# swacisko/ALGA

Hardware: AMD Instinct MI355X
Metric: overlap_edges_per_sec (higher is better)
Workload: dtype u32; 1 GPU; cfg4_50M_150bp: 50000000 x 150 bp reads, genome 250000000, seed 11, err 0.00 -> 90621096 nodes (both strands, duplicates removed), min_overlap 82, rsoemo 116; generated on the device (alga_amd.workload.device_build) in 1.0 s; nodes=90621096, edges=92350115

## Files before the change

### alga_amd/csrc/engine.hip

```cpp
#include <hip/hip_runtime.h>

#include <algorithm>
#include <chrono>
#include <cstdio>
#include <cstdlib>
#include <cstring>
#include <new>
#include <string>
#include <thread>
#include <vector>

#include "engine_internal.h"

using namespace alga;

namespace {

using Prepared = AlgaPrepared;

int prepare(alga_engine *e, const alga_nodes *nodes, const alga_prefsuf_params *p, hipStream_t s, Prepared &out) {
    if (!nodes || !p) return alga_fail(e, ALGA_ERR_INVALID_ARGUMENT, "nodes/params must not be NULL");
    if (nodes->n < 0) return alga_fail(e, ALGA_ERR_INVALID_ARGUMENT, "negative node count");
    if (nodes->n > 0 && (!nodes->words || !nodes->len)) return alga_fail(e, ALGA_ERR_INVALID_ARGUMENT, "words/len must not be NULL");
    if (nodes->stride_words <= 0 && nodes->n > 0) return alga_fail(e, ALGA_ERR_INVALID_ARGUMENT, "stride_words must be positive");
    if (p->min_overlap < 1 || p->min_overlap > 501) return alga_fail(e, ALGA_ERR_INVALID_ARGUMENT, "min_overlap must be in [1, 501]");
    if (p->soes != 3) return alga_fail(e, ALGA_ERR_INVALID_ARGUMENT, "soes must be 3 (the reference hard-codes SOES = 3)");
    if (p->max_len_cap < 1 || p->max_len_cap > 500) return alga_fail(e, ALGA_ERR_INVALID_ARGUMENT, "max_len_cap must be in [1, 500]");
    if (p->rsoe_min_overlap < 0) return alga_fail(e, ALGA_ERR_INVALID_ARGUMENT, "rsoe_min_overlap must be >= 0");
    if (p->keys_shared < 0 || p->keys_shared > 2) return alga_fail(e, ALGA_ERR_INVALID_ARGUMENT, "keys_shared must be 0, 1 or 2");
    int rc;
    if ((rc = alga_ensure(e, e->counters, (CNT_TOTAL + 2) * sizeof(unsigned long long)))) return rc;
    HIP_TRY(e, hipMemsetAsync(e->counters.p, 0, (CNT_TOTAL + 2) * sizeof(unsigned long long), s));
    NodesDev nd;
    nd.words = nodes->words; nd.len = nodes->len; nd.from = nodes->align_from; nd.to = nodes->align_to;
    nd.n = nodes->n; nd.stride = nodes->stride_words;
    unsigned long long *cnt = (unsigned long long *) e->counters.p;
    int *d_maxlen = (int *) (cnt + CNT_TOTAL);
    unsigned long long mask_asym = 0;
    int min_len = 0;
    if (p->keys_shared == 2 && e->store_n == nodes->n && e->store_words == (const void *) nodes->words && e->stat_len == (const void *) nodes->len &&
        e->stat_from == (const void *) nodes->align_from && e->stat_to == (const void *) nodes->align_to) {
        out.max_len = e->stat_max_len; out.live = e->stat_live; mask_asym = e->stat_mask_asym; min_len = e->stat_min_len;
    } else {
        launch_node_stats(nd, cnt, d_maxlen, s);
        if ((rc = alga_check_launch(e, "k_node_stats"))) return rc;
        HIP_TRY(e, hipMemcpyAsync(e->h_counters, e->counters.p, (CNT_TOTAL + 2) * sizeof(unsigned long long), hipMemcpyDeviceToHost, s));
        HIP_TRY(e, hipStreamSynchronize(s));
        out.max_len = (int) (e->h_counters[CNT_TOTAL] & 0xFFFFFFFFull);
        min_len = out.max_len > 0 ? 0x7FFFFFFF - (int) (e->h_counters[CNT_TOTAL] >> 32) : 0;
        out.live = e->h_counters[CNT_LIVE_NODES];
        mask_asym = e->h_counters[CNT_MASK_ASYM];
        e->stat_max_len = out.max_len; e->stat_min_len = min_len; e->stat_live = out.live; e->stat_mask_asym = mask_asym;
        e->stat_len = (const void *) nodes->len; e->stat_from = (const void *) nodes->align_from; e->stat_to = (const void *) nodes->align_to;
    }
    out.nd = nd;
    out.uniform_len = (out.max_len > 0 && min_len == out.max_len && !nodes->align_from) ? out.max_len : 0;
    if ((int64_t) blocks_of(out.max_len) > (int64_t) nodes->stride_words)
        return alga_fail(e, ALGA_ERR_INVALID_ARGUMENT, "stride_words is smaller than the longest read needs");
    if (out.max_len > OL_MAX_NODE_LEN) return alga_fail(e, ALGA_ERR_CAPACITY, "a node is longer than 4 194 303 nt (overlap records keep the offset in 22 bits)");
    PrefSufCfg c;
    c.Lmin = p->min_overlap;
    c.rsoemo = p->rsoe_min_overlap;
    c.Lcap = std::min(out.max_len, p->max_len_cap) + 1;
    c.soes = p->soes;
    const int seed_nt = std::min(c.Lmin, SEED_MAX_NT);
    c.seed_words = (2 * seed_nt + 31) >> 5;
    c.seed_last_mask = (2 * seed_nt & 31) ? ((1u << (2 * seed_nt & 31)) - 1u) : 0xFFFFFFFFu;
    c.reversed = (c.rsoemo > c.Lcap) ? 1 : 0;
    c.stats = p->collect_stats ? 1 : 0;
    out.cfg = c;
    if (p->reduction < ALGA_REDUCTION_AUTO || p->reduction > ALGA_REDUCTION_SOURCE_SIDE)
        return alga_fail(e, ALGA_ERR_INVALID_ARGUMENT, "reduction must be an alga_reduction value");
    out.local_ok = out.max_len <= p->max_len_cap && out.max_len - c.Lmin <= LOCAL_MAX_SPAN && c.Lmin <= c.rsoemo && c.rsoemo <= c.Lcap &&
                   mask_asym == 0;
    out.local_sw = out.max_len - c.Lmin <= 63 ? 1 : 2;
    out.cluster_eq = 0;
    const bool wide = out.local_sw == 2 || blocks_of(out.max_len) > 13;
    if (out.local_ok && e->opt_probe != ALGA_PROBE_TABLE && !(wide && e->opt_probe == ALGA_PROBE_AUTO && out.live < (4ull << 20))) {
        int eq = 0;
        if (cluster_plan(c, out.max_len, out.live, e->opt_cluster_bucket_bias, &out.cluster, &eq)) out.cluster_eq = eq;
    }
    out.keys_shared = p->keys_shared;
    out.reduction = p->reduction;
    if (out.reduction == ALGA_REDUCTION_AUTO && e->opt_force_per_target) out.reduction = ALGA_REDUCTION_PER_TARGET;
    return ALGA_OK;
}

int cluster_alloc(alga_engine *e, const Prepared &pp) {
    int rc;
    const uint64_t n = (uint64_t) pp.nd.n;
    for (int k = 0; k < 2; k++) {
        if ((rc = alga_ensure(e, e->cl_keys[k], (n + ALGA_KEY_ARRAY_SLACK + 1) * sizeof(uint32_t)))) return rc;
        if ((rc = alga_ensure(e, e->cl_vals[k], (n + 1) * sizeof(uint32_t)))) return rc;
    }
    if ((rc = alga_ensure(e, e->cl_meta, (n + ALGA_KEY_ARRAY_SLACK + 1) * sizeof(uint32_t)))) return rc;
    if ((rc = alga_ensure(e, e->cl_runs, (n + 1) * CL_RMAX * 8))) return rc;
    if ((rc = alga_ensure(e, e->cl_nruns, n + 16))) return rc;
    if ((rc = alga_ensure(e, e->cl_store, (n + 2) * 16 * (size_t) pp.cluster_eq))) return rc;
    if ((rc = alga_ensure(e, e->cl_dir, ((size_t) pp.cluster.n_buckets + 2) * 16))) return rc;
    return alga_ensure(e, e->sort_temp, cluster_sort_temp_bytes(n));
}

int pile_alloc(alga_engine *e, uint64_t n, uint32_t n_buckets, hipStream_t s) {
    int rc;
    if ((rc = alga_ensure(e, e->cl_pile_rec, pile_record_bytes(n)))) return rc;
    if ((rc = alga_ensure(e, e->cl_pile_rec2, pile_record_bytes(n)))) return rc;
    if ((rc = alga_ensure(e, e->cl_pile_succ, ((size_t) n + 64) * 16))) return rc;
    if ((rc = alga_ensure(e, e->cl_pile_cnt, PILE_CNT_WORDS * sizeof(unsigned long long)))) return rc;
    if ((rc = alga_ensure(e, e->cl_pile_own, pile_own_mask_bytes(n)))) return rc;
    if (e->opt_pile_runs_list && (rc = alga_ensure(e, e->cl_pile_list, pile_list_bytes(n)))) return rc;
    if ((rc = alga_ensure(e, e->cl_defer, (size_t) (n + 64) * sizeof(int32_t)))) return rc;
    const void *before = e->cl_pile_tab.p;
    const size_t cap_before = e->cl_pile_tab.cap;
    if ((rc = alga_ensure(e, e->cl_pile_tab, pile_table_bytes(n_buckets)))) return rc;
    if (e->cl_pile_tab.p != before || e->cl_pile_tab.cap != cap_before) {
        HIP_TRY(e, hipMemsetAsync(e->cl_pile_tab.p, 0, e->cl_pile_tab.cap, s));
        HIP_TRY(e, hipStreamSynchronize(s));
        e->pile_epoch = 0;
    }
    return ALGA_OK;
}

int discover_impl(alga_engine *e, const Prepared &pp, int32_t src_begin, int32_t src_end, hipStream_t s, uint64_t *n_rec, bool local = false,
                  bool *overflow = nullptr) {
    int rc;
    const NodesDev &nd = pp.nd;
    const PrefSufCfg &cfg = pp.cfg;
    unsigned long long *cnt = (unsigned long long *) e->counters.p;
    *n_rec = 0;
    HIP_TRY(e, hipEventRecord(e->ev[EV_START], s));
    if (pp.live >= (1ull << 31)) return alga_fail(e, ALGA_ERR_CAPACITY, "too many nodes for one seed table; shard the input");
    const bool clustered = local && pp.cluster_eq != 0;
    e->pairs_timed = false;
    e->store_timed = false;
    e->pile_timed = false;
    e->pile_deg_pending = false;
    const bool all_sources = src_begin == 0 && src_end == pp.nd.n;
    const bool pile_index_left = e->opt_pile_range != 0 && e->pile_n == pp.nd.n && e->pile_words == (const void *) pp.nd.words;
    bool pile = clustered && e->opt_pile != 0 && e->opt_cluster_pairs != 0 && e->opt_cluster_order != 0 && pp.local_sw == 1 &&
                      (pp.keys_shared == 0 || (pp.keys_shared == 2 && pile_index_left)) &&
                      (all_sources || (e->opt_pile_range != 0 && src_begin >= 0 && src_end <= pp.nd.n && src_begin < src_end)) && pile_plan(cfg, pp.cluster, pp.cluster_eq, pp.uniform_len, pp.nd.from != nullptr || pp.nd.to != nullptr);
    e->loc_second_used = false;
    bool keys_only = false;
    const bool need_vals = !e->opt_own_sort || e->opt_test_unsorted_index;
    uint32_t n_buckets = 0, filter_bits = 0;
    bool have_table = false;
    auto build_table = [&]() -> int {
        n_buckets = seed_buckets_for(pp.live, e->seed_fill_x10);
        const size_t table_bytes = (size_t) n_buckets * SEED_BUCKET * sizeof(unsigned long long);
        int r;
        if ((r = alga_ensure(e, e->table, table_bytes))) return r;
        HIP_TRY(e, hipMemsetAsync(e->table.p, 0xFF, table_bytes, s));
        filter_bits = seed_filter_bits_for(pp.live);
        if (filter_bits) {
            if ((r = alga_ensure(e, e->filter, filter_bits / 8))) return r;
            HIP_TRY(e, hipMemsetAsync(e->filter.p, 0, filter_bits / 8, s));
        }
        launch_seed_build(nd, cfg, (unsigned long long *) e->table.p, n_buckets, (uint32_t *) e->filter.p, filter_bits, s);
        if ((r = alga_check_launch(e, "k_seed_build"))) return r;
        e->stats.table_slots = (uint64_t) n_buckets * SEED_BUCKET;
        have_table = true;
        return ALGA_OK;
    };
    ClusterCfg cc{};
    if (clustered) {
        cc = pp.cluster;
        if ((rc = cluster_alloc(e, pp))) return rc;
        if (pp.keys_shared == 2) {
            const bool store_left = e->store_n == nd.n && e->store_words == (const void *) nd.words && e->store_eq == pp.cluster_eq && e->store_buckets == cc.n_buckets;
            const bool piles_serve = pile && e->pile_kept_pure && e->store_buckets == cc.n_buckets && e->store_eq == pp.cluster_eq;
            if (!(store_left || piles_serve) || src_begin < e->store_run_begin || src_end > e->store_run_end)
                return alga_fail(e, ALGA_ERR_INVALID_ARGUMENT, "keys_shared = 2: no entry array of this node set that covers the sources is left from the previous build");
            keys_only = pile && e->pile_keys_only;
        } else {
            int32_t run_begin = 0, run_end = nd.n;
            if (pp.keys_shared == 1) {
                if (e->keyed_n != nd.n || e->keyed_words != (const void *) nd.words || src_begin < e->keyed_begin || src_end > e->keyed_end)
                    return alga_fail(e, ALGA_ERR_INVALID_ARGUMENT, "keys_shared: alga_prefsuf_keys_device has not been called on this node set for a range that covers the sources");
                run_begin = e->keyed_begin; run_end = e->keyed_end;
            } else {
                keys_only = pile && e->opt_pile_runs != 0 && !e->expect_pairwise && !e->opt_pile_check;
                launch_cluster_keys(nd, cfg, cc, 0, nd.n, (uint32_t *) e->cl_keys[0].p, need_vals ? (uint32_t *) e->cl_vals[0].p : nullptr, (uint32_t *) e->cl_meta.p, e->cl_runs.p,
                                    (uint8_t *) e->cl_nruns.p, s, !keys_only);
                if ((rc = alga_check_launch(e, "k_node_runs"))) return rc;
            }
            HIP_TRY(e, hipEventRecord(e->ev[EV_KEYS], s));
            e->keyed_n = -1;
            e->store_n = -1;
            HIP_TRY(e, launch_cluster_store(nd, cc, (uint32_t *) e->cl_keys[0].p, (uint32_t *) e->cl_vals[0].p, (uint32_t *) e->cl_keys[1].p,
                                            (uint32_t *) e->cl_vals[1].p, e->sort_temp.p, cluster_sort_temp_bytes((uint64_t) nd.n), e->cl_dir.p, pp.keys_shared == 1 || !need_vals,
                                            e->ev[EV_SORT], cnt + CNT_TOTAL + 1, e->opt_test_unsorted_index != 0, s, e->opt_own_sort != 0));
            HIP_TRY(e, hipEventRecord(e->ev[EV_DIR], s));
            e->pile_n = -1;
            if (pile) {
                rc = e->opt_test_pile_oom ? alga_fail(e, ALGA_ERR_OUT_OF_MEMORY, "pile_alloc (option test_pile_oom)") : pile_alloc(e, (uint64_t) nd.n, cc.n_buckets, s);
                if (rc == ALGA_ERR_OUT_OF_MEMORY) {
                    (void) hipGetLastError();
                    alga_release(e->cl_pile_tab); alga_release(e->cl_pile_rec); alga_release(e->cl_pile_rec2); alga_release(e->cl_pile_succ); alga_release(e->cl_pile_own);
                    alga_release(e->cl_pile_list);
                    e->pile_epoch = 0; e->pile_n = -1;
                    e->err.clear();
                    pile = false;
                    rc = ALGA_OK;
                    if (keys_only) {
                        launch_cluster_keys(nd, cfg, cc, 0, nd.n, (uint32_t *) e->cl_keys[0].p, (uint32_t *) e->cl_vals[0].p, (uint32_t *) e->cl_meta.p, e->cl_runs.p,
                                            (uint8_t *) e->cl_nruns.p, s, true);
                        if ((rc = alga_check_launch(e, "k_node_runs"))) return rc;
                        keys_only = false;
                    }
                } else if (rc) return rc;
            }
            if (pile) {
                launch_pile_sample(nd, cc, pp.uniform_len, (const uint32_t *) e->cl_keys[1].p, (const uint32_t *) e->cl_vals[1].p, e->cl_dir.p,
                                   (unsigned long long *) e->cl_pile_cnt.p, e->opt_pile >= 2 ? e->opt_pile - 1 : 0, s);
                if ((rc = alga_check_launch(e, "k_pile_build<sample>"))) return rc;
            }
            HIP_TRY(e, launch_cluster_gather(nd, cc, pp.cluster_eq, (const uint32_t *) e->cl_keys[1].p, (const uint32_t *) e->cl_vals[1].p, (const uint32_t *) e->cl_meta.p,
                                             pp.uniform_len, e->cl_store.p, (pile && e->opt_pile_skip_gather) ? (const unsigned long long *) e->cl_pile_cnt.p : nullptr, s));
            HIP_TRY(e, hipEventRecord(e->ev[EV_GATHER], s));
            if (pile) {
                if (e->pile_epoch >= 511u) {
                    HIP_TRY(e, hipMemsetAsync(e->cl_pile_tab.p, 0, e->cl_pile_tab.cap, s));
                    e->pile_epoch = 0;
                }
                e->pile_epoch++;
                const bool from_consensus = e->opt_pile_runs != 0;
                launch_pile_build(nd, cfg, cc, pp.uniform_len, (const uint32_t *) e->cl_keys[1].p, (const uint32_t *) e->cl_vals[1].p, e->cl_dir.p, e->cl_pile_rec.p, e->cl_pile_rec2.p, e->cl_pile_tab.p,
                                  e->pile_epoch, e->cl_pile_succ.p, e->cl_runs.p, pp.uniform_len - cfg.Lmin + 1, (const unsigned long long *) e->cl_pile_cnt.p,
                                  from_consensus ? (uint32_t *) e->cl_pile_own.p : nullptr, (from_consensus && e->opt_pile_runs_list) ? e->cl_pile_list.p : nullptr, s);
                if ((rc = alga_check_launch(e, "k_pile_build"))) return rc;
                if (keys_only) {
                    launch_pile_own_ids((const uint32_t *) e->cl_pile_own.p, (const uint32_t *) e->cl_vals[1].p, (uint64_t) nd.n, (int32_t *) e->cl_defer.p, (uint32_t) nd.n,
                                        (unsigned long long *) e->cl_pile_cnt.p, s);
                    launch_cluster_runs_list(nd, cfg, cc, (const int32_t *) e->cl_defer.p, (const unsigned long long *) e->cl_pile_cnt.p + 3, (uint32_t) nd.n, (uint32_t) e->n_cu * 16u,
                                             e->cl_runs.p, (uint8_t *) e->cl_nruns.p, s);
                    launch_cluster_keys(nd, cfg, cc, 0, nd.n, (uint32_t *) e->cl_keys[0].p, (uint32_t *) e->cl_vals[0].p, (uint32_t *) e->cl_meta.p, e->cl_runs.p,
                                        (uint8_t *) e->cl_nruns.p, s, true, (const unsigned long long *) e->cl_pile_cnt.p);
                    if ((rc = alga_check_launch(e, "k_node_runs (own lists)"))) return rc;
                }
                if (e->opt_pile_check && from_consensus)
                    launch_pile_check(e->cl_pile_succ.p, (uint64_t) nd.n, cc.n_buckets, e->cl_pile_tab.p, e->cl_pile_rec2.p, e->pile_epoch, e->cl_runs.p, nd.n, pp.uniform_len - cfg.Lmin + 1,
                                      (unsigned long long *) e->cl_pile_cnt.p, s);
                e->pile_n = nd.n; e->pile_words = (const void *) nd.words;
                e->pile_keys_only = keys_only; e->pile_kept_pure = false;
                e->pile_timed = nd.n > 0;
            }
            e->store_timed = nd.n > 0;
            e->store_n = pile ? -1 : nd.n;
            e->store_words = (const void *) nd.words; e->store_eq = pp.cluster_eq; e->store_buckets = cc.n_buckets;
            e->store_run_begin = run_begin; e->store_run_end = run_end;
        }
        e->stats.table_slots = cc.n_buckets;
    } else if ((rc = build_table())) return rc;
    HIP_TRY(e, hipEventRecord(e->ev[EV_SEED], s));

    const uint64_t n_src = (uint64_t) std::max<int64_t>(0, (int64_t) src_end - src_begin);
    const uint64_t slack = std::max(probe_record_slack(e->n_cu, n_src, local), clustered ? cluster_record_slack(e->n_cu, n_src) : 0);
    uint64_t &hint = local ? e->rec_cap_hint_local : e->rec_cap_hint;
    uint64_t cap = std::max<uint64_t>(hint, (local ? 2 : 16) * n_src + 4096) + slack;
    if (local) {
        if ((rc = alga_ensure(e, e->outdeg, (size_t) (n_src + 1) * sizeof(uint32_t)))) return rc;
        if ((rc = alga_ensure(e, e->loc_first, (size_t) (n_src + 1) * sizeof(unsigned long long)))) return rc;
    }
    const uint32_t big_list_cap = 1u << 20;
    if (local && (rc = alga_ensure(e, e->loc_big_list, big_list_cap * sizeof(int32_t)))) return rc;
    for (int attempt = 0; attempt < 4; attempt++) {
        if (cap >= (1ull << 32) - 16) return alga_fail(e, ALGA_ERR_CAPACITY, "more than 2^32 overlap records; shard the input");
        if (local) HIP_TRY(e, hipMemsetAsync(e->outdeg.p, 0, (size_t) (n_src + 1) * sizeof(uint32_t), s));
        if ((rc = alga_ensure(e, e->rec_dst, cap * sizeof(uint32_t)))) return rc;
        if ((rc = alga_ensure(e, e->rec_val, cap * sizeof(unsigned long long)))) return rc;
        HIP_TRY(e, hipMemsetAsync(cnt, 0, CNT_TOTAL * sizeof(unsigned long long), s));
        ProbeBig big{(int32_t *) e->loc_big_list.p, big_list_cap, 0u, nullptr, 0u};
        e->defer_list_valid = clustered && e->opt_cluster_pairs && pp.local_sw == 1 && pp.cluster_eq <= 4;
        if (clustered) {
            if (e->opt_cluster_pairs && pp.local_sw == 1 && pp.cluster_eq <= 4) {
                if ((rc = alga_ensure(e, e->cl_defer, (size_t) (n_src + 64) * sizeof(int32_t)))) return rc;
                const uint32_t slot_stride = e->opt_stream_slots >= 4 ? (uint32_t) (n_src + 1) : 0u;
                if ((rc = alga_ensure(e, e->loc_second, (size_t) (slot_stride ? LOCAL_SLOTS_MAX - 1 : 1) * (n_src + 1) * sizeof(unsigned long long)))) return rc;
                e->loc_second_used = true;
                e->loc_slot_stride = slot_stride;
                const bool by_key = e->opt_cluster_order != 0 && src_begin == 0 && src_end == nd.n;
                const bool piled = pile && e->pile_n == nd.n && e->pile_words == (const void *) nd.words;
                if (piled) {
                    if (!all_sources) {
                        if ((rc = alga_ensure(e, e->cl_pile_side_r, (size_t) (n_src + 64) * 16))) return rc;
                        if ((rc = alga_ensure(e, e->cl_pile_cursor, 64))) return rc;
                    }
                    launch_pile_probe(nd, cfg, cc, pp.uniform_len, e->cl_pile_tab.p, e->pile_epoch, e->cl_pile_rec.p, e->cl_pile_rec2.p, e->cl_pile_succ.p,
                                      e->cl_runs.p, cnt, (uint32_t *) e->outdeg.p, (unsigned long long *) e->loc_first.p, (unsigned long long *) e->loc_second.p,
                                      (int32_t *) e->cl_defer.p, (uint32_t) n_src, (const unsigned long long *) e->cl_pile_cnt.p, e->n_cu, s, src_begin, src_end,
                                      e->cl_pile_side_r.p, (unsigned long long *) e->cl_pile_cursor.p, e->opt_pile_probe_lean != 0);
                    if ((rc = alga_check_launch(e, "k_pile_probe"))) return rc;
                    if (keys_only)
                        launch_cluster_runs_list(nd, cfg, cc, (const int32_t *) e->cl_defer.p, cnt + CNT_DEFERRED, (uint32_t) std::min<uint64_t>(n_src + 64, 0xFFFFFFFFull),
                                                 (uint32_t) e->n_cu * 16u, e->cl_runs.p, (uint8_t *) e->cl_nruns.p, s);
                }
                launch_probe_stream(nd, cfg, cc, pp.cluster_eq, e->cl_store.p, e->cl_dir.p, e->cl_runs.p, (const uint8_t *) e->cl_nruns.p,
                                    src_begin, src_end, by_key, cnt, e->n_cu, (uint32_t *) e->outdeg.p, (unsigned long long *) e->loc_first.p,
                                    (unsigned long long *) e->loc_second.p, (int32_t *) e->cl_defer.p, (uint32_t) n_src,
                                    piled ? (const unsigned long long *) e->cl_pile_cnt.p : nullptr, s, slot_stride);
                if ((rc = alga_check_launch(e, "k_probe_stream"))) return rc;
                if (piled) {
                    if ((rc = alga_ensure(e, e->cl_defer2, (size_t) (n_src + 64) * sizeof(int32_t)))) return rc;
                    launch_probe_stream_list(nd, cfg, cc, pp.cluster_eq, e->cl_store.p, e->cl_dir.p, e->cl_runs.p, (const uint8_t *) e->cl_nruns.p, (int32_t *) e->cl_defer.p,
                                             (uint32_t) n_src, cnt, e->n_cu, (uint32_t *) e->outdeg.p, (unsigned long long *) e->loc_first.p,
                                             (unsigned long long *) e->loc_second.p, (int32_t *) e->cl_defer2.p, (const unsigned long long *) e->cl_pile_cnt.p, s, slot_stride, src_begin);
                    if ((rc = alga_check_launch(e, "k_probe_stream (list)"))) return rc;
                }
                HIP_TRY(e, hipEventRecord(e->ev[EV_PAIRS], s));
                e->pairs_timed = true;
                launch_probe_clustered(nd, cfg, cc, pp.cluster_eq, e->cl_store.p, e->cl_dir.p, e->cl_runs.p, (const uint8_t *) e->cl_nruns.p, 0,
                                       (int32_t) n_src, (const int32_t *) e->cl_defer.p, src_begin, (uint32_t *) e->rec_dst.p, (unsigned long long *) e->rec_val.p,
                                       cap, cnt, e->n_cu, (uint32_t *) e->outdeg.p, (unsigned long long *) e->loc_first.p, &big, cnt + CNT_DEFERRED, 1, s,
                                       (const uint32_t *) e->cl_keys[1].p, (const uint32_t *) e->cl_vals[1].p, pp.uniform_len,
                                       (piled && e->opt_pile_skip_gather) ? (const unsigned long long *) e->cl_pile_cnt.p : nullptr);
                e->pile_deg_pending = piled && e->opt_pile_deg_fold != 0;
                if (piled && !e->pile_deg_pending) launch_pile_deg((int32_t) n_src, (unsigned long long *) e->loc_first.p, (uint32_t *) e->outdeg.p, (const unsigned long long *) e->cl_pile_cnt.p, s);
            } else {
                launch_probe_clustered(nd, cfg, cc, pp.cluster_eq, e->cl_store.p, e->cl_dir.p, e->cl_runs.p, (const uint8_t *) e->cl_nruns.p, src_begin,
                                       src_end, nullptr, src_begin, (uint32_t *) e->rec_dst.p, (unsigned long long *) e->rec_val.p, cap, cnt, e->n_cu,
                                       (uint32_t *) e->outdeg.p, (unsigned long long *) e->loc_first.p, &big, nullptr, pp.local_sw, s);
            }
        }
        else
            launch_probe(nd, cfg, (const unsigned long long *) e->table.p, n_buckets, (const uint32_t *) e->filter.p, filter_bits, src_begin, src_end,
                         (uint32_t *) e->rec_dst.p, (unsigned long long *) e->rec_val.p, cap, cnt, e->n_cu, local ? pp.local_sw : 0, (uint32_t *) e->outdeg.p,
                         (unsigned long long *) e->loc_first.p, local ? &big : nullptr, s);
        if ((rc = alga_check_launch(e, "k_probe_sources"))) return rc;
        HIP_TRY(e, hipEventRecord(e->ev[EV_PROBE], s));
        HIP_TRY(e, hipMemcpyAsync(e->h_counters, cnt, (CNT_TOTAL + 2) * sizeof(unsigned long long), hipMemcpyDeviceToHost, s));
        HIP_TRY(e, hipStreamSynchronize(s));
        if (clustered && e->h_counters[CNT_TOTAL + 1] != 0) {
            e->store_n = -1; e->keyed_n = -1;
            return alga_fail(e, ALGA_ERR_HIP, "clustered index: the sorted key array is not in order (entry directory invalid)");
        }
        if (local && e->h_counters[CNT_LOCAL_OVERFLOW] != 0) {
            const uint64_t n_big = e->h_counters[CNT_LOCAL_OVERFLOW], max_items = e->h_counters[CNT_LOCAL_MAXITEMS];
            const uint64_t limit = e->big_limit >= 0 ? (uint64_t) e->big_limit : (uint64_t) local_big_limit();
            if (n_big > big_list_cap || max_items > limit) { if (overflow) *overflow = true; *n_rec = 0; return ALGA_OK; }
            big.count = (uint32_t) n_big;
            big.item_cap = (uint32_t) ((max_items + 63) & ~63ull);
            if ((rc = alga_ensure(e, e->loc_big_items, probe_big_bytes(e->n_cu, big.count, pp.local_sw, big.item_cap)))) return rc;
            big.items = e->loc_big_items.p;
            if (!have_table && (rc = build_table())) return rc;
            if (e->pile_deg_pending) {
                launch_pile_deg((int32_t) n_src, (unsigned long long *) e->loc_first.p, (uint32_t *) e->outdeg.p, (const unsigned long long *) e->cl_pile_cnt.p, s);
                e->pile_deg_pending = false;
            }
            HIP_TRY(e, hipMemsetAsync(cnt + CNT_LOCAL_OVERFLOW, 0, sizeof(unsigned long long), s));
            launch_probe(nd, cfg, (const unsigned long long *) e->table.p, n_buckets, (const uint32_t *) e->filter.p, filter_bits, src_begin, src_end,
                         (uint32_t *) e->rec_dst.p, (unsigned long long *) e->rec_val.p, cap, cnt, e->n_cu, pp.local_sw, (uint32_t *) e->outdeg.p,
                         (unsigned long long *) e->loc_first.p, &big, s);
            if ((rc = alga_check_launch(e, "k_probe_sources (second pass)"))) return rc;
            HIP_TRY(e, hipEventRecord(e->ev[EV_PROBE], s));
            HIP_TRY(e, hipMemcpyAsync(e->h_counters, cnt, CNT_TOTAL * sizeof(unsigned long long), hipMemcpyDeviceToHost, s));
            HIP_TRY(e, hipStreamSynchronize(s));
            if (e->h_counters[CNT_LOCAL_OVERFLOW] != 0) { if (overflow) *overflow = true; *n_rec = 0; return ALGA_OK; }
            e->stats.big_sources = n_big;
        }
        const uint64_t need = e->h_counters[CNT_RECORDS];
        if (need <= cap) {
            *n_rec = need;
            hint = std::max<uint64_t>(hint, need + need / 16 + 4096);
            if (overflow) *overflow = false;
            if (local) { e->stats.transitive_compares = e->h_counters[CNT_TR_COMPARES]; e->stats.generic_sources = e->h_counters[CNT_LOCAL_GENERIC]; }
            e->stats.records = e->h_counters[CNT_VALID_RECORDS];
            e->stats.raw_overlaps = e->h_counters[CNT_RAW];
            e->stats.windows_probed = e->h_counters[CNT_WINDOWS];
            e->stats.slots_scanned = e->h_counters[CNT_SLOTS];
            e->stats.probe_rounds = e->h_counters[CNT_ROUNDS];
            e->stats.pile_buckets = e->h_counters[CNT_PILE_BUCKETS]; e->stats.pile_irregular = e->h_counters[CNT_PILE_IRREGULAR];
            e->stats.pile_own_lists = e->h_counters[CNT_PILE_OWN];
            if (pile && pp.keys_shared != 2 && e->pile_n == nd.n) {
                const bool kept = e->opt_pile == 2 || e->stats.pile_irregular * (uint64_t) ALGA_PILE_DECLINE_ONE_IN <= e->stats.pile_buckets;
                e->stats.pile_mixed = kept && e->stats.pile_irregular * (uint64_t) ALGA_PILE_IRREGULAR_ONE_IN > e->stats.pile_buckets;
                e->stats.pile_deferred = e->stats.pile_mixed ? e->h_counters[CNT_DEFERRED_PILE] : (kept ? e->h_counters[CNT_DEFERRED] : 0);
                if (!kept || e->stats.pile_mixed || !e->opt_pile_skip_gather) e->store_n = nd.n;
                e->expect_pairwise = !kept;
                e->pile_kept_pure = kept && !e->stats.pile_mixed && e->opt_pile_skip_gather != 0;
                e->stats.pile_list_checked = 0; e->stats.pile_list_mismatch = 0;
                if (e->opt_pile_check) {
                    unsigned long long chk[2] = {0ull, 0ull};
                    HIP_TRY(e, hipMemcpyAsync(chk, (const unsigned long long *) e->cl_pile_cnt.p + 4, sizeof(chk), hipMemcpyDeviceToHost, s));
                    HIP_TRY(e, hipStreamSynchronize(s));
                    e->stats.pile_list_checked = chk[0]; e->stats.pile_list_mismatch = chk[1];
                }
            }
            if (!pile) e->expect_pairwise = false;
            e->stats.probe_used = clustered ? ALGA_PROBE_CLUSTER : ALGA_PROBE_TABLE;
            if (clustered) e->stats.deferred_sources = e->defer_list_valid ? e->h_counters[CNT_DEFERRED] : n_src;
            return ALGA_OK;
        }
        cap = need + need / 16 + 4096 + slack;
    }
    return alga_fail(e, ALGA_ERR_HIP, "record buffer kept overflowing");
}

int key_bits_for(int64_t n_owned) {
    int b = 1;
    while (b < 31 && (1ll << b) < n_owned) b++;
    return std::min(32, b + 1);
}

int reduce_impl(alga_engine *e, const Prepared &pp, const uint32_t *rec_dst, const unsigned long long *rec_val, uint64_t n_rec,
                uint64_t n_valid_hint, int32_t dst_begin, int32_t dst_end, hipStream_t s, uint64_t *n_edges) {
    int rc;
    const NodesDev &nd = pp.nd;
    const PrefSufCfg &cfg = pp.cfg;
    unsigned long long *cnt = (unsigned long long *) e->counters.p;
    const int32_t n_owned = dst_end - dst_begin;
    *n_edges = 0;
    if (n_rec >= (1ull << 32) - 16) return alga_fail(e, ALGA_ERR_CAPACITY, "more than 2^32 overlap records; shard the input");
    const int bits = key_bits_for(n_owned);
    const size_t temp_bytes = sort_records_temp_bytes(n_rec, bits);
    if ((rc = alga_ensure(e, e->keys, (size_t) (n_rec + 1) * sizeof(uint32_t)))) return rc;
    if ((rc = alga_ensure(e, e->seg_key, (size_t) (n_rec + 1) * sizeof(uint32_t)))) return rc;
    if ((rc = alga_ensure(e, e->seg_val, (size_t) (n_rec + 1) * sizeof(unsigned long long)))) return rc;
    if ((rc = alga_ensure(e, e->sort_temp, temp_bytes))) return rc;
    if ((rc = alga_ensure(e, e->heads, (size_t) (n_rec + 1) * 16))) return rc;
    if ((rc = alga_ensure(e, e->rowptr, (size_t) (n_owned + 2) * sizeof(uint32_t)))) return rc;
    HIP_TRY(e, hipMemsetAsync(cnt + CNT_SORT_VALID, 0, sizeof(unsigned long long), s));
    launch_make_keys(rec_dst, n_rec, dst_begin, dst_end, (uint32_t *) e->keys.p, cnt + CNT_SORT_VALID, s);
    if ((rc = alga_check_launch(e, "k_make_keys"))) return rc;
    HIP_TRY(e, sort_records(e->sort_temp.p, temp_bytes, (const uint32_t *) e->keys.p, (uint32_t *) e->seg_key.p, rec_val,
                            (unsigned long long *) e->seg_val.p, n_rec, bits, s));
    launch_rowptr_from_sorted((const uint32_t *) e->seg_key.p, cnt + CNT_SORT_VALID, n_rec, n_owned, (uint32_t *) e->rowptr.p, s);
    if ((rc = alga_check_launch(e, "k_rowptr_from_sorted"))) return rc;
    launch_gather_heads(nd, (const unsigned long long *) e->seg_val.p, cnt + CNT_SORT_VALID, n_rec, e->heads.p, s);
    if ((rc = alga_check_launch(e, "k_gather_heads"))) return rc;
    HIP_TRY(e, hipEventRecord(e->ev[EV_GROUP], s));

    if ((rc = alga_ensure(e, e->out_cnt, (size_t) (n_owned + 1) * sizeof(uint32_t)))) return rc;
    if ((rc = alga_ensure(e, e->outdeg, (size_t) (nd.n + 1) * sizeof(uint32_t)))) return rc;
    HIP_TRY(e, hipMemsetAsync(e->outdeg.p, 0, (size_t) (nd.n + 1) * sizeof(uint32_t), s));
    const int tpb = reduce_targets_per_block(n_valid_hint, (uint64_t) std::max(1, n_owned));
    launch_reduce_targets(nd, cfg, dst_begin, n_owned, tpb, (const uint32_t *) e->rowptr.p, (unsigned long long *) e->seg_val.p,
                          e->heads.p, (uint32_t *) e->out_cnt.p, (uint32_t *) e->outdeg.p, cnt, s);
    if ((rc = alga_check_launch(e, "k_reduce_targets"))) return rc;
    HIP_TRY(e, hipEventRecord(e->ev[EV_REDUCE], s));

    if ((rc = alga_ensure(e, e->scan_scratch, scan_scratch_bytes((uint64_t) nd.n)))) return rc;
    if ((rc = alga_ensure(e, e->out_rowptr, (size_t) (nd.n + 1) * sizeof(uint32_t)))) return rc;
    launch_exclusive_scan((const uint32_t *) e->outdeg.p, (uint64_t) nd.n, (uint32_t *) e->out_rowptr.p, (uint64_t *) e->scan_scratch.p, s);
    if ((rc = alga_check_launch(e, "scan(outdeg)"))) return rc;
    uint64_t *d_total = (uint64_t *) e->scan_scratch.p + scan_total_index((uint64_t) nd.n);
    HIP_TRY(e, hipMemcpyAsync(&e->h_counters[CNT_TOTAL], d_total, sizeof(uint64_t), hipMemcpyDeviceToHost, s));
    HIP_TRY(e, hipMemcpyAsync(e->h_counters, cnt, CNT_TOTAL * sizeof(unsigned long long), hipMemcpyDeviceToHost, s));
    HIP_TRY(e, hipStreamSynchronize(s));
    const uint64_t E = e->h_counters[CNT_TOTAL];
    if (E >= (1ull << 32) - 16) return alga_fail(e, ALGA_ERR_CAPACITY, "more than 2^32 edges; shard the input");
    if ((rc = alga_ensure(e, e->edges, (size_t) (E + 1) * sizeof(alga_edge_dev)))) return rc;
    launch_scatter_by_source(cfg, dst_begin, n_owned, (const uint32_t *) e->rowptr.p, (const unsigned long long *) e->seg_val.p,
                             (const uint32_t *) e->out_cnt.p, (const uint32_t *) e->out_rowptr.p, (uint32_t *) e->outdeg.p,
                             (alga_edge_dev *) e->edges.p, s);
    if ((rc = alga_check_launch(e, "k_scatter_by_source"))) return rc;
    launch_sort_rows(nd.n, (const uint32_t *) e->out_rowptr.p, (alga_edge_dev *) e->edges.p, s);
    if ((rc = alga_check_launch(e, "k_sort_rows"))) return rc;
    HIP_TRY(e, hipEventRecord(e->ev[EV_EMIT], s));
    HIP_TRY(e, hipStreamSynchronize(s));
    *n_edges = E;
    e->stats.edges = E;
    e->stats.transitive_listed = e->h_counters[CNT_TR_LISTED];
    e->stats.transitive_compares = e->h_counters[CNT_TR_COMPARES];
    e->stats.transitive_removed = e->h_counters[CNT_TR_REMOVED];
    e->stats.max_in_records = e->h_counters[CNT_MAX_IN];
    return ALGA_OK;
}

int finalize_local(alga_engine *e, const Prepared &pp, int32_t src_begin, int32_t src_end, uint64_t n_rec, hipStream_t s, uint64_t *n_edges) {
    int rc;
    *n_edges = 0;
    const uint64_t n_src = (uint64_t) std::max<int64_t>(0, (int64_t) src_end - src_begin);
    if ((rc = alga_ensure(e, e->scan_scratch, scan_scratch_bytes(n_src)))) return rc;
    if ((rc = alga_ensure(e, e->out_rowptr, (size_t) (n_src + 1) * sizeof(uint32_t)))) return rc;
    if ((rc = alga_ensure(e, e->out_cnt, (size_t) (n_src + 1) * sizeof(uint32_t)))) return rc;
    HIP_TRY(e, hipEventRecord(e->ev[EV_GROUP], s));
    HIP_TRY(e, hipEventRecord(e->ev[EV_REDUCE], s));
    if (e->pile_deg_pending)
        launch_exclusive_scan_pile_deg((uint32_t *) e->outdeg.p, n_src, (uint32_t *) e->out_rowptr.p, (uint64_t *) e->scan_scratch.p, (unsigned long long *) e->loc_first.p,
                                       (const unsigned long long *) e->cl_pile_cnt.p, s);
    else
        launch_exclusive_scan((const uint32_t *) e->outdeg.p, n_src, (uint32_t *) e->out_rowptr.p, (uint64_t *) e->scan_scratch.p, s);
    e->pile_deg_pending = false;
    if ((rc = alga_check_launch(e, "scan(outdeg)"))) return rc;
    const uint64_t E = e->stats.records;
    if (E >= (1ull << 32) - 16) return alga_fail(e, ALGA_ERR_CAPACITY, "more than 2^32 edges; shard the input");
    if ((rc = alga_ensure(e, e->edges, (size_t) (E + 1) * sizeof(alga_edge_dev)))) return rc;
    launch_local_emit(src_begin, (int32_t) n_src, (const uint32_t *) e->outdeg.p, (const unsigned long long *) e->loc_first.p,
                      e->loc_second_used ? (const unsigned long long *) e->loc_second.p : nullptr, (const uint32_t *) e->rec_dst.p, (const unsigned long long *) e->rec_val.p, n_rec, (const uint32_t *) e->out_rowptr.p,
                      (uint32_t *) e->out_cnt.p, (alga_edge_dev *) e->edges.p,
                      e->defer_list_valid ? (const int32_t *) e->cl_defer.p : nullptr, (const unsigned long long *) e->counters.p + CNT_DEFERRED, (uint32_t) n_src, s,
                      e->loc_second_used ? e->loc_slot_stride : 0u);
    if ((rc = alga_check_launch(e, "k_local_emit"))) return rc;
    HIP_TRY(e, hipEventRecord(e->ev[EV_EMIT], s));
    uint64_t *d_total = (uint64_t *) e->scan_scratch.p + scan_total_index(n_src);
    HIP_TRY(e, hipMemcpyAsync(&e->h_counters[CNT_TOTAL], d_total, sizeof(uint64_t), hipMemcpyDeviceToHost, s));
    HIP_TRY(e, hipStreamSynchronize(s));
    if (e->h_counters[CNT_TOTAL] != E) return alga_fail(e, ALGA_ERR_HIP, "source-side emit: out-degrees and edge count disagree");
    *n_edges = E;
    e->stats.edges = E;
    return ALGA_OK;
}

int build_local(alga_engine *e, const Prepared &pp, int32_t src_begin, int32_t src_end, hipStream_t s, uint64_t *n_edges) {
    if (!pp.local_ok) return alga_fail(e, ALGA_ERR_UNSUPPORTED, "source-side reduction is not exact for this input (read lengths / masks / rsoemo)");
    uint64_t n_rec = 0;
    bool overflow = false;
    int rc = discover_impl(e, pp, src_begin, src_end, s, &n_rec, true, &overflow);
    if (rc) return rc;
    if (overflow) return alga_fail(e, ALGA_ERR_UNSUPPORTED, "a source node has more raw overlaps than the source-side reduction holds");
    if ((rc = finalize_local(e, pp, src_begin, src_end, n_rec, s, n_edges))) return rc;
    e->stats.reduction_used = ALGA_REDUCTION_SOURCE_SIDE;
    return ALGA_OK;
}

double now_ms_host() { return std::chrono::duration<double, std::milli>(std::chrono::steady_clock::now().time_since_epoch()).count(); }

float ev_ms(alga_engine *e, int a, int b) {
    float ms = 0.f;
    if (hipEventElapsedTime(&ms, e->ev[a], e->ev[b]) != hipSuccess) return 0.f;
    return ms;
}

void store_phase_stats(alga_engine *e) {
    if (!e->store_timed) return;
    e->stats.ms_keys = ev_ms(e, EV_START, EV_KEYS);
    e->stats.ms_sort = ev_ms(e, EV_KEYS, EV_SORT);
    e->stats.ms_dir = ev_ms(e, EV_SORT, EV_DIR);
    e->stats.ms_gather = ev_ms(e, EV_DIR, EV_GATHER);
    e->stats.ms_pile = e->pile_timed ? ev_ms(e, EV_GATHER, EV_SEED) : 0.0;
}

}

int alga_prepare(alga_engine *e, const alga_nodes *nodes, const alga_prefsuf_params *p, hipStream_t s, AlgaPrepared &out) { return prepare(e, nodes, p, s, out); }
int alga_cluster_alloc(alga_engine *e, const AlgaPrepared &pp) { return cluster_alloc(e, pp); }

extern "C" {

int alga_abi_version(void) { return ALGA_AMD_ABI_VERSION; }

struct DeviceGuard {
    int prev = -1;
    DeviceGuard() { if (hipGetDevice(&prev) != hipSuccess) prev = -1; }
    ~DeviceGuard() { if (prev >= 0) (void) hipSetDevice(prev); }
};

static void engine_free_handles(alga_engine *e) {
    if (e->h_counters) (void) hipHostFree(e->h_counters);
    for (int i = 0; i < EV_COUNT; i++) if (e->ev[i]) (void) hipEventDestroy(e->ev[i]);
    if (e->own_stream) (void) hipStreamDestroy(e->own_stream);
    if (e->side_stream) (void) hipStreamDestroy(e->side_stream);
    if (e->ev_side) (void) hipEventDestroy(e->ev_side);
    e->h_counters = nullptr; e->own_stream = nullptr; e->side_stream = nullptr; e->ev_side = nullptr;
    for (int i = 0; i < EV_COUNT; i++) e->ev[i] = nullptr;
}

int alga_engine_create(int hip_device, alga_engine **out) {
    if (!out) return ALGA_ERR_INVALID_ARGUMENT;
    *out = nullptr;
    int ndev = 0;
    hipError_t err = hipGetDeviceCount(&ndev);
    if (err != hipSuccess || ndev <= 0) return ALGA_ERR_NO_DEVICE;
    if (hip_device < 0 || hip_device >= ndev) return ALGA_ERR_INVALID_ARGUMENT;
    DeviceGuard guard;
    if (hipSetDevice(hip_device) != hipSuccess) return ALGA_ERR_NO_DEVICE;
    alga_engine *e = new (std::nothrow) alga_engine();
    if (!e) return ALGA_ERR_OUT_OF_MEMORY;
    e->device = hip_device;
    memset(&e->stats, 0, sizeof(e->stats));
    hipDeviceProp_t prop;
    if (hipGetDeviceProperties(&prop, hip_device) == hipSuccess) {
        snprintf(e->dev_name, sizeof(e->dev_name), "%s (%s, %d CUs)", prop.name, prop.gcnArchName, prop.multiProcessorCount);
        if (prop.multiProcessorCount > 0) e->n_cu = prop.multiProcessorCount;
    }
    int rc = ALGA_OK;
    if (hipStreamCreateWithFlags(&e->own_stream, hipStreamNonBlocking) != hipSuccess) { e->own_stream = nullptr; rc = ALGA_ERR_HIP; }
    if (rc == ALGA_OK && hipStreamCreateWithFlags(&e->side_stream, hipStreamNonBlocking) != hipSuccess) { e->side_stream = nullptr; rc = ALGA_ERR_HIP; }
    if (rc == ALGA_OK && hipEventCreateWithFlags(&e->ev_side, hipEventDisableTiming) != hipSuccess) { e->ev_side = nullptr; rc = ALGA_ERR_HIP; }
    for (int i = 0; i < EV_COUNT && rc == ALGA_OK; i++)
        if (hipEventCreate(&e->ev[i]) != hipSuccess) { e->ev[i] = nullptr; rc = ALGA_ERR_HIP; }
    if (rc == ALGA_OK && hipHostMalloc((void **) &e->h_counters, (CNT_TOTAL + 2 + alga_engine::H_EXTRA) * sizeof(unsigned long long)) != hipSuccess) { e->h_counters = nullptr; rc = ALGA_ERR_OUT_OF_MEMORY; }
    if (rc == ALGA_OK && hipHostGetDevicePointer((void **) &e->h_counters_dev, e->h_counters, 0) != hipSuccess) rc = ALGA_ERR_HIP;
    if (rc != ALGA_OK) { engine_free_handles(e); delete e; return rc; }
    *out = e;
    return ALGA_OK;
}

void alga_engine_destroy(alga_engine *e) {
    if (!e) return;
    DeviceGuard guard;
    (void) hipSetDevice(e->device);
    if (e->own_stream) (void) hipStreamSynchronize(e->own_stream);
    if (e->side_stream) (void) hipStreamSynchronize(e->side_stream);
    for (DevBuf *b : e->owned) alga_release(*b);
    alga_release(e->up_raw);
    for (DevBuf *b : {&e->in_bytes[0], &e->in_bytes[1], &e->in_nl[0], &e->in_nl[1], &e->in_tiles, &e->in_tile_off}) alga_release(*b);
    for (DevBuf *b : {&e->sp_rowptr, &e->sp_sorted, &e->sp_list, &e->sp_cnt, &e->sp_orow, &e->sp_out, &e->sp_in}) alga_release(*b);
    alga_staging_release(e);
    for (void *&p : e->gfa_pin) { if (p) (void) hipHostFree(p); p = nullptr; }
    for (auto &kv : e->host_lists) free(kv.first);
    e->host_lists.clear();
    engine_free_handles(e);
    delete e;
}

const char *alga_last_error(const alga_engine *e) { return e ? e->err.c_str() : "no engine"; }

int alga_engine_device_name(const alga_engine *e, char *buf, size_t buflen) {
    if (!e || !buf || buflen == 0) return ALGA_ERR_INVALID_ARGUMENT;
    snprintf(buf, buflen, "%s", e->dev_name);
    return ALGA_OK;
}

int alga_engine_set_option(alga_engine *e, const char *name, int64_t value) {
    if (!e || !name) return ALGA_ERR_INVALID_ARGUMENT;
    e->err.clear();
    if (!strcmp(name, "probe")) {
        if (value < ALGA_PROBE_AUTO || value > ALGA_PROBE_CLUSTER) return alga_fail(e, ALGA_ERR_INVALID_ARGUMENT, "option probe: 0 auto, 1 table, 2 cluster");
        e->opt_probe = (int) value;
    } else if (!strcmp(name, "cluster_bucket_bias")) {
        if (value < -8 || value > 8) return alga_fail(e, ALGA_ERR_INVALID_ARGUMENT, "option cluster_bucket_bias: -8 .. 8");
        e->opt_cluster_bucket_bias = (int) value;
    } else if (!strcmp(name, "cluster_pairs")) {
        e->opt_cluster_pairs = value != 0;
    } else if (!strcmp(name, "pile")) {
        e->opt_pile = (value == 2 || value == 3) ? (int) value : (value != 0);
    } else if (!strcmp(name, "pile_runs")) {
        e->opt_pile_runs = value != 0;
    } else if (!strcmp(name, "pile_runs_list")) {
        e->opt_pile_runs_list = value != 0;
    } else if (!strcmp(name, "pile_deg_fold")) {
        e->opt_pile_deg_fold = value != 0;
    } else if (!strcmp(name, "pile_probe_lean")) {
        e->opt_pile_probe_lean = value != 0;
    } else if (!strcmp(name, "pile_check")) {
        e->opt_pile_check = value != 0;
    } else if (!strcmp(name, "pile_skip_gather")) {
        e->opt_pile_skip_gather = value != 0;
    } else if (!strcmp(name, "cluster_order")) {
        e->opt_cluster_order = value != 0;
    } else if (!strcmp(name, "local_big_max")) {
        e->big_limit = value < 0 ? -1 : (int) std::min<int64_t>(value, 1 << 20);
    } else if (!strcmp(name, "shard_bucket_max")) {
        e->opt_shard_dmax = (int) std::max<int64_t>(1, std::min<int64_t>(value, 4096));
    } else if (!strcmp(name, "rsort_variant")) {
        rsort_set_variant((int) value);
    } else if (!strcmp(name, "stream_slots")) {
        e->opt_stream_slots = value >= 4 ? 4 : 2;
    } else if (!strcmp(name, "pile_range")) {
        e->opt_pile_range = value != 0;
    } else if (!strcmp(name, "pkb_legacy")) {
        e->opt_pkb_legacy = (int) value;
    } else if (!strcmp(name, "own_sort")) {
        e->opt_own_sort = value != 0;
    } else if (!strcmp(name, "test_presort_oom")) {
        e->opt_test_presort_oom = value != 0;
    } else if (!strcmp(name, "test_pile_oom")) {
        e->opt_test_pile_oom = value != 0;
    } else if (!strcmp(name, "test_unsorted_index")) {
        e->opt_test_unsorted_index = value != 0;
    } else if (!strcmp(name, "gfa_chunk_mb")) {
        if (value < 1 || value > 4096) return alga_fail(e, ALGA_ERR_INVALID_ARGUMENT, "option gfa_chunk_mb: 1 .. 4096");
        e->opt_gfa_chunk_mb = (int) value;
    } else if (!strcmp(name, "mst_mid_nodes")) {
        if (value < 8 || value > (1 << 20)) return alga_fail(e, ALGA_ERR_INVALID_ARGUMENT, "option mst_mid_nodes: 8 .. 2^20");
        e->opt_mst_mid_nodes = (int) value;
    } else if (!strcmp(name, "consensus_max_blocks")) {
        if (value < 0 || value > (1 << 20)) return alga_fail(e, ALGA_ERR_INVALID_ARGUMENT, "option consensus_max_blocks: 0 .. 2^20");
        e->opt_consensus_max_blocks = (int) value;
    } else if (!strcmp(name, "unitig_ruling")) {
        if (value < -1 || value > 1) return alga_fail(e, ALGA_ERR_INVALID_ARGUMENT, "option unitig_ruling: -1, 0 or 1");
        e->opt_unitig_ruling = (int) value;
    } else if (!strcmp(name, "auto_reduction_per_target")) {
        e->opt_force_per_target = value != 0;
    } else return alga_fail(e, ALGA_ERR_INVALID_ARGUMENT, "unknown option");
    return ALGA_OK;
}

int alga_engine_reserve(alga_engine *e, int32_t n_nodes, int32_t max_len, int32_t min_overlap, uint64_t n_edges_hint) {
    if (!e) return ALGA_ERR_INVALID_ARGUMENT;
    e->err.clear();
    if (n_nodes < 0 || max_len < 1 || min_overlap < 1) return alga_fail(e, ALGA_ERR_INVALID_ARGUMENT, "alga_engine_reserve: n_nodes >= 0, max_len >= 1, min_overlap >= 1");
    DeviceGuard guard;
    HIP_TRY(e, hipSetDevice(e->device));
    int rc;
    const uint64_t n = (uint64_t) n_nodes;
    const uint64_t E = n_edges_hint ? n_edges_hint : n + n / 16 + 4096;
    if ((rc = alga_ensure(e, e->counters, (CNT_TOTAL + 2) * sizeof(unsigned long long)))) return rc;
    Prepared pp;
    pp.nd.n = n_nodes; pp.max_len = max_len; pp.live = n;
    pp.cfg.Lmin = min_overlap; pp.cfg.Lcap = std::min(max_len, 500) + 1; pp.cfg.rsoemo = min_overlap; pp.cfg.soes = 3;
    int eq = 0;
    const bool local = max_len <= 500 && max_len - min_overlap <= LOCAL_MAX_SPAN;
    const bool clustered = local && e->opt_probe != ALGA_PROBE_TABLE &&
                           cluster_plan(pp.cfg, max_len, n, e->opt_cluster_bucket_bias, &pp.cluster, &eq);
    if (clustered) {
        pp.cluster_eq = eq;
        if ((rc = cluster_alloc(e, pp))) return rc;
        if (max_len - min_overlap <= 63 && eq <= 4) {
            if ((rc = alga_ensure(e, e->cl_defer, (size_t) (n + 64) * sizeof(int32_t)))) return rc;
            if ((rc = alga_ensure(e, e->loc_second, (size_t) (e->opt_stream_slots >= 4 ? LOCAL_SLOTS_MAX - 1 : 1) * (n + 1) * sizeof(unsigned long long)))) return rc;
        }
        if (e->opt_pile != 0 && e->opt_cluster_pairs != 0 && e->opt_cluster_order != 0 && max_len - min_overlap <= 63 && pile_plan(pp.cfg, pp.cluster, eq, max_len, false)) {
            if ((rc = pile_alloc(e, n, pp.cluster.n_buckets, e->own_stream))) return rc;
        }
    } else {
        const uint32_t nb = seed_buckets_for(n, e->seed_fill_x10);
        if ((rc = alga_ensure(e, e->table, (size_t) nb * SEED_BUCKET * sizeof(unsigned long long)))) return rc;
        const uint32_t fb = seed_filter_bits_for(n);
        if (fb && (rc = alga_ensure(e, e->filter, fb / 8))) return rc;
    }
    if (local) {
        const uint64_t slack = std::max(probe_record_slack(e->n_cu, n, true), clustered ? cluster_record_slack(e->n_cu, n) : 0);
        const uint64_t cap = std::max<uint64_t>(e->rec_cap_hint_local, 2 * n + 4096) + slack;
        if ((rc = alga_ensure(e, e->outdeg, (size_t) (n + 1) * sizeof(uint32_t)))) return rc;
        if ((rc = alga_ensure(e, e->loc_first, (size_t) (n + 1) * sizeof(unsigned long long)))) return rc;
        if ((rc = alga_ensure(e, e->loc_big_list, (1u << 20) * sizeof(int32_t)))) return rc;
        if ((rc = alga_ensure(e, e->rec_dst, cap * sizeof(uint32_t)))) return rc;
        if ((rc = alga_ensure(e, e->rec_val, cap * sizeof(unsigned long long)))) return rc;
        if ((rc = alga_ensure(e, e->scan_scratch, scan_scratch_bytes(n)))) return rc;
        if ((rc = alga_ensure(e, e->out_rowptr, (size_t) (n + 1) * sizeof(uint32_t)))) return rc;
        if ((rc = alga_ensure(e, e->out_cnt, (size_t) (n + 1) * sizeof(uint32_t)))) return rc;
    }
    if ((rc = alga_ensure(e, e->edges, (size_t) (E + 1) * sizeof(alga_edge_dev)))) return rc;
    if (!e->warmed && n_nodes > 0) {
        const int W = blocks_of(max_len), stride = hbm_row_stride(W), wn = 4096;
        std::vector<uint32_t> rows((size_t) wn * stride, 0u);
        std::vector<int32_t> lens((size_t) wn, max_len);
        uint64_t x = 0x9E3779B97F4A7C15ull;
        for (int i = 0; i < wn; i++)
            for (int k = 0; k < W; k++) {
                x ^= x << 13; x ^= x >> 7; x ^= x << 17;
                uint32_t w = (uint32_t) (x >> 16);
                const int used = 2 * max_len - 32 * k;
                if (used < 32) w &= used <= 0 ? 0u : ((1u << used) - 1u);
                rows[(size_t) i * stride + k] = w;
            }
        void *d_rows = nullptr, *d_len = nullptr;
        if (hipMalloc(&d_rows, rows.size() * 4) == hipSuccess && hipMalloc(&d_len, lens.size() * 4) == hipSuccess &&
            hipMemcpy(d_rows, rows.data(), rows.size() * 4, hipMemcpyHostToDevice) == hipSuccess &&
            hipMemcpy(d_len, lens.data(), lens.size() * 4, hipMemcpyHostToDevice) == hipSuccess) {
            alga_nodes nd{(const uint32_t *) d_rows, stride, (const int32_t *) d_len, wn, nullptr, nullptr};
            alga_prefsuf_params wp;
            alga_prefsuf_default_params(&wp);
            wp.min_overlap = min_overlap; wp.rsoe_min_overlap = std::min(max_len, min_overlap + (max_len - min_overlap) / 2);
            const alga_edge *d = nullptr;
            uint64_t m = 0;
            const int wrc = alga_prefsuf_build_device(e, &nd, &wp, nullptr, &d, &m);
            (void) wrc;
            e->err.clear();
            e->warmed = true;
        }
        if (d_rows) (void) hipFree(d_rows);
        if (d_len) (void) hipFree(d_len);
        (void) hipGetLastError();
        alga_forget_node_set(e);
        memset(&e->stats, 0, sizeof(e->stats));
    }
    return ALGA_OK;
}

void alga_prefsuf_default_params(alga_prefsuf_params *p) {
    if (!p) return;
    memset(p, 0, sizeof(*p));
    p->min_overlap = 0;
    p->rsoe_min_overlap = 0;
    p->soes = 3;
    p->max_len_cap = 500;
    p->collect_stats = 0;
}

int alga_prefsuf_build_device(alga_engine *e, const alga_nodes *nodes, const alga_prefsuf_params *p, void *hip_stream,
                              const alga_edge **d_edges, uint64_t *n_edges) {
    if (!e) return ALGA_ERR_INVALID_ARGUMENT;
    e->err.clear();
    if (!d_edges || !n_edges) return alga_fail(e, ALGA_ERR_INVALID_ARGUMENT, "output pointers must not be NULL");
    *d_edges = nullptr; *n_edges = 0;
    HIP_TRY(e, hipSetDevice(e->device));
    hipStream_t s = hip_stream ? (hipStream_t) hip_stream : e->own_stream;
    memset(&e->stats, 0, sizeof(e->stats));
    Prepared pp;
    int rc = prepare(e, nodes, p, s, pp);
    if (rc) return rc;
    e->stats.nodes_live = pp.live;
    uint64_t n_rec = 0, E = 0;
    bool done = false;
    if (pp.reduction == ALGA_REDUCTION_SOURCE_SIDE || (pp.reduction == ALGA_REDUCTION_AUTO && pp.local_ok)) {
        rc = build_local(e, pp, 0, nodes->n, s, &E);
        if (rc == ALGA_OK) done = true;
        else if (rc != ALGA_ERR_UNSUPPORTED || pp.reduction == ALGA_REDUCTION_SOURCE_SIDE) return rc;
        else { e->err.clear(); memset(&e->stats, 0, sizeof(e->stats)); e->stats.nodes_live = pp.live; }
    }
    if (!done) {
        if ((rc = discover_impl(e, pp, 0, nodes->n, s, &n_rec))) return rc;
        if ((rc = reduce_impl(e, pp, (const uint32_t *) e->rec_dst.p, (const unsigned long long *) e->rec_val.p, n_rec, e->stats.records,
                              0, nodes->n, s, &E))) return rc;
        e->stats.reduction_used = ALGA_REDUCTION_PER_TARGET;
    }
    e->stats.ms_seed = ev_ms(e, EV_START, EV_SEED);
    e->stats.ms_probe = ev_ms(e, EV_SEED, EV_PROBE);
    e->stats.ms_probe_pairs = e->pairs_timed ? ev_ms(e, EV_SEED, EV_PAIRS) : 0.0;
    store_phase_stats(e);
    e->stats.ms_group = ev_ms(e, EV_PROBE, EV_GROUP);
    e->stats.ms_reduce = ev_ms(e, EV_GROUP, EV_REDUCE);
    e->stats.ms_emit = ev_ms(e, EV_REDUCE, EV_EMIT);
    e->stats.ms_total = ev_ms(e, EV_START, EV_EMIT);
    *d_edges = (const alga_edge *) e->edges.p;
    *n_edges = E;
    return ALGA_OK;
}

static int upload_nodes_impl(alga_engine *e, const alga_nodes *nodes, alga_nodes *dev, bool twin_rows, int mode = 0, uint64_t row_begin = 0, uint64_t row_end = 0,
                             uint64_t raw_rows_cap = 0, uint32_t **d_raw = nullptr);

int alga_upload_nodes(alga_engine *e, const alga_nodes *nodes, alga_nodes *dev) { return upload_nodes_impl(e, nodes, dev, false); }
int alga_upload_twin_nodes(alga_engine *e, const alga_nodes *nodes, alga_nodes *dev) { return upload_nodes_impl(e, nodes, dev, true); }
int alga_upload_nodes_phase(alga_engine *e, const alga_nodes *nodes, bool twin_rows, int mode, uint64_t row_begin, uint64_t row_end, uint64_t raw_rows_cap, alga_nodes *dev,
                            uint32_t **d_raw) { return upload_nodes_impl(e, nodes, dev, twin_rows, mode, row_begin, row_end, raw_rows_cap, d_raw); }

static int upload_nodes_impl(alga_engine *e, const alga_nodes *nodes, alga_nodes *dev, bool twin_rows, int mode, uint64_t row_begin, uint64_t row_end, uint64_t raw_rows_cap,
                             uint32_t **d_raw) {
    if (!e) return ALGA_ERR_INVALID_ARGUMENT;
    e->err.clear();
    if (!nodes || !dev) return alga_fail(e, ALGA_ERR_INVALID_ARGUMENT, "nodes / output must not be NULL");
    if (nodes->n < 0 || (nodes->n > 0 && (!nodes->words || !nodes->len || nodes->stride_words <= 0)))
        return alga_fail(e, ALGA_ERR_INVALID_ARGUMENT, "bad node set");
    HIP_TRY(e, hipSetDevice(e->device));
    hipStream_t s = e->own_stream;
    int rc;
    const size_t n = (size_t) nodes->n;
    const double t_check0 = now_ms_host();
    int32_t max_len = 0;
    if (twin_rows && (n & 1)) return alga_fail(e, ALGA_ERR_INVALID_ARGUMENT, "twin_rows: the node count must be even");
    const char *check_msg = nullptr;
    double check_ms = 0.0;
    auto check = [&]() {
        const int T = n >= (1u << 22) ? 8 : 1;
        int32_t part[8] = {0, 0, 0, 0, 0, 0, 0, 0};
        char bad[8] = {0, 0, 0, 0, 0, 0, 0, 0};
        auto job = [&](int t) {
            int32_t m = 0; char b = 0;
            size_t i0 = n * (size_t) t / T, i1 = n * (size_t) (t + 1) / T;
            i0 &= ~(size_t) 1; if (t + 1 < T) i1 &= ~(size_t) 1;
            if (twin_rows) { for (size_t i = i0; i + 1 < i1 + 1 && i + 1 < n; i += 2) { const int32_t a = nodes->len[i], c = nodes->len[i + 1]; m = std::max(m, std::max(a, c)); b |= (a != 0 && a != c); } }
            else for (size_t i = i0; i < i1; i++) m = std::max(m, nodes->len[i]);
            part[t] = m; bad[t] = b;
        };
        std::vector<std::thread> th;
        try { for (int t = 1; t < T; t++) th.emplace_back(job, t); } catch (...) { }
        job(0);
        for (size_t t = th.size() + 1; t < (size_t) T; t++) job((int) t);
        for (std::thread &x : th) x.join();
        bool any_bad = false;
        int32_t mx = 0;
        for (int t = 0; t < T; t++) { mx = std::max(mx, part[t]); any_bad = any_bad || bad[t]; }
        max_len = mx;
        if ((int64_t) blocks_of(mx) > (int64_t) nodes->stride_words) check_msg = "stride_words is smaller than the longest read needs";
        else if (any_bad) check_msg = "twin_rows: node 2k is neither removed nor as long as node 2k + 1";
        check_ms = now_ms_host() - t_check0;
    };
    struct Joiner { std::thread t; ~Joiner() { if (t.joinable()) t.join(); } } chk;
    bool async_check = n >= (1u << 22) && mode != 2;
    if (mode == 2) async_check = false;
    if (async_check) { try { chk.t = std::thread(check); } catch (...) { async_check = false; } }
    if (!async_check && mode != 2) { check(); if (check_msg) return alga_fail(e, ALGA_ERR_INVALID_ARGUMENT, check_msg); }
    const double t_up0 = now_ms_host();
    auto upload_len = [&]() -> int {
        int r;
        const int len_bytes = max_len <= 255 ? 1 : (max_len <= 65535 ? 2 : 4);
        if (len_bytes == 4 || n < (1u << 20)) return alga_staged_h2d(e, e->up_len.p, nodes->len, n * sizeof(int32_t));
        if ((r = alga_ensure(e, e->up_len_narrow, n * (size_t) len_bytes + 16))) return r;
        const int32_t *src = nodes->len;
        const AlgaStageFill fill = [src, len_bytes](void *dst, size_t off, size_t bytes) {
            if (len_bytes == 1) { uint8_t *d = (uint8_t *) dst; const int32_t *p = src + off; for (size_t i = 0; i < bytes; i++) d[i] = (uint8_t) p[i]; }
            else { uint16_t *d = (uint16_t *) dst; const int32_t *p = src + off / 2; for (size_t i = 0; i < bytes / 2; i++) d[i] = (uint16_t) p[i]; }
        };
        if ((r = alga_staged_h2d_fill(e, e->up_len_narrow.p, n * (size_t) len_bytes, fill))) return r;
        launch_widen_len(e->up_len_narrow.p, len_bytes, (int32_t *) e->up_len.p, (uint64_t) n, s);
        return alga_check_launch(e, "k_widen_len");
    };
    auto join_check = [&]() -> int {
        if (chk.t.joinable()) chk.t.join();
        return check_msg ? alga_fail(e, ALGA_ERR_INVALID_ARGUMENT, check_msg) : ALGA_OK;
    };
    const int stride_up = alga::hbm_row_stride(nodes->stride_words);
    const size_t wbytes = n * (size_t) stride_up * sizeof(uint32_t);
    const size_t raw_bytes = (twin_rows ? n / 2 : n) * (size_t) nodes->stride_words * sizeof(uint32_t);
    if (mode != 2) alga_forget_node_set(e);
    if ((rc = alga_ensure(e, e->up_words, wbytes))) return rc;
    if ((rc = alga_ensure(e, e->up_len, n * sizeof(int32_t)))) return rc;
    alga_nodes dn = *nodes;
    const size_t rows_total = twin_rows ? n / 2 : n, row_bytes = (size_t) nodes->stride_words * sizeof(uint32_t);
    const bool via_raw = twin_rows || stride_up != nodes->stride_words || mode != 0;
    if (n && mode != 2) {
        HIP_TRY(e, hipStreamSynchronize(s));
        if (via_raw) {
            if ((rc = alga_ensure(e, e->up_raw, std::max(raw_bytes, (size_t) raw_rows_cap * row_bytes) + 64))) return rc;
            const size_t r0 = mode == 1 ? (size_t) std::min<uint64_t>(row_begin, rows_total) : 0, r1 = mode == 1 ? (size_t) std::min<uint64_t>(row_end, rows_total) : rows_total;
            if (r1 > r0 && (rc = alga_staged_h2d(e, (char *) e->up_raw.p + r0 * row_bytes, (const char *) nodes->words + r0 * row_bytes, (r1 - r0) * row_bytes))) return rc;
        } else if ((rc = alga_staged_h2d(e, e->up_words.p, nodes->words, raw_bytes))) return rc;
        if ((rc = join_check())) return rc;
        if ((rc = upload_len())) return rc;
        HIP_TRY(e, hipStreamSynchronize(s));
    }
    if (d_raw) *d_raw = (uint32_t *) e->up_raw.p;
    if (mode == 1) { e->stats_host[0] = check_ms; e->stats_host[1] = now_ms_host() - t_up0; return ALGA_OK; }
    if (n && via_raw) {
        if (twin_rows) {
            launch_expand_twins((const uint32_t *) e->up_raw.p, nodes->stride_words, (const int32_t *) e->up_len.p, (uint32_t *) e->up_words.p, stride_up, (uint64_t) (n / 2), s);
            if ((rc = alga_check_launch(e, "k_expand_twins"))) return rc;
        } else {
            launch_restride((const uint32_t *) e->up_raw.p, nodes->stride_words, (uint32_t *) e->up_words.p, stride_up, (uint64_t) n, s);
            if ((rc = alga_check_launch(e, "k_restride"))) return rc;
        }
        HIP_TRY(e, hipStreamSynchronize(s));
    }
    if ((rc = join_check())) return rc;
    e->stats_host[0] = check_ms;
    dn.stride_words = stride_up;
    dn.words = (const uint32_t *) e->up_words.p;
    dn.len = (const int32_t *) e->up_len.p;
    if (nodes->align_from) {
        if ((rc = alga_ensure(e, e->up_from, n))) return rc;
        if (n && (rc = alga_staged_h2d(e, e->up_from.p, nodes->align_from, n))) return rc;
        dn.align_from = (const uint8_t *) e->up_from.p;
    }
    if (nodes->align_to) {
        if ((rc = alga_ensure(e, e->up_to, n))) return rc;
        if (n && (rc = alga_staged_h2d(e, e->up_to.p, nodes->align_to, n))) return rc;
        dn.align_to = (const uint8_t *) e->up_to.p;
    }
    *dev = dn;
    e->stats_host[1] = (mode == 2 ? e->stats_host[1] : 0.0) + now_ms_host() - t_up0;
    return ALGA_OK;
}
// ... 407 lines not shown
```

### alga_amd/csrc/engine_internal.h

```cpp
#pragma once
#include <hip/hip_runtime.h>

#include <cstdio>
#include <algorithm>
#include <string>
#include <vector>
#include <unordered_map>

#include "../../include/alga_amd.h"
#include "prefsuf_common.h"
#include "prefsuf_kernels.h"
#include "pkb_kernels.h"

struct DevBuf {
    void  *p = nullptr;
    size_t cap = 0;
};

enum { EV_START = 0, EV_SEED, EV_PROBE, EV_GROUP, EV_REDUCE, EV_EMIT, EV_PAIRS, EV_KEYS, EV_SORT, EV_GATHER, EV_DIR, EV_COUNT };
constexpr int ALGA_STAGE_THREADS = 8;

struct alga_engine {
    std::vector<DevBuf *> owned;
    int         device = -1;
    hipStream_t own_stream = nullptr;
    hipStream_t side_stream = nullptr;
    hipEvent_t  ev_side = nullptr;
    std::string err;
    char        dev_name[256] = {0};
    int         n_cu = 256;
    int         seed_fill_x10 = 20;
    int         opt_probe = 0;
    int         opt_cluster_bucket_bias = 0;
    int         opt_force_per_target = 0;
    int         opt_shard_dmax = 4096;
    int         opt_test_unsorted_index = 0;
    hipEvent_t  ev[EV_COUNT] = {};
    DevBuf table, filter, counters, rowptr, rec_dst, rec_val, keys, seg_key, seg_val, heads, sort_temp, out_cnt, outdeg, out_rowptr, edges, scan_scratch;
    DevBuf cl_defer;
    uint32_t h_first_hkey = 255;
    int32_t keyed_n = -1, keyed_begin = 0, keyed_end = 0;
    bool defer_list_valid = false;
    const void *keyed_words = nullptr;
    int32_t store_n = -1, store_run_begin = 0, store_run_end = 0, store_eq = 0;
    uint32_t store_buckets = 0;
    const void *store_words = nullptr;
    int stat_max_len = 0, stat_min_len = 0; uint64_t stat_live = 0; unsigned long long stat_mask_asym = 0;
    const void *stat_len = nullptr, *stat_from = nullptr, *stat_to = nullptr;
    bool   warmed = false;
    bool   pairs_timed = false;
    bool   store_timed = false;
    bool   pile_keys_only = false, pile_kept_pure = false;
    int    opt_pile_range = 1;
    int    opt_pile_skip_gather = 1;
    int    opt_pile = 1;
    int    opt_pile_runs = 1;
    int    opt_pile_runs_list = 1;
    DevBuf cl_pile_list;
    int    opt_pile_deg_fold = 1;
    int    opt_pile_probe_lean = 1;
    bool   pile_deg_pending = false;
    int    opt_pile_check = 0;
    bool   expect_pairwise = false;
    DevBuf cl_pile_side_r, cl_pile_cursor;
    DevBuf cl_pile_own;
    int    opt_pkb_legacy = 0;
    int    opt_own_sort = 1;
    int    opt_test_presort_oom = 0;
    int    opt_test_pile_oom = 0;
    bool   pile_timed = false;
    DevBuf cl_pile_succ;
    DevBuf cl_pile_rec2;
    DevBuf cl_pile_rec, cl_pile_cnt, cl_pile_tab;
    uint32_t pile_epoch = 0;
    int32_t pile_n = -1; const void *pile_words = nullptr;
    int    opt_cluster_order = 1;
    int    opt_cluster_pairs = 1;
    DevBuf cl_keys[2], cl_vals[2], cl_meta, cl_runs, cl_nruns, cl_store, cl_dir;
    DevBuf loc_second;
    bool   loc_second_used = false;
    uint32_t loc_slot_stride = 0;
    int    opt_stream_slots = 4;
    DevBuf loc_first, loc_big_list, loc_big_items;
    int    big_limit = -1;
    DevBuf edge_keys, edge_keys2, edge_vals, edge_vals2, edges_sorted, xs_dst, xs_val;
    DevBuf up_words, up_len, up_from, up_to;
    DevBuf up_len_narrow;
    DevBuf cp_deg, cp_dst, cp_off;
    DevBuf cl_defer2;
    DevBuf pk_keys, pk_keys2, pk_vals, pk_vals2, pk_marks, pk_big, pk_add, pk_ekeys, pk_ekeys2, pk_flag, pk_pos, pk_edges[2], pk_rowptr, pk_deg,
           pk_mask, pk_cnt, pk_io, pk_io2, pk_tips, pk_heads, pk_g[2], pk_addk, pk_addk2, pk_merged, pk_hsz, pk_hsz2, pk_heads2, pk_nadd, pk_koff,
           pk_gsz, pk_fixlist, pk_bounds, pk_tiprec, pk_tipidx, pk_keys_all, pk_vals_all;
    DevBuf pk_keys2b, pk_vals2b, pk_headsb, pk_hszb, sort_temp2, pk_fixlist2, pk_cnt2;
    DevBuf pp_rows, pp_len, pp_perm[2], pp_keys[2], pp_mark, pp_keep, pp_pos, pp_out_rows, pp_out_len, pp_out_pair, pp_tally;
    bool        stage_ready = false;
    void       *stage_pin[ALGA_STAGE_THREADS][2] = {};
    hipEvent_t  stage_ev[ALGA_STAGE_THREADS][2] = {};
    hipStream_t stage_stream[ALGA_STAGE_THREADS] = {};
    DevBuf      up_raw;
    std::unordered_map<void *, size_t> host_lists;
    void       *host_spare = nullptr;
    size_t      host_spare_cap = 0;
    DevBuf      in_bytes[2], in_nl[2], in_tiles, in_tile_off;
    DevBuf      sp_rowptr, sp_sorted, sp_list, sp_cnt, sp_orow, sp_out, sp_in;
    DevBuf      tp_cnt, tp_keys[2], tp_vals[2], tp_flag, tp_pos, tp_best, tp_est, tp_rev, tp_rfid, tp_rowptr[2], tp_alive, tp_kill, tp_rec[2], tp_branch,
                tp_overflow, tp_ws, tp_out;
    DevBuf      mp_cnt, mp_rowptr, mp_rows, mp_len, mp_owner, mp_pend[2], mp_win, mp_overflow, mp_overflow2, mp_ws, mp_ws_big, mp_orow, mp_out;
    struct MstFilled { const void *p = nullptr; size_t bytes = 0; uint32_t hbits = 0, cap_nodes = 0, cap_edges = 0; int32_t n_ws = 0; } mp_filled[2];
    int         opt_mst_mid_nodes = 4096;
    DevBuf      gfa_sizes, gfa_off, gfa_rowptr, gfa_tiles, gfa_bounds, gfa_buf;
    void       *gfa_pin[2] = {nullptr, nullptr};
    size_t      gfa_pin_cap = 0;
    int         opt_gfa_chunk_mb = 256;
    DevBuf      ut_cnt, ut_keys[2], ut_vals[2], ut_flag, ut_pos, ut_best, ut_estar, ut_rowptr, ut_nxt, ut_noff, ut_prv, ut_rank[2], ut_min[2], ut_tail,
                ut_win, ut_pair, ut_pcnt, ut_ulen, ut_ulen2, ut_uwords, ut_path_off, ut_word_off, ut_tiles, ut_path_node, ut_path_pos, ut_uid, ut_words,
                ut_edges, ut_link, ut_rnode, ut_rrec[2];
    int         opt_unitig_ruling = -1;
    uint64_t    ut_n_pairs = 0, ut_n_edges = 0;
    bool        ut_valid = false;
    int32_t     ut_n_nodes = 0;
    uint64_t    ut_total_bases = 0;
    bool        ut_is_contig = false;
    DevBuf      ex_cnt, ex_rowptr, ex_w, ex_kcnt, ex_dlink, ex_outcnt, ex_sole, ex_xhead, ex_xbase, ex_xrank, ex_uid, ex_scnt, ex_seam_off,
                ex_seam_entry, ex_pcnt, ex_uwords, ex_ulen, ex_ulen2, ex_path_off, ex_word_off, ex_path_node, ex_path_pos, ex_words, ex_edges;
    bool        ut_is_extended = false;
    DevBuf      ct_cnt, ct_B[2], ct_rowptr, ct_pflag, ct_runkey, ct_chain, ct_headchain, ct_drop, ct_flag, ct_pos, ct_keys[2], ct_vals[2], ct_hw, ct_hk, ct_H,
                ct_hrow, ct_hsorted, ct_hlist, ct_hcnt, ct_win, ct_pair, ct_oid, ct_cid, ct_deg, ct_epos, ct_ekeys[2], ct_evals[2], ct_names;
    DevBuf      cs_cnt, cs_words, cs_mask, cs_votes, cs_trim, cs_len, cs_changed;
    bool        cs_valid = false;
    bool        cs_has_votes = false;
    DevBuf      fc_cnt, fc_keys[2], fc_vals, fc_first, fc_min, fc_list[2], fc_flag, fc_ids, fc_verdict, fc_rank, fc_id, fc_new, fc_trim, fc_begin, fc_len,
                fc_order, fc_wbegin, fc_wlen, fc_rows, fc_rlen, fc_tid;
    bool        fc_valid = false;
    uint64_t    fc_n_accepted = 0;
    int         opt_consensus_max_blocks = 0;
    DevBuf      sh_keys[2], sh_vals[2], sh_store, sh_dir, sh_desc_out, sh_dkey[2], sh_dval[2], sh_small_top, sh_pending, sh_bitmap, sh_small_out,
                sh_ssrc[2], sh_skey[2], sh_edges_out, sh_deg, sh_rowptr, sh_cursor, sh_edges, sh_flagged, sh_cnt, sh_gflag, sh_gpos, sh_gstart;
    struct {
        int      phase = 0;
        int      rank = 0, n_ranks = 1, eq = 0, uniform_len = 0;
        int32_t  n = 0;
        const void *words = nullptr;
        alga::PrefSufCfg cfg{};
        alga::ClusterCfg cc{};
        uint32_t bucket_base = 0, bpr = 0;
        uint64_t n_targets = 0, n_desc = 0, n_rec = 0;
        uint32_t *d_keys_sorted = nullptr;
        unsigned long long *d_vals_sorted = nullptr;
    } sh;
    alga_shard_stats shard_stats{};
    struct {
        int      phase = 0;
        int      rounds = 0, round = 0, rank = 0, n_ranks = 1, cur = 0, key_bits = 0;
        int32_t  prio[4] = {0, 1, 2, 3};
        uint64_t E = 0, nk = 0;
        uint32_t n_tips = 0;
        int      pre_set = 0, cur_set = 0;
        bool     no_look_ahead = false;
        int      pre_round = -1;
        bool     kmers_all = false;
        size_t   kmers_stride = 0;
        int      kmers_sort_bits = 0;
        alga_nodes dn{};
        alga::PkbCfg cfg{};
    } pkb;
    unsigned long long *h_counters = nullptr;
    static constexpr int H_EXTRA = 132 + 16, H_PRE = alga::CNT_TOTAL + 2 + 132;
    uint32_t *h_counters_dev = nullptr;
    uint64_t    rec_cap_hint = 0, rec_cap_hint_local = 0;
    alga_prefsuf_stats stats;
    double      stats_host[2] = {0.0, 0.0};
    alga_pkb_stats pkb_stats;
};

struct AlgaPrepared {
    alga::NodesDev   nd;
    alga::PrefSufCfg cfg;
    int        max_len = 0;
    int        uniform_len = 0;
    uint64_t   live = 0;
    bool       local_ok = false;
    int        local_sw = 1;
    int        cluster_eq = 0;
    alga::ClusterCfg cluster{};
    int        reduction = ALGA_REDUCTION_AUTO;
    int        keys_shared = 0;
};

extern "C" int alga_upload_nodes_phase(alga_engine *e, const alga_nodes *nodes, bool twin_rows, int mode, uint64_t row_begin, uint64_t row_end, uint64_t raw_rows_cap, alga_nodes *dev,
                            uint32_t **d_raw);
int alga_prepare(alga_engine *e, const alga_nodes *nodes, const alga_prefsuf_params *p, hipStream_t s, AlgaPrepared &out);
int alga_cluster_alloc(alga_engine *e, const AlgaPrepared &pp);

inline int alga_fail(alga_engine *e, int code, const char *what, hipError_t herr = hipSuccess) {
    char buf[512];
    if (herr != hipSuccess) snprintf(buf, sizeof(buf), "%s: %s", what, hipGetErrorString(herr));
    else snprintf(buf, sizeof(buf), "%s", what);
    e->err = buf;
    return code;
}

#define HIP_TRY(e, call)                                                                     \
    do {                                                                                     \
        hipError_t _err = (call);                                                            \
        if (_err != hipSuccess) return alga_fail((e), _err == hipErrorOutOfMemory ? ALGA_ERR_OUT_OF_MEMORY : ALGA_ERR_HIP, #call, _err); \
    } while (0)

inline int alga_ensure(alga_engine *e, DevBuf &b, size_t bytes) {
    if (bytes == 0) bytes = 16;
    if (b.cap >= bytes) return ALGA_OK;
    if (b.p) { HIP_TRY(e, hipFree(b.p)); b.p = nullptr; b.cap = 0; }
    else if (std::find(e->owned.begin(), e->owned.end(), &b) == e->owned.end()) e->owned.push_back(&b);
    HIP_TRY(e, hipMalloc(&b.p, bytes));
    b.cap = bytes;
    return ALGA_OK;
}

inline void alga_forget_node_set(alga_engine *e) {
    e->keyed_n = -1; e->store_n = -1; e->pile_n = -1;
    e->stat_len = nullptr; e->stat_from = nullptr; e->stat_to = nullptr;
}

inline void alga_release(DevBuf &b) {
    if (b.p) (void) hipFree(b.p);
    b.p = nullptr; b.cap = 0;
}

#include <functional>
typedef std::function<void(void * , size_t , size_t )> AlgaStageFill;
int  alga_staged_h2d(alga_engine *e, void *d_dst, const void *h_src, size_t bytes);
int  alga_staged_h2d_fill(alga_engine *e, void *d_dst, size_t bytes, const AlgaStageFill &fill);
int  alga_staged_d2h(alga_engine *e, void *h_dst, const void *d_src, size_t bytes);
void alga_staging_release(alga_engine *e);
void *alga_host_list_take(alga_engine *e, size_t bytes);
void alga_host_list_give(alga_engine *e, void *p);

constexpr int ALGA_UT_MAX_ROUNDS = 112;
int alga_ut_check(alga_engine *e, const alga_nodes *nodes, const alga::alga_edge_dev *d_in, uint64_t m, unsigned long long *cnt, hipStream_t s);
int alga_ut_estar(alga_engine *e, const alga_nodes *nodes, const alga::alga_edge_dev *d_in, uint64_t m, unsigned long long *cnt, hipStream_t s, uint64_t *ms_out);
int alga_ut_rank(alga_engine *e, const int32_t *len, int32_t n, int32_t *nxt, const int32_t *noff, int32_t *prv, unsigned long long *cnt, uint32_t *p_flag,
                 int &cur, int &rounds, hipStream_t s);

struct AlgaTextJob {
    uint64_t items;
    std::function<void(uint32_t *sizes, unsigned long long *counters, hipStream_t s)> sizes;
    std::function<void(const unsigned long long *off, uint64_t i0, uint64_t i1, char *buf, hipStream_t s)> format;
};
int alga_text_job_run(alga_engine *e, const AlgaTextJob &job, const char *path, alga_gfa_info *info);

inline int alga_check_launch(alga_engine *e, const char *what) {
    hipError_t err = hipGetLastError();
    if (err != hipSuccess) return alga_fail(e, ALGA_ERR_HIP, what, err);
    return ALGA_OK;
}
```

### alga_amd/csrc/prefsuf_kernels.h

```cpp
#pragma once
#include <hip/hip_runtime.h>
#include <stddef.h>
#include <stdint.h>
#include "prefsuf_common.h"

namespace alga {

struct alga_edge_dev { int32_t src, dst, offset; };

void launch_restride(const uint32_t *in, int stride_in, uint32_t *out, int stride_out, uint64_t n, hipStream_t s);
void launch_widen_len(const void *in, int elem_bytes , int32_t *out, uint64_t n, hipStream_t s);
void launch_compact_edges(const alga_edge_dev *edges, int32_t n, uint64_t n_edges, uint8_t *deg, uint32_t *dst, uint8_t *off, unsigned long long *bad, hipStream_t s);
void launch_expand_twins(const uint32_t *in, int stride_in, const int32_t *len , uint32_t *out, int stride_out, uint64_t n_pairs, hipStream_t s);
void launch_node_stats(const NodesDev &nd, unsigned long long *counters, int *max_len , hipStream_t s);

uint32_t seed_buckets_for(uint64_t live_nodes, int fill_x10);
uint32_t seed_filter_bits_for(uint64_t live_nodes);
void launch_seed_build(const NodesDev &nd, const PrefSufCfg &cfg, unsigned long long *table, uint32_t n_buckets, uint32_t *filter,
                       uint32_t filter_bits, hipStream_t s);

struct ProbeBig { int32_t *list; uint32_t list_cap; uint32_t count; void *items; uint32_t item_cap; };
int    local_item_capacity();
int    local_big_limit();
size_t probe_big_bytes(int n_cu, uint32_t count, int local, uint32_t item_cap);

void launch_probe(const NodesDev &nd, const PrefSufCfg &cfg, const unsigned long long *table, uint32_t n_buckets,
                  const uint32_t *filter, uint32_t filter_bits, int32_t src_begin, int32_t src_end, uint32_t *rec_dst, unsigned long long *rec_val, uint64_t rec_cap,
                  unsigned long long *counters, int n_cu, int local , uint32_t *deg , unsigned long long *first ,
                  const ProbeBig *big , hipStream_t s);
uint64_t probe_record_slack(int n_cu, uint64_t n_src, bool local);
void launch_local_emit(int32_t src_base, int32_t n_src, const uint32_t *deg, const unsigned long long *first, const unsigned long long *second,
                       const uint32_t *rec_dst, const unsigned long long *rec_val, uint64_t n_rec, const uint32_t *rowptr, uint32_t *cursor,
                       alga_edge_dev *edges, const int32_t *record_sources, const unsigned long long *record_sources_count, uint32_t record_sources_cap, hipStream_t s, uint32_t slot_stride = 0);

bool       cluster_plan(const PrefSufCfg &cfg, int max_len, uint64_t live, int bucket_log2_bias, ClusterCfg *c, int *eq);
size_t     cluster_sort_temp_bytes(uint64_t n);
void       launch_cluster_keys(const NodesDev &nd, const PrefSufCfg &cfg, const ClusterCfg &cc, int32_t node_begin, int32_t node_end, uint32_t *keys,
                               uint32_t *vals, uint32_t *meta, void *runs, uint8_t *nruns, hipStream_t s, bool with_runs = true ,
                               const unsigned long long *only_if_declined = nullptr );
void       launch_cluster_runs_list(const NodesDev &nd, const PrefSufCfg &cfg, const ClusterCfg &cc, const int32_t *ids, const unsigned long long *count, uint32_t cap,
                                    uint32_t grid_blocks, void *runs, uint8_t *nruns, hipStream_t s);
hipError_t launch_cluster_store(const NodesDev &nd, const ClusterCfg &cc, uint32_t *keys, uint32_t *vals, uint32_t *keys2 , uint32_t *vals2, void *sort_temp,
                                size_t sort_temp_bytes, void *dir, bool fill_vals, hipEvent_t ev_sorted ,
                                unsigned long long *bad_flag ,
                                bool test_skip_sort , hipStream_t s, bool own_sort = true);
hipError_t launch_cluster_gather(const NodesDev &nd, const ClusterCfg &cc, int eq, const uint32_t *keys2, const uint32_t *vals2, const uint32_t *meta,
                                 int uniform_len , void *store,
                                 const unsigned long long *pile_cnt , hipStream_t s);
uint64_t   cluster_record_slack(int n_cu, uint64_t n_src);
void       launch_probe_clustered(const NodesDev &nd, const PrefSufCfg &cfg, const ClusterCfg &cc, int eq, const void *store, const void *dir,
                                  const void *runs, const uint8_t *nruns, int32_t src_begin, int32_t src_end, const int32_t *src_list, int32_t src_base, uint32_t *rec_dst, unsigned long long *rec_val, uint64_t rec_cap,
                                  unsigned long long *counters, int n_cu, uint32_t *deg, unsigned long long *first, const ProbeBig *big,
                                  const unsigned long long *list_count ,
                                  int sw , hipStream_t s,
                                  const uint32_t *skeys = nullptr, const uint32_t *sids = nullptr, int uniform_len = 0,
                                  const unsigned long long *pile_cnt = nullptr );
void       launch_probe_stream(const NodesDev &nd, const PrefSufCfg &cfg, const ClusterCfg &cc, int eq, const void *store, const void *dir,
                               const void *runs, const uint8_t *nruns, int32_t src_begin, int32_t src_end, bool by_key ,
                               unsigned long long *counters, int n_cu, uint32_t *deg, unsigned long long *first, unsigned long long *second, int32_t *defer_list,
                               uint32_t defer_cap, const unsigned long long *pile_cnt ,
                               hipStream_t s, uint32_t slot_stride = 0 );
void       launch_pile_deg(int32_t n, unsigned long long *first, uint32_t *deg, const unsigned long long *pile_cnt, hipStream_t s);
bool       pile_plan(const PrefSufCfg &cfg, const ClusterCfg &cc, int eq, int uniform_len, bool masks);
size_t     pile_record_bytes(uint64_t n);
size_t     pile_table_bytes(uint32_t n_buckets);
void       launch_pile_sample(const NodesDev &nd, const ClusterCfg &cc, int uniform_len, const uint32_t *skeys , const uint32_t *sids , const void *dir,
                              unsigned long long *pile_cnt , int no_sample, hipStream_t s);
constexpr int PILE_CNT_WORDS = 6;
size_t     pile_own_mask_bytes(uint64_t n);
size_t     pile_list_bytes(uint64_t n);
void       launch_pile_build(const NodesDev &nd, const PrefSufCfg &cfg, const ClusterCfg &cc, int uniform_len, const uint32_t *skeys, const uint32_t *sids, const void *dir, void *rec,
                             void *rec2 , void *tab, uint32_t epoch, void *side, const void *runs, int nwin, const unsigned long long *pile_cnt,
                             uint32_t *own_mask ,
                             void *plist , hipStream_t s);
void       launch_pile_own_ids(const uint32_t *own_mask, const uint32_t *sids, uint64_t n_entries, int32_t *list, uint32_t cap, unsigned long long *pile_cnt, hipStream_t s);
void       launch_pile_check(const void *side, uint64_t n_entries, uint32_t n_buckets, const void *tab, const void *rec2, uint32_t epoch, const void *runs, int n_nodes, int nwin,
                             unsigned long long *pile_cnt, hipStream_t s);
void       launch_probe_stream_list(const NodesDev &nd, const PrefSufCfg &cfg, const ClusterCfg &cc, int eq, const void *store, const void *dir, const void *runs, const uint8_t *nruns,
                                    int32_t *src_list, uint32_t list_cap, unsigned long long *counters, int n_cu, uint32_t *deg, unsigned long long *first,
                                    unsigned long long *second, int32_t *defer2, const unsigned long long *pile_cnt, hipStream_t s, uint32_t slot_stride = 0,
                                    int32_t src_base = 0 );
void       launch_pile_probe(const NodesDev &nd, const PrefSufCfg &cfg, const ClusterCfg &cc, int uniform_len, const void *tab, uint32_t epoch, const void *rec, const void *rec2, const void *side,
                             const void *runs, unsigned long long *counters, uint32_t *deg, unsigned long long *first, unsigned long long *second, int32_t *defer_list,
                             uint32_t defer_cap, const unsigned long long *pile_cnt, int n_cu, hipStream_t s, int32_t src_begin, int32_t src_end,
                             void *side_range , unsigned long long *cursor ,
                             bool lean = true );

size_t     rsort_u32_pairs_temp_bytes(uint64_t n);
void       rsort_set_variant(int v);
hipError_t rsort_u32_pairs(void *temp, size_t temp_bytes, const uint32_t *keys_in, uint32_t *keys_out, const uint32_t *vals_in, uint32_t *vals_out, uint64_t n,
                           int begin_bit, hipStream_t s);
size_t     sort_u32_pairs_temp_bytes(uint64_t n);
hipError_t sort_u32_pairs(void *temp, size_t temp_bytes, const uint32_t *keys_in, uint32_t *keys_out, const uint32_t *vals_in, uint32_t *vals_out,
                          uint64_t n, int begin_bit , hipStream_t s, bool own_sort = true );
size_t     rsort_u64_pairs_temp_bytes(uint64_t n);
hipError_t rsort_u64_pairs(void *temp, size_t temp_bytes, const unsigned long long *keys_in, unsigned long long *keys_out, const unsigned long long *vals_in,
                           unsigned long long *vals_out, uint64_t n, int bits, hipStream_t s);
hipError_t rsort_u32_u64(void *temp, size_t temp_bytes, const uint32_t *keys_in, uint32_t *keys_out, const unsigned long long *vals_in, unsigned long long *vals_out,
                         uint64_t n, int begin_bit, int end_bit, hipStream_t s);
size_t     sort_u64_pairs_temp_bytes(uint64_t n, int bits);
hipError_t sort_u64_pairs(void *temp, size_t temp_bytes, const unsigned long long *keys_in, unsigned long long *keys_out,
                          const unsigned long long *vals_in, unsigned long long *vals_out, uint64_t n, int bits, hipStream_t s);

void launch_make_keys(const uint32_t *rec_dst, uint64_t n_rec, int32_t dst_begin, int32_t dst_end, uint32_t *keys,
                      unsigned long long *n_valid, hipStream_t s);
size_t     sort_records_temp_bytes(uint64_t n, int bits);
hipError_t sort_records(void *temp, size_t temp_bytes, const uint32_t *keys_in, uint32_t *keys_out, const unsigned long long *vals_in,
                        unsigned long long *vals_out, uint64_t n, int bits, hipStream_t s);
void launch_rowptr_from_sorted(const uint32_t *keys, const unsigned long long *n_valid_ptr, uint64_t n_rec_max, int32_t n_owned,
                               uint32_t *rowptr, hipStream_t s);

size_t   scan_scratch_bytes(uint64_t n);
uint64_t scan_total_index(uint64_t n);
void launch_exclusive_scan(const uint32_t *in, uint64_t n, uint32_t *out, uint64_t *scratch, hipStream_t s);
void launch_exclusive_scan_pile_deg(uint32_t *deg, uint64_t n, uint32_t *out, uint64_t *scratch, unsigned long long *first, const unsigned long long *pile_cnt, hipStream_t s);
constexpr int MAIL_SEGS = 6;
struct MailSeg { const uint32_t *src; uint32_t words, dst; };
struct MailArgs {
    MailSeg seg[MAIL_SEGS];
    int n = 0;
    void add(const void *src, uint32_t words, uint32_t dst_word) { seg[n].src = (const uint32_t *) src; seg[n].words = words; seg[n].dst = dst_word; n++; }
};
void launch_mail(const MailArgs &a, uint32_t *host_block_dev, hipStream_t s);

int  reduce_targets_per_block(uint64_t n_records, uint64_t n_targets);
void launch_gather_heads(const NodesDev &nd, const unsigned long long *seg_val, const unsigned long long *n_valid_ptr, uint64_t n_rec_max,
                         void *heads , hipStream_t s);
void launch_reduce_targets(const NodesDev &nd, const PrefSufCfg &cfg, int32_t dst_begin, int32_t n_owned, int32_t targets_per_block,
                           const uint32_t *rowptr, unsigned long long *seg_val, const void *heads, uint32_t *out_cnt, uint32_t *outdeg,
                           unsigned long long *counters, hipStream_t s);
void launch_scatter_by_source(const PrefSufCfg &cfg, int32_t dst_begin, int32_t n_owned, const uint32_t *rowptr,
                              const unsigned long long *seg_val, const uint32_t *out_cnt, const uint32_t *out_rowptr, uint32_t *out_cursor,
                              alga_edge_dev *edges, hipStream_t s);
void launch_sort_rows(int32_t n, const uint32_t *out_rowptr, alga_edge_dev *edges, hipStream_t s);

void launch_edges_to_keys(const alga_edge_dev *e, uint64_t n, unsigned long long *keys, uint32_t *vals, hipStream_t s);
void launch_keys_to_edges(const unsigned long long *keys, const uint32_t *vals, uint64_t n, alga_edge_dev *e, hipStream_t s);
size_t     sort_edges_temp_bytes(uint64_t n);
hipError_t sort_edges(void *temp, size_t temp_bytes, const unsigned long long *keys_in, unsigned long long *keys_out, const uint32_t *vals_in,
                      uint32_t *vals_out, uint64_t n, int src_bits, hipStream_t s);

}
```

### alga_amd/csrc/prefsuf_pile.hip

```cpp
#include <hip/hip_runtime.h>
#include <algorithm>
#include "prefsuf_common.h"
#include "prefsuf_kernels.h"
#include "prefsuf_device.h"
#include "prefsuf_cluster_device.h"

namespace alga {

constexpr int PB_TILE = 192, PB_HALO = 64, PB_THREADS = PB_TILE + PB_HALO;
constexpr int PILE_SW = 13;
constexpr int PILE_MAXSUB = 4;
constexpr int PILE_EQ = 3;

__device__ __forceinline__ bool pile_declines(const unsigned long long *pile_cnt) { return pile_cnt_declines(pile_cnt); }

__device__ __forceinline__ uint32_t pile_who(uint32_t group, uint32_t w, uint32_t n_buckets, uint64_t n_entries) {
    return group == 0u ? min(w, n_buckets) : (uint32_t) min((uint64_t) w, n_entries) | 0x80000000u;
}

__device__ __forceinline__ void load_row9(const NodesDev &nd, uint32_t id, uint32_t (&row)[9]) {
    const uint32_t *rp = nd.words + (size_t) id * nd.stride;
    if ((nd.stride & 3) == 0 && nd.stride >= 12 && ((uintptr_t) nd.words & 15u) == 0) {
        const uint4 v0 = reinterpret_cast<const uint4 *>(rp)[0], v1 = reinterpret_cast<const uint4 *>(rp)[1];
        row[0] = v0.x; row[1] = v0.y; row[2] = v0.z; row[3] = v0.w; row[4] = v1.x; row[5] = v1.y; row[6] = v1.z; row[7] = v1.w;
        row[8] = rp[8];
    } else {
#pragma unroll
        for (int k = 0; k < 9; k++) row[k] = k < nd.stride ? rp[k] : 0u;
    }
}

template <bool SAMPLE>
__global__ void __launch_bounds__(PB_THREADS, 6) k_pile_build(NodesDev nd, const uint32_t *__restrict__ skeys, const uint32_t *__restrict__ sids, uint64_t n_entries, const uint4 *__restrict__ dir, ClusterCfg cc, int U,
                                                           uint4 *__restrict__ rec, uint4 *__restrict__ tab, uint32_t epoch,
                                                           uint4 *__restrict__ side, unsigned long long *__restrict__ pile_cnt, uint32_t *__restrict__ own_mask,
                                                           uint32_t *__restrict__ plist, uint32_t *__restrict__ pcount) {
    if (!SAMPLE && pile_declines(pile_cnt)) return;
    const int idx_shift = cc.idx_shift, kk = cc.kk;
    __shared__ uint32_t sRow[PB_THREADS][PILE_SW];
    __shared__ unsigned long long sKm[PB_THREADS];
    __shared__ unsigned long long sLead[PB_THREADS];
    __shared__ unsigned long long sRm[PB_THREADS];
    __shared__ uint32_t sMin[PB_THREADS], sMax[PB_THREADS];
    __shared__ uint32_t sBad[PB_THREADS];
    __shared__ uint8_t sTag[PB_THREADS];
    __shared__ uint32_t sCount[3];
    __shared__ uint32_t sPiles;
    const int t = (int) threadIdx.x;
    const uint64_t base = (uint64_t) blockIdx.x * PB_TILE;
    const uint64_t j = base + (uint64_t) t;
    const bool have = j < n_entries;
    const uint64_t jc = have ? j : (n_entries ? n_entries - 1 : 0);
    const uint32_t key = skeys[jc], node_id = min(sids[jc], (uint32_t) nd.n - 1u);
    const uint32_t meta = key >> (cc.idx_shift - CL_MBITS);
    const bool tgt = have && key != 0xFFFFFFFFu;
    uint4 drec = make_uint4(0u, 0u, 0u, 0u);
    if (tgt) drec = dir[key >> idx_shift];
    const uint64_t e0 = drec.x;
    const uint32_t cnt = drec.y;
    const bool owned = tgt && e0 >= base && e0 < base + PB_TILE && e0 <= j && j - e0 < (uint64_t) cnt;
    const int s = owned ? (int) (e0 - base) : 0;
    const int i = owned ? (int) (j - e0) : 0;
    const bool part = owned && cnt <= 64u;
    uint32_t row[9] = {0u, 0u, 0u, 0u, 0u, 0u, 0u, 0u, 0u};
    if (part) load_row9(nd, node_id, row);
    sLead[t] = 0ull; sRm[t] = 0ull; sMin[t] = 0xFFFFFFFFu; sMax[t] = 0u; sBad[t] = 0u;
    if (t < 3) sCount[t] = 0u;
    if (t == 0) sPiles = 0u;
    __syncthreads();
    const int m = (int) (meta & 63u);
    uint32_t A[PILE_SW];
    {
        const int w0 = (2 * m) >> 5, sh = (2 * m) & 31;
        const int lo = 2 * (64 - m), hi = lo + 2 * U;
        uint32_t Rp[18];
#pragma unroll
        for (int k = 0; k < 18; k++) Rp[k] = 0u;
#pragma unroll
        for (int k = 0; k < 9; k++) Rp[4 + k] = row[k];
        uint32_t m1 = 0u - (uint32_t) (w0 & 1), m2 = 0u - (uint32_t) ((w0 >> 1) & 1);
        asm volatile("" : "+v"(m1), "+v"(m2));
        uint32_t y1[PILE_SW + 3], y[PILE_SW + 1];
#pragma unroll
        for (int k = 0; k < PILE_SW + 3; k++) y1[k] = (Rp[k + 1] & m1) | (Rp[k] & ~m1);
#pragma unroll
        for (int k = 0; k <= PILE_SW; k++) y[k] = (y1[k + 2] & m2) | (y1[k] & ~m2);
#pragma unroll
        for (int k = 0; k < PILE_SW; k++) A[k] = funnel(y[k], y[k + 1], sh) & low_bits32(hi - 32 * k) & ~low_bits32(lo - 32 * k);
    }
    const unsigned long long kmask = kk >= 32 ? ~0ull : ((1ull << (2 * kk)) - 1ull);
    const unsigned long long kmer = (((unsigned long long) A[5] << 32) | A[4]) & kmask;
    sKm[t] = kmer;
#pragma unroll
    for (int k = 0; k < PILE_SW; k++) sRow[t][k] = A[k];
    __syncthreads();
    int L = t;
    if (part) {
        for (int u = 0; u < i; u++) if (sKm[s + u] == kmer) { L = s + u; break; }
        if (L == t) {
            atomicOr(&sLead[s], 1ull << i);
            sTag[t] = (uint8_t) (cluster_key(kmer_hash((uint32_t) kmer & cc.lo_mask, (uint32_t) (kmer >> 32) & cc.hi_mask), idx_shift - CL_MBITS) & 31u);
        }
        atomicMin(&sMin[L], ((uint32_t) m << 16) | (uint32_t) t);
        atomicMax(&sMax[L], ((uint32_t) m << 16) | (uint32_t) t);
        const unsigned long long bit = 1ull << (63 - m);
        if (atomicOr(&sRm[L], bit) & bit) atomicOr(&sBad[s], 1u);
    }
    __syncthreads();
    uint32_t *sSlot = reinterpret_cast<uint32_t *>(sKm);
    int my_slot = -1, my_rank = 0;
    if (part) {
        const unsigned long long lm = sLead[s];
        const int kgrp = __popcll(lm & ((1ull << (L - s)) - 1ull));
        if (kgrp < PILE_MAXSUB) {
            int before = 0;
            unsigned long long rest = lm;
#pragma unroll
            for (int g = 0; g < PILE_MAXSUB - 1; g++) {
                if (g < kgrp) { before += __popcll(sRm[s + __builtin_ctzll(rest)]); rest &= rest - 1ull; }
            }
            my_rank = m == 0 ? 0 : __popcll(sRm[L] >> (64 - m));
            my_slot = s + before + my_rank;
            if (my_slot < s + (int) cnt) sSlot[my_slot] = node_id; else my_slot = -1;
        }
    }
    uint32_t S[PILE_SW];
#pragma unroll
    for (int k = 0; k < PILE_SW; k++) S[k] = 0u;
    if (part) {
        const int t0 = (int) (sMax[L] & 0xFFFFu), t1 = (int) (sMin[L] & 0xFFFFu);
        const int lo = 2 * (64 - m), hi = lo + 2 * U;
        uint32_t diff = 0u;
#pragma unroll
        for (int k = 0; k < PILE_SW; k++) {
            S[k] = sRow[t0][k] | sRow[t1][k];
            diff |= (A[k] ^ S[k]) & low_bits32(hi - 32 * k) & ~low_bits32(lo - 32 * k);
        }
        if (diff != 0u) atomicOr(&sBad[s], 1u);
    }
    __syncthreads();
    if (owned) {
        uint4 *line = tab + (size_t) (key >> idx_shift) * 8;
        if (!part) {
            if (i == 0) {
                if (!SAMPLE) { line[3] = make_uint4(0u, 0u, 0u, (1u << 22) | (epoch << 23)); line[4] = make_uint4(127u, drec.x, drec.z, drec.w); }
                atomicAdd(&sCount[0], 1u); atomicAdd(&sCount[1], 1u);
            }
        } else {
            const unsigned long long lm = sLead[s];
            const int nsub = __popcll(lm);
            const int iL = L - s;
            const int k = __popcll(lm & ((1ull << iL) - 1ull));
            if (!SAMPLE) {
                const unsigned long long right = m == 0 ? 0ull : (sRm[L] >> (64 - m));
                uint32_t succ_id = 0xFFFFFFFFu, delta = 0u;
                if (right != 0ull && my_slot > s && my_rank >= 1) { succ_id = sSlot[my_slot - 1]; delta = 1u + (uint32_t) __builtin_ctzll(right); }
                const bool first_group = (k == 0 || own_mask != nullptr) && k < PILE_MAXSUB && sBad[s] == 0u && nsub <= PILE_MAXSUB;
                const bool leftmost = first_group && t == (int) (sMax[L] & 0xFFFFu);
                side[j] = make_uint4(node_id, succ_id, delta | ((uint32_t) m << 8) | ((uint32_t) k << 16) | (leftmost ? 0x40000000u : 0u) | (first_group ? 0x80000000u : 0u),
                                     k == 0 ? key >> idx_shift : (uint32_t) (e0 + (uint64_t) k));
                if (leftmost && plist) plist[(size_t) blockIdx.x * PB_THREADS + atomicAdd(&sPiles, 1u)] = pile_who((uint32_t) k, k == 0 ? key >> idx_shift : (uint32_t) (e0 + (uint64_t) k), cc.n_buckets, n_entries);
                if (!first_group && own_mask) atomicOr(&own_mask[j >> 5], 1u << (j & 31u));
            }
            if (!SAMPLE && L == t && k >= 1 && k < PILE_MAXSUB) {
                const unsigned long long rm = sRm[t];
                const uint64_t slot = e0 + (uint64_t) k;
                rec[slot * 4 + 0] = make_uint4(S[0], S[1], S[2], S[3]);
                rec[slot * 4 + 1] = make_uint4(S[4], S[5], S[6], S[7]);
                rec[slot * 4 + 2] = make_uint4(S[8], S[9], S[10], S[11]);
                rec[slot * 4 + 3] = make_uint4(S[12], 0u, (uint32_t) rm, (uint32_t) (rm >> 32));
            }
            if (i == 0) {
                uint32_t tg[PILE_MAXSUB] = {0u, 0u, 0u, 0u};
                unsigned long long rest = lm;
#pragma unroll
                for (int g = 0; g < PILE_MAXSUB; g++) {
                    if (rest) { tg[g] = sTag[s + __builtin_ctzll(rest)]; rest &= rest - 1ull; }
                }
                const bool irregular = sBad[s] != 0u || nsub > PILE_MAXSUB;
                const uint32_t ns1 = (uint32_t) (nsub < PILE_MAXSUB ? nsub : PILE_MAXSUB) - 1u;
                if (!SAMPLE) {
                    const unsigned long long rm = sRm[t];
                    line[0] = make_uint4(S[0], S[1], S[2], S[3]);
                    line[1] = make_uint4(S[4], S[5], S[6], S[7]);
                    line[2] = make_uint4(S[8], S[9], S[10], S[11]);
                    line[3] = make_uint4(S[12], (uint32_t) rm, (uint32_t) (rm >> 32), tg[0] | (tg[1] << 5) | (tg[2] << 10) | (tg[3] << 15) | (ns1 << 20) | (irregular ? 1u << 22 : 0u) | (epoch << 23));
                }
                atomicAdd(&sCount[0], 1u);
                if (irregular) atomicAdd(&sCount[1], 1u);
            }
            if (!SAMPLE && L == s && t == (int) (sMax[s] & 0xFFFFu)) {
                line[4] = make_uint4(cnt, drec.x, drec.z, drec.w);
                line[5] = make_uint4(sSlot[s], sMin[s] >> 16, 0u, 0u);
            }
        }
    }
    if (!SAMPLE && have && t < PB_TILE && !(tgt && cnt <= 64u)) {
        side[j] = make_uint4(node_id, 0xFFFFFFFFu, 0u, 0u);
        if (own_mask) atomicOr(&own_mask[j >> 5], 1u << (j & 31u));
    }
    if (SAMPLE && owned) atomicAdd(&sCount[2], 1u);
    __syncthreads();
    if (!SAMPLE && plist && t == 0) pcount[blockIdx.x] = sPiles;
    if (SAMPLE && t < 3 && sCount[t]) atomicAdd(&pile_cnt[t], (unsigned long long) sCount[t]);
}

constexpr int PILE_RUNS = 8;
__device__ __forceinline__ void pile_list_store(uint4 *line, uint32_t entries, bool ok, int n, const uint32_t (&key)[PILE_RUNS], const uint32_t (&kc)[PILE_RUNS], uint32_t c1_last) {
    uint32_t *lw = reinterpret_cast<uint32_t *>(line);
    if (ok) {
        line[5] = make_uint4(key[0], key[1], key[2], key[3]);
        line[6] = make_uint4(key[4], key[5], key[6], key[7]);
        line[7] = make_uint4(kc[0] | (kc[1] << 16), kc[2] | (kc[3] << 16), kc[4] | (kc[5] << 16), kc[6] | (kc[7] << 16));
        bool dup = false;
#pragma unroll
        for (int a = 0; a < PILE_RUNS; a++)
#pragma unroll
            for (int b = a + 1; b < PILE_RUNS; b++) dup = dup || (b < n && key[a] == key[b]);
        lw[16] = (entries & 255u) | ((uint32_t) n << 8) | ((c1_last & 255u) << 16) | (dup ? 0x80000000u : 0u);
    } else lw[16] = entries & 255u;
}

__global__ void __launch_bounds__(256) k_pile_runs(const uint4 *__restrict__ side, uint64_t n_entries, uint32_t n_buckets, uint4 *__restrict__ tab, const uint2 *__restrict__ runs,
                                                   int n_nodes, int nwin, const unsigned long long *__restrict__ pile_cnt) {
    if (pile_declines(pile_cnt)) return;
    const uint64_t j = (uint64_t) blockIdx.x * 256 + threadIdx.x;
    if (j >= n_entries) return;
    const uint4 sd = side[j];
    if (((sd.z >> 30) & 1u) == 0u) return;
    uint4 *line = tab + (size_t) min(sd.w, n_buckets) * 8;
    const uint4 l4 = line[4], l5 = line[5];
    const uint4 *r0 = reinterpret_cast<const uint4 *>(runs + (size_t) min(sd.x, (uint32_t) n_nodes - 1u) * CL_RMAX);
    const uint4 *r1 = reinterpret_cast<const uint4 *>(runs + (size_t) min(l5.x, (uint32_t) n_nodes - 1u) * CL_RMAX);
    const uint4 a0 = r0[0], a1 = r0[1], a2 = r0[2], a3 = r0[3], b0 = r1[0], b1 = r1[1], b2 = r1[2];
    const int s0 = -(int) ((sd.z >> 8) & 63u), s1 = -(int) (l5.y & 63u), seam = s0 + nwin;
    const uint32_t k0[CL_RMAX] = {a0.x, a0.z, a1.x, a1.z, a2.x, a2.z, a3.x, a3.z}, y0[CL_RMAX] = {a0.y, a0.w, a1.y, a1.w, a2.y, a2.w, a3.y, a3.w};
    const uint32_t k1[6] = {b0.x, b0.z, b1.x, b1.z, b2.x, b2.z}, y1[6] = {b0.y, b0.w, b1.y, b1.w, b2.y, b2.w};
    const int nr0 = (int) (y0[0] >> 24), nr1 = (int) (y1[0] >> 24);
    bool ok = nr0 >= 1 && nr0 <= CL_RMAX && nr1 >= 1 && nr1 <= 6 && s1 <= seam;
    uint32_t ok_[PILE_RUNS], kc_[PILE_RUNS];
#pragma unroll
    for (int k = 0; k < PILE_RUNS; k++) { ok_[k] = 0u; kc_[k] = 0u; }
    int n = 0;
    uint32_t last_key = 0u, last_pos = 0xFFFFFFFFu, c1_last = 0u;
#pragma unroll
    for (int r = CL_RMAX - 1; r >= 0; r--) {
        if (ok && r < nr0) {
            const uint32_t kpos = (uint32_t) (s0 + (int) (y0[r] & 255u) + 64), c0 = (uint32_t) (s0 + (int) ((y0[r] >> 8) & 255u) + 64), c1 = (uint32_t) (s0 + (int) ((y0[r] >> 16) & 255u) + 64);
#pragma unroll
            for (int k = 0; k < PILE_RUNS; k++) if (k == n) { ok_[k] = k0[r]; kc_[k] = kpos | (c0 << 8); }
            last_key = k0[r]; last_pos = kpos; c1_last = c1;
            n++;
        }
    }
#pragma unroll
    for (int r = 5; r >= 0; r--) {
        if (ok && r < nr1) {
            const int c1i = s1 + (int) ((y1[r] >> 16) & 255u);
            if (c1i > seam) {
                const int c0i = max(s1 + (int) ((y1[r] >> 8) & 255u), seam);
                const uint32_t kpos = (uint32_t) (s1 + (int) (y1[r] & 255u) + 64), c1 = (uint32_t) (c1i + 64);
                if (n >= 1 && k1[r] == last_key && kpos == last_pos) c1_last = c1;
                else {
#pragma unroll
                    for (int k = 0; k < PILE_RUNS; k++) if (k == n) { ok_[k] = k1[r]; kc_[k] = kpos | ((uint32_t) (c0i + 64) << 8); }
                    last_key = k1[r]; last_pos = kpos; c1_last = c1;
                    n++;
                }
            }
        }
    }
    ok = ok && n >= 1 && n <= PILE_RUNS;
    pile_list_store(line, l4.x, ok, n, ok_, kc_, c1_last);
}

constexpr int PR_TILE = 3072;
constexpr int PR_TKW = 21;
constexpr int PR_RCAP = 14;
constexpr int PR_SEGS = 32;

template <int RS, int RW>
__device__ __forceinline__ void pile_consensus_one(uint32_t who, bool in, uint32_t *row, uint32_t (*stk)[TK_ROWS], uint16_t (*rbuf)[TK_ROWS], int t, const uint4 *__restrict__ side,
                                                   uint64_t n_entries, uint4 *__restrict__ tab, const uint4 *__restrict__ rec, uint4 *__restrict__ rec2, const ClusterCfg &cc, int U,
                                                   int Lmin, uint32_t *__restrict__ own_mask) {
    const int fs = cc.idx_shift - CL_MBITS;
    const int step = max(16, min(64, cc.w) & ~15);
    const bool further = (who >> 31) != 0u;
    const uint32_t slot = who & 0x7FFFFFFFu;
    uint4 *line = tab + (size_t) (further ? 0u : who) * 8;
    const uint4 *src = further ? rec + (size_t) slot * 4 : (const uint4 *) line;
    uint32_t S[PILE_SW + 1];
    unsigned long long rm = 0ull;
    {
        const uint4 l0 = src[0], l1 = src[1], l2 = src[2], l3 = src[3];
        S[0] = l0.x; S[1] = l0.y; S[2] = l0.z; S[3] = l0.w; S[4] = l1.x; S[5] = l1.y; S[6] = l1.z; S[7] = l1.w;
        S[8] = l2.x; S[9] = l2.y; S[10] = l2.z; S[11] = l2.w; S[12] = l3.x; S[13] = 0u;
        rm = !in ? 0ull : (further ? (((unsigned long long) l3.w << 32) | l3.z) : (((unsigned long long) l3.z << 32) | l3.y));
    }
    const bool act = in && rm != 0ull;
    const int m_min = act ? __clzll((long long) rm) : 0, m_max = act ? 63 - __builtin_ctzll(rm) : 0;
    const int len_v = U + m_max - m_min;
    const int nwin = len_v - Lmin + 1;
    {
        const int ob = 2 * (64 - m_max), w0 = ob >> 5, sh = ob & 31;
        uint32_t m1 = 0u - (uint32_t) (w0 & 1), m2 = 0u - (uint32_t) ((w0 >> 1) & 1), m4 = 0u - (uint32_t) ((w0 >> 2) & 1);
        asm volatile("" : "+v"(m1), "+v"(m2), "+v"(m4));
        uint32_t y1[PILE_SW + 1], y2[PILE_SW + 1], y[PILE_SW + 1];
#pragma unroll
        for (int k = 0; k <= PILE_SW; k++) y1[k] = ((k + 1 <= PILE_SW ? S[k + 1] : 0u) & m1) | (S[k] & ~m1);
#pragma unroll
        for (int k = 0; k <= PILE_SW; k++) y2[k] = ((k + 2 <= PILE_SW ? y1[k + 2] : 0u) & m2) | (y1[k] & ~m2);
#pragma unroll
        for (int k = 0; k <= PILE_SW; k++) y[k] = ((k + 4 <= PILE_SW ? y2[k + 4] : 0u) & m4) | (y2[k] & ~m4);
#pragma unroll
        for (int k = 0; k < (RW > 0 ? RW : PR_TKW); k++) row[k * RS] = k < PILE_SW ? funnel(y[k], y[k + 1], sh) : 0u;
    }
    int nr = 0;
    bool uncovered = false, stack_ovf = false;
    uint32_t cur0 = 0u;
    node_runs_core<true, PR_RCAP, RS, RW>(row, nwin, act, cc, stk, rbuf, t, nr, uncovered, stack_ovf, cur0, step);
    bool ok = act && nr >= 1 && nr <= PR_RCAP && !uncovered && !stack_ovf;
    uint32_t key_[PILE_RUNS], kc_[PILE_RUNS];
#pragma unroll
    for (int k = 0; k < PILE_RUNS; k++) { key_[k] = 0u; kc_[k] = 0u; }
    int n = 0;
    uint32_t last_q = 0xFFFFFFFFu;
    const int nrs = nr < PR_RCAP ? nr : PR_RCAP;
    for (int r = PR_RCAP - 1; r >= 0; r--) {
        if (ok && r < nrs) {
            const uint32_t d = rbuf[r][t];
            const int q = (int) (d & 255u), p0 = (int) (d >> 8);
            if ((uint32_t) q != last_q) {
                uint32_t h, pk;
                kmer_key<RS, RW>(row, q < 192 ? q : 0, true, cc, h, pk);
                const uint32_t kv = cluster_key(h, fs), cv = (uint32_t) (q - m_max + 64) | ((uint32_t) (p0 - m_max + 64) << 8);
#pragma unroll
                for (int k = 0; k < PILE_RUNS; k++) if (k == n) { key_[k] = kv; kc_[k] = cv; }
                n++;
                last_q = (uint32_t) q;
            }
        }
    }
    ok = ok && n >= 1 && n <= PILE_RUNS;
    if (in && further) {
        uint4 *l2 = rec2 + (size_t) slot * 4 - 4;
        pile_list_store(l2, 0u, ok, n, key_, kc_, (uint32_t) (nwin - m_max + 64));
        if (!ok) {
            const uint64_t jb = slot >= 3u ? (uint64_t) slot - 3u : 0ull;
            for (uint64_t j2 = jb; j2 < jb + 64u + 3u && j2 < n_entries; j2++) {
                const uint4 s2 = side[j2];
                if ((s2.z >> 31) && ((s2.z >> 16) & 3u) != 0u && s2.w == slot) atomicOr(&own_mask[j2 >> 5], 1u << (j2 & 31u));
            }
        }
    } else if (in) {
        uint32_t *lw = reinterpret_cast<uint32_t *>(line);
        pile_list_store(line, lw[16], ok, n, key_, kc_, (uint32_t) (nwin - m_max + 64));
        if (!ok) {
            lw[16] = lw[16] & 255u;
            const uint32_t cntb = min(lw[16] & 255u, 64u), e0b = lw[17];
            for (uint32_t i2 = 0; i2 < cntb; i2++) {
                const uint64_t j2 = (uint64_t) e0b + i2;
                if (j2 < n_entries) { const uint4 s2 = side[j2]; if ((s2.z >> 31) && ((s2.z >> 16) & 3u) == 0u) atomicOr(&own_mask[j2 >> 5], 1u << (j2 & 31u)); }
            }
        }
    }
}

__global__ void __launch_bounds__(TK_ROWS) k_pile_runs_consensus(const uint4 *__restrict__ side, uint64_t n_entries, uint32_t n_buckets, uint4 *__restrict__ tab, const uint4 *__restrict__ rec,
                                                                 uint4 *__restrict__ rec2, ClusterCfg cc, int U, int Lmin,
                                                                 const unsigned long long *__restrict__ pile_cnt, uint32_t *__restrict__ own_mask) {
    if (pile_declines(pile_cnt)) return;
    __shared__ uint32_t s[TK_ROWS][PR_TKW];
    __shared__ uint32_t stk[2 * (NR_STACK + 1)][TK_ROWS];
    __shared__ uint16_t rbuf[PR_RCAP + 1][TK_ROWS];
    __shared__ uint32_t sList[PR_TILE];
    __shared__ uint32_t sN;
    const int t = (int) threadIdx.x;
    if (t == 0) sN = 0u;
    __syncthreads();
    const uint64_t base = (uint64_t) blockIdx.x * PR_TILE;
#pragma unroll
    for (int q = 0; q < PR_TILE / TK_ROWS; q++) {
        const uint64_t j = base + (uint64_t) q * TK_ROWS + (uint64_t) t;
        if (j < n_entries) {
            const uint4 sd = side[j];
            if ((sd.z >> 30) & 1u) sList[atomicAdd(&sN, 1u)] = pile_who((sd.z >> 16) & 3u, sd.w, n_buckets, n_entries);
        }
    }
    __syncthreads();
    const int np = (int) sN;
    for (int c0 = 0; c0 < np; c0 += TK_ROWS) {
        const bool in = c0 + t < np;
        pile_consensus_one<1, 0>(sList[in ? c0 + t : 0], in, s[t], stk, rbuf, t, side, n_entries, tab, rec, rec2, cc, U, Lmin, own_mask);
    }
}

__global__ void __launch_bounds__(TK_ROWS) k_pile_runs_consensus_list(const uint32_t *__restrict__ plist, const uint32_t *__restrict__ pcount, uint32_t n_segs, const uint4 *__restrict__ side,
                                                                      uint64_t n_entries, uint4 *__restrict__ tab, const uint4 *__restrict__ rec, uint4 *__restrict__ rec2, ClusterCfg cc,
                                                                      int U, int Lmin, const unsigned long long *__restrict__ pile_cnt, uint32_t *__restrict__ own_mask) {
    if (pile_declines(pile_cnt)) return;
    __shared__ uint32_t s[PILE_SW][TK_ROWS];
    __shared__ uint32_t stk[2 * (NR_STACK + 1)][TK_ROWS];
    __shared__ uint16_t rbuf[PR_RCAP + 1][TK_ROWS];
    __shared__ uint32_t sOff[PR_SEGS + 1];
    const int t = (int) threadIdx.x;
    const uint32_t seg0 = blockIdx.x * PR_SEGS;
    if (t < 64) {
        const uint32_t g = seg0 + (uint32_t) t;
        uint32_t c = (t < PR_SEGS && g < n_segs) ? min(pcount[g], (uint32_t) PB_THREADS) : 0u;
#pragma unroll
        for (int d = 1; d < PR_SEGS; d <<= 1) { const uint32_t o = __shfl_up(c, d); if (t >= d) c += o; }
        if (t < PR_SEGS) sOff[t + 1] = c;
        if (t == 0) sOff[0] = 0u;
    }
    __syncthreads();
    const int np = (int) sOff[PR_SEGS];
    for (int c0 = 0; c0 < np; c0 += TK_ROWS) {
        const int i = c0 + t;
        const bool in = i < np;
        int g = 0;
#pragma unroll
        for (int b = PR_SEGS / 2; b >= 1; b >>= 1) g += (g + b <= PR_SEGS - 1 && (int) sOff[g + b] <= i) ? b : 0;
        const uint32_t who = in ? plist[(size_t) (seg0 + (uint32_t) g) * PB_THREADS + (uint32_t) (i - (int) sOff[g])] : 0u;
        pile_consensus_one<TK_ROWS, PILE_SW>(who, in, &s[0][t], stk, rbuf, t, side, n_entries, tab, rec, rec2, cc, U, Lmin, own_mask);
    }
}

__global__ void __launch_bounds__(256) k_pile_own_ids(const uint32_t *__restrict__ own_mask, const uint32_t *__restrict__ sids, uint64_t n_entries, int32_t *__restrict__ out, uint32_t cap,
                                                      unsigned long long *__restrict__ count, const unsigned long long *__restrict__ pile_cnt) {
    if (pile_declines(pile_cnt)) return;
    __shared__ uint32_t sTot, sBase;
    const uint64_t words = (n_entries + 31) / 32;
    const uint64_t w0 = (uint64_t) blockIdx.x * 1024 + threadIdx.x;
    uint32_t mw[4];
    uint32_t mine = 0u;
#pragma unroll
    for (int q = 0; q < 4; q++) { const uint64_t w = w0 + (uint64_t) q * 256; mw[q] = w < words ? own_mask[w] : 0u; mine += (uint32_t) __popc(mw[q]); }
    if (threadIdx.x == 0) sTot = 0u;
    __syncthreads();
    const uint32_t at = atomicAdd(&sTot, mine);
    __syncthreads();
    if (threadIdx.x == 0) sBase = (uint32_t) atomicAdd(count, (unsigned long long) sTot);
    __syncthreads();
    uint32_t o = sBase + at;
#pragma unroll
    for (int q = 0; q < 4; q++) {
        const uint64_t w = w0 + (uint64_t) q * 256;
        uint32_t m = mw[q];
        while (m) {
            const int b = __builtin_ctz(m);
            m &= m - 1u;
            const uint64_t j = w * 32 + (uint64_t) b;
            if (j < n_entries && o < cap) out[o] = (int32_t) sids[j];
            o++;
        }
    }
}

__global__ void __launch_bounds__(256) k_pile_list_check(const uint4 *__restrict__ side, uint64_t n_entries, uint32_t n_buckets, const uint4 *__restrict__ tab, const uint4 *__restrict__ rec2,
                                                         uint32_t epoch, const uint2 *__restrict__ runs, int n_nodes, int nwin, unsigned long long *__restrict__ out ,
                                                         const unsigned long long *__restrict__ pile_cnt) {
    if (pile_declines(pile_cnt)) return;
    const uint64_t j = (uint64_t) blockIdx.x * 256 + threadIdx.x;
    if (j >= n_entries) return;
    const uint4 sd = side[j];
    if ((sd.z >> 31) == 0u) return;
    const bool further = ((sd.z >> 16) & 3u) != 0u;
    const uint4 *line = further ? rec2 + (size_t) min((uint64_t) sd.w, n_entries - 1) * 4 - 4 : tab + (size_t) min(sd.w, n_buckets) * 8;
    const uint4 l4 = line[4];
    if (!further) { const uint4 l3 = line[3]; if ((l3.w >> 23) != epoch || ((l3.w >> 22) & 1u)) return; }
    const int npr = (int) ((l4.x >> 8) & 15u);
    if (npr == 0) return;
    const uint32_t *lw = reinterpret_cast<const uint32_t *>(line);
    const uint2 *own = runs + (size_t) min(sd.x, (uint32_t) n_nodes - 1u) * CL_RMAX;
    const int code = (int) (own[0].y >> 24);
    if (code == 0 || code == CL_RUNS_FLAGGED) return;
    const int nown = code < CL_RMAX ? code : CL_RMAX;
    const int sB = 64 - (int) ((sd.z >> 8) & 63u);
    bool bad = false;
    int r = nown - 1;
    for (int a = 0; a < npr && a < PILE_RUNS; a++) {
        const uint32_t vx = lw[20 + a], pq = (lw[28 + (a >> 1)] >> (16 * (a & 1))) & 0xFFFFu;
        const uint32_t pqn = a + 1 < npr ? (lw[28 + ((a + 1) >> 1)] >> (16 * ((a + 1) & 1))) & 0xFFFFu : 0u;
        const int kpos = (int) (pq & 255u), c0 = (int) (pq >> 8), c1 = a + 1 < npr ? (int) (pqn >> 8) : (int) ((l4.x >> 16) & 255u);
        const int p0 = max(c0, sB) - sB, p1 = min(c1, sB + nwin) - sB;
        if (p0 >= p1) continue;
        if (r < 0) { bad = true; break; }
        const uint2 o = own[r];
        const int oq = (int) (o.y & 255u), op0 = (int) ((o.y >> 8) & 255u), op1 = (int) ((o.y >> 16) & 255u);
        bad = bad || o.x != vx || oq != kpos - sB || op0 != p0 || op1 != p1;
        r--;
    }
    bad = bad || r >= 0;
    atomicAdd(&out[0], 1ull);
    if (bad) atomicAdd(&out[1], 1ull);
}

__device__ __forceinline__ unsigned long long smear_up(unsigned long long x, int g ) {
    unsigned long long acc = 0ull, pw = x;
    int done = 0;
#pragma unroll
    for (int b = 0; b < 6; b++) {
        if ((g >> b) & 1) { acc |= pw << (done + 1); done += 1 << b; }
        pw |= pw << (1 << b);
    }
    return acc;
}
// ... 95 lines not shown
            rk[a] = k; ry[a] = y;
            vmask |= v ? 1u << a : 0u;
        }
        if (!row_from_pile) {
            const int code = have ? (int) (oy[0] >> 24) : 0;
            vmask = (code == 0 || code == CL_RUNS_FLAGGED) ? 0u : (code >= CL_RMAX ? 0xFFu : ((1u << code) - 1u));
            ry[0] |= (uint32_t) code << 24;
        }
    }
    uint32_t B[9] = {0u, 0u, 0u, 0u, 0u, 0u, 0u, 0u, 0u};
    if (!row_from_pile) load_row9(nd, (uint32_t) Bs, B);
    next_side = side_of(tile + gridDim.x < n_tiles ? tile + gridDim.x : tile);
    const int nr_code = !have ? 0 : (row_from_pile ? 1 : (int) (ry[0] >> 24));
    bool dfr = nr_code == CL_RUNS_FLAGGED;
    const bool active = nr_code != 0 && !dfr;
    vmask = active ? vmask : 0u;
#ifndef PP_NO_COMPACT
    {
        const int sh = vmask ? __builtin_ctz(vmask) : 0;
        const bool s4 = (sh & 4) != 0, s2 = (sh & 2) != 0, s1 = (sh & 1) != 0;
#pragma unroll
        for (int a = 0; a < CL_RMAX; a++) { rk[a] = s4 ? (a + 4 < CL_RMAX ? rk[a + 4] : 0u) : rk[a]; ry[a] = s4 ? (a + 4 < CL_RMAX ? ry[a + 4] : 0u) : ry[a]; }
#pragma unroll
        for (int a = 0; a < CL_RMAX; a++) { rk[a] = s2 ? (a + 2 < CL_RMAX ? rk[a + 2] : 0u) : rk[a]; ry[a] = s2 ? (a + 2 < CL_RMAX ? ry[a + 2] : 0u) : ry[a]; }
#pragma unroll
        for (int a = 0; a < CL_RMAX; a++) { rk[a] = s1 ? (a + 1 < CL_RMAX ? rk[a + 1] : 0u) : rk[a]; ry[a] = s1 ? (a + 1 < CL_RMAX ? ry[a + 1] : 0u) : ry[a]; }
        vmask >>= sh;
    }
#endif
    uint32_t um = 0u;
#pragma unroll
    for (int a = 0; a < CL_RMAX; a++) um |= __ballot(((vmask >> a) & 1u) != 0u) != 0ull ? 1u << a : 0u;
    dfr = dfr || (row_from_pile && (Qr[0].x >> 31) != 0u);
    if (__ballot(active && !row_from_pile) != 0ull) {
#pragma unroll
        for (int a = 0; a < CL_RMAX; a++)
#pragma unroll
            for (int b = a + 1; b < CL_RMAX; b++) dfr = dfr || (((vmask >> a) & (vmask >> b) & 1u) != 0u && rk[a] == rk[b]);
    }
    const int Lbig = cfg.rsoemo > cfg.Lmin ? cfg.rsoemo : cfg.Lmin;
    const int G = min(max(U - Lbig, 0), 63);
    unsigned long long occ = 0ull;
    uint32_t grp = 0u;
    uint32_t Ea[4] = {0u, 0u, 0u, 0u};
    int ea_len = 0;
    auto take_record = [&](int lb, unsigned long long rm, int slot_a, uint32_t group, uint32_t y, bool on, bool home) {
        const int q = (int) (y & 255u), p0 = (int) ((y >> 8) & 255u), p1 = (int) ((y >> 16) & 255u);
        const uint32_t *ss = sl + lb - 4;
        const int ob = 2 * (128 - min(q, 127)), w0 = ob >> 5, sh = ob & 31;
        uint32_t x[10];
#pragma unroll
        for (int k = 0; k < 10; k++) x[k] = ss[w0 + k];
        uint32_t dv = 0u;
        int dk = 0;
        uint32_t dhi = 0u;
#pragma unroll
        for (int k = 0; k < 9; k++) {
            const uint32_t sw = funnel(x[k], x[k + 1], sh) & low_bits32(2 * U - 32 * k);
            B[k] = home ? sw : B[k];
            const uint32_t dd = (sw ^ B[k]) & low_bits32(2 * U - 32 * k);
            if (!LEAN || k < 4) {
                dk = dd ? k : dk;
                dv = dd ? dd : dv;
            } else {
                dhi |= dd;
            }
        }
        const int mism = dv ? 16 * dk + ((31 - __clz((int) dv)) >> 1) : -1;
        unsigned long long oc = q <= 63 ? (rm >> (63 - q)) : (q - 63 >= 64 ? 0ull : (rm << (q - 63)));
        if constexpr (LEAN) {
            const int lo = dhi != 0u ? 64 : max(max(p0 & 63, 1), mism + 1), hi = min(p1, 64);
            oc &= hi > lo ? (~0ull >> (64 - (hi - lo))) << lo : 0ull;
        } else {
            oc &= (p1 >= 64 ? ~0ull : ((1ull << p1) - 1ull)) & ~((1ull << (p0 & 63)) - 1ull) & ~1ull;
            if (mism >= 0) oc &= mism >= 63 ? 0ull : ~((2ull << mism) - 1ull);
        }
        oc = (on && !dfr) ? oc : 0ull;
        if (oc != 0ull) {
            uint32_t E[4];
            {
                const int oe = ob + 2 * U, we = oe >> 5, she = oe & 31;
                uint32_t xe[5];
#pragma unroll
                for (int k = 0; k < 5; k++) xe[k] = ss[we + k];
#pragma unroll
                for (int k = 0; k < 4; k++) E[k] = funnel(xe[k], xe[k + 1], she);
            }
            const int len = min(64, max(0, q - __clzll((long long) rm)));
            if (occ != 0ull) {
                const int nb = 2 * min(len, ea_len);
                uint32_t df = 0u;
#pragma unroll
                for (int k = 0; k < 4; k++) df |= (E[k] ^ Ea[k]) & low_bits32(nb - 32 * k);
                if (df != 0u) dfr = true;
            }
            if (occ == 0ull || len > ea_len) {
#pragma unroll
                for (int k = 0; k < 4; k++) Ea[k] = E[k];
                ea_len = len;
            }
            occ |= oc;
            grp = (grp & ~(3u << (2 * slot_a))) | (group << (2 * slot_a));
        }
    };
    auto bucket_of = [&](int a) -> uint32_t { return ((vmask >> a) & 1u) ? min(rk[a] >> cc.idx_shift, cc.n_buckets) : cc.n_buckets; };
    uint32_t more = 0u;
    bool got_row = !row_from_pile;
    uint4 V0 = make_uint4(0u, 0u, 0u, 0u), V1 = V0;
    int li_next = 0, nl_next = 0, li = 0;
    const int l0 = lane >> 2, c4 = lane & 3;
    uint32_t *bk = sBk[wave];
    auto issue = [&](int a) {
        const uint32_t b = bucket_of(a);
        const uint32_t bp = (uint32_t) __builtin_amdgcn_update_dpp((int) ~b, (int) b, 0x138 , 0xF, 0xF, false);
        const bool lead = b != bp;
        const uint64_t lm = __ballot(lead);
        li_next = (int) __builtin_amdgcn_mbcnt_hi((uint32_t) (lm >> 32), __builtin_amdgcn_mbcnt_lo((uint32_t) lm, 0u)) + (lead ? 1 : 0) - 1;
        nl_next = __popcll(lm);
        if (lead) bk[li_next] = b;
        wave_lds_fence();
        V0 = tab[(size_t) bk[min(l0, nl_next - 1)] * 8 + c4];
        if (nl_next > 16) V1 = tab[(size_t) bk[min(16 + l0, nl_next - 1)] * 8 + c4];
    };
    auto commit = [&]() {
        li = li_next;
        *reinterpret_cast<uint4 *>(sl + l0 * PP_LSTRIDE + 4 * c4) = V0;
        if (nl_next > 16) *reinterpret_cast<uint4 *>(sl + (16 + l0) * PP_LSTRIDE + 4 * c4) = V1;
        for (int r = 32; r < nl_next; r += 16) {
            const uint4 v = tab[(size_t) bk[min(r + l0, nl_next - 1)] * 8 + c4];
            *reinterpret_cast<uint4 *>(sl + (r + l0) * PP_LSTRIDE + 4 * c4) = v;
        }
        wave_lds_fence();
    };
    if (um & 1u) issue(0);
    {
        const bool fur = row_from_pile && ((my.z >> 16) & 3u) != 0u;
        if (__ballot(fur) != 0ull) {
            const uint64_t se = min((uint64_t) my.w, last);
            uint4 Q0 = make_uint4(0u, 0u, 0u, 0u), Q1 = Q0, Q2 = Q0, Q3 = Q0;
            if (fur) { Q0 = rec[se * 4]; Q1 = rec[se * 4 + 1]; Q2 = rec[se * 4 + 2]; Q3 = rec[se * 4 + 3]; }
            uint4 *mine = reinterpret_cast<uint4 *>(sl + lane * PP_LSTRIDE);
            mine[0] = Q0; mine[1] = Q1; mine[2] = Q2; mine[3] = make_uint4(Q3.x, 0u, 0u, 0u);
            wave_lds_fence();
            const int mC = (int) ((my.z >> 8) & 63u);
            const uint32_t *ss = sl + lane * PP_LSTRIDE - 4;
            const int ob = 2 * (128 - mC), w0 = ob >> 5, sh = ob & 31;
            uint32_t x[10];
#pragma unroll
            for (int k = 0; k < 10; k++) x[k] = ss[w0 + k];
#pragma unroll
            for (int k = 0; k < 9; k++) { const uint32_t sw = funnel(x[k], x[k + 1], sh) & low_bits32(2 * U - 32 * k); B[k] = fur ? sw : B[k]; }
            got_row = got_row || fur;
            wave_lds_fence();
        }
    }
#pragma unroll
    for (int a = 0; a < CL_RMAX; a++) {
        const bool use = ((um >> a) & 1u) != 0u;
        if (use) commit();
        if (a + 1 < CL_RMAX && ((um >> (a + 1)) & 1u)) issue(a + 1);
        if (!use) continue;
        const uint4 R3 = *reinterpret_cast<const uint4 *>(sl + li * PP_LSTRIDE + 12);
        const uint32_t y = R3.w, tag = rk[a] & 31u;
        const bool live = ((vmask >> a) & 1u) != 0u && (y >> 23) == epoch;
        dfr = dfr || (live && ((y >> 22) & 1u) != 0u);
        const uint32_t ns = ((y >> 20) & 3u) + 1u;
        uint32_t mt = ((y & 31u) == tag ? 1u : 0u) | ((ns >= 2u && ((y >> 5) & 31u) == tag) ? 2u : 0u) | ((ns >= 3u && ((y >> 10) & 31u) == tag) ? 4u : 0u) |
                      ((ns >= 4u && ((y >> 15) & 31u) == tag) ? 8u : 0u);
        mt = (live && !dfr) ? mt : 0u;
        more |= (mt & ~1u) << (4 * a);
        const bool on = (mt & 1u) != 0u;
        if (__ballot(on) == 0ull) continue;
        const bool home = (!LEAN || PP_HOME_ANY_SLOT || a == 0) && on && row_from_pile && !got_row && ((ry[a] >> 8) & 255u) == 0u;
        got_row = got_row || home;
        take_record(li * PP_LSTRIDE, ((unsigned long long) R3.z << 32) | R3.y, a, 0u, ry[a], on, home);
    }
    {
        const uint4 *rp = run_list_of(next_side);
#pragma unroll
        for (int c = 0; c < CL_RMAX / 2; c++) Qr[c] = rp[c];
    }
    dfr = dfr || (active && !got_row);
    more = dfr ? 0u : more;
    while (__ballot(more != 0u) != 0ull) {
        const bool on = more != 0u;
        const int bit = on ? __builtin_ctz(more) : 0;
        more &= more - 1u;
        const int a = bit >> 2;
        const uint32_t g = (uint32_t) (bit & 3);
        uint32_t ya = ry[0], ka = rk[0];
#pragma unroll
        for (int k = 1; k < CL_RMAX; k++) { ya = a == k ? ry[k] : ya; ka = a == k ? rk[k] : ka; }
        const uint32_t xa = reinterpret_cast<const uint32_t *>(tab)[(size_t) min(ka >> cc.idx_shift, cc.n_buckets) * 32 + 17];
        const uint64_t se = min((uint64_t) xa + g, last);
        const uint4 Q0 = rec[se * 4], Q1 = rec[se * 4 + 1], Q2 = rec[se * 4 + 2], Q3 = rec[se * 4 + 3];
        uint4 *mine = reinterpret_cast<uint4 *>(sl + lane * PP_LSTRIDE);
        mine[0] = Q0; mine[1] = Q1; mine[2] = Q2; mine[3] = Q3;
        wave_lds_fence();
        take_record(lane * PP_LSTRIDE, ((unsigned long long) Q3.w << 32) | Q3.z, a, g, ya, on, false);
        wave_lds_fence();
    }
    const unsigned long long kept = occ & ~smear_up(occ, G);
    const int nkept = __popcll(kept);
    if (nkept > 2) dfr = true;
    auto lookup = [&](int d) -> uint32_t {
        uint32_t ya = 0u, ka = 0u, ga = 0u;
#pragma unroll
        for (int k = 0; k < CL_RMAX; k++) {
            const bool in = ((vmask >> k) & 1u) != 0u && d >= (int) ((ry[k] >> 8) & 255u) && d < (int) ((ry[k] >> 16) & 255u);
            ya = in ? ry[k] : ya; ka = in ? rk[k] : ka; ga = in ? (grp >> (2 * k)) & 3u : ga;
        }
        const uint4 dd = tab[(size_t) min(ka >> cc.idx_shift, cc.n_buckets) * 8 + 4];
        const int mm = (int) (ya & 255u) - d;
        const int cl = (mm >> 3) & 7;
        const uint32_t b0 = ((cl < 4 ? dd.z : dd.w) >> (8 * (cl & 3))) & 255u;
        const uint32_t b1 = cl >= 7 ? (dd.x & 127u) : ((((cl + 1) < 4 ? dd.z : dd.w) >> (8 * ((cl + 1) & 3))) & 255u);
        uint32_t id = 0xFFFFFFFFu;
        for (uint32_t e = b0; e < b1 && e < 64u; e++) {
            const uint64_t ei = min((uint64_t) dd.y + e, last);
            const uint4 sd = side[ei];
            if ((int) ((sd.z >> 8) & 63u) == mm && ((sd.z >> 16) & 3u) == ga) id = sd.x;
        }
        return id;
    };
    unsigned long long slot_val = LOCAL_FIRST_NONE;
    if (active && !dfr && nkept > 0) {
        const int d1 = __builtin_ctzll(kept);
        int p1_home = 0;
#pragma unroll
        for (int k = 0; k < CL_RMAX; k++) p1_home = (((vmask >> k) & 1u) != 0u && ((ry[k] >> 8) & 255u) == 0u) ? (int) ((ry[k] >> 16) & 255u) : p1_home;
        const bool by_succ = d1 < p1_home && (int) (my.z & 255u) == d1 && my.y != 0xFFFFFFFFu;
#ifdef PP_LK
        const int d2 = nkept == 2 ? 63 - __clzll((long long) kept) : -1;
        const int dA = by_succ ? d2 : d1, dB = by_succ ? -1 : d2;
        uint32_t idA = 0xFFFFFFFFu, idB = 0xFFFFFFFFu;
        if (dA >= 0) idA = lookup(dA);
        if (dB >= 0) idB = lookup(dB);
        const uint32_t id1 = by_succ ? my.y : idA;
        const uint32_t id2 = by_succ ? idA : idB;
        bool two = false;
        if (nkept == 2) {
#else
        const uint32_t id1 = by_succ ? my.y : lookup(d1);
        uint32_t id2 = 0u;
        int d2 = 0;
        bool two = false;
        if (nkept == 2) {
            d2 = 63 - __clzll((long long) kept);
            id2 = lookup(d2);
#endif
            const int ds0 = U - cfg.rsoemo + 1;
            const unsigned long long lowm = ds0 <= 0 ? 0ull : (ds0 >= 64 ? ~0ull : ((1ull << ds0) - 1ull));
            two = d2 < ds0 || __popcll(occ & ((1ull << d2) - 1ull) & ~lowm) < 3;
        }
        if (id1 == 0xFFFFFFFFu || (nkept == 2 && id2 == 0xFFFFFFFFu)) dfr = true;
        else {
            slot_val = ((unsigned long long) id1 << 32) | (uint32_t) d1 | (two ? 0x100u : 0u);
            if (two) o.second[Bs - o.src_base] = ((unsigned long long) id2 << 32) | (uint32_t) d2;
            st_rec += two ? 2 : 1;
        }
    }
    if (have) o.first[Bs - o.src_base] = slot_val;
    dfr = dfr && nr_code != 0;
    const uint64_t dm = __ballot(dfr);
    if (dm != 0ull) {
        if (dfr) sDefer[wave][n_defer + (int) __builtin_amdgcn_mbcnt_hi((uint32_t) (dm >> 32), __builtin_amdgcn_mbcnt_lo((uint32_t) dm, 0u))] = Bs;
        n_defer += __popcll(dm);
        wave_lds_fence();
        if (n_defer >= 64) flush_defer();
    }
    }
    flush_defer();
    st_rec = wave_sum_u64(st_rec);
    if (lane == 0 && st_rec) atomicAdd(&o.counters[CNT_VALID_RECORDS], (unsigned long long) st_rec);
}

__global__ void __launch_bounds__(256) k_pile_deg(int32_t n, unsigned long long *__restrict__ first, uint32_t *__restrict__ deg, const unsigned long long *__restrict__ pile_cnt) {
    if (pile_declines(pile_cnt)) return;
    const int64_t i = (int64_t) blockIdx.x * 256 + threadIdx.x;
    if (i >= n) return;
    const unsigned long long f = first[i];
    if (f == LOCAL_FIRST_NONE || deg[i] != 0u) return;
    deg[i] = 1u + (uint32_t) ((f >> 8) & 1ull);
    if (f & 0x100ull) first[i] = f & ~0x100ull;
}

bool pile_plan(const PrefSufCfg &cfg, const ClusterCfg &cc, int eq, int uniform_len, bool masks) {
    if (eq != PILE_EQ || uniform_len <= 0 || masks || cfg.stats) return false;
    if (uniform_len > 144 || blocks_of(uniform_len) > 9) return false;
    if (uniform_len - cfg.Lmin + 1 > 64 || cc.w > 64 || cc.w < 16 || cc.kk > 32 || cc.kk < 1) return false;
    return true;
}
size_t pile_record_bytes(uint64_t n) { return (size_t) (n + 2) * 64; }

size_t pile_table_bytes(uint32_t n_buckets) { return ((size_t) n_buckets + 2) * 128; }

__global__ void k_pile_sample_close(unsigned long long *__restrict__ pile_cnt) {
    const unsigned long long by_entries = pile_cnt[2] / 8ull;
    if (by_entries > pile_cnt[0]) pile_cnt[0] = by_entries;
}

__global__ void k_pile_sample_force(unsigned long long *__restrict__ pile_cnt, unsigned long long buckets, unsigned long long irregular) { pile_cnt[0] = buckets; pile_cnt[1] = irregular; }

void launch_pile_sample(const NodesDev &nd, const ClusterCfg &cc, int uniform_len, const uint32_t *skeys, const uint32_t *sids, const void *dir, unsigned long long *pile_cnt,
                        int no_sample, hipStream_t s) {
    (void) hipMemsetAsync(pile_cnt, 0, PILE_CNT_WORDS * sizeof(unsigned long long), s);
    const uint64_t n_entries = nd.n > 0 ? (uint64_t) nd.n : 0;
    if (no_sample == 2) hipLaunchKernelGGL(k_pile_sample_force, dim3(1), dim3(1), 0, s, pile_cnt, 100ull, 1ull);
    if (n_entries == 0 || no_sample) return;
    const uint64_t tiles = (n_entries + PB_TILE - 1) / PB_TILE;
    const dim3 sample((unsigned) std::max<uint64_t>(1, std::min<uint64_t>(tiles, std::max<uint64_t>(64, tiles / 32)))), block(PB_THREADS);
    hipLaunchKernelGGL((k_pile_build<true>), sample, block, 0, s, nd, skeys, sids, n_entries, (const uint4 *) dir, cc, uniform_len, (uint4 *) nullptr, (uint4 *) nullptr, 0u, (uint4 *) nullptr, pile_cnt,
                       (uint32_t *) nullptr, (uint32_t *) nullptr, (uint32_t *) nullptr);
    hipLaunchKernelGGL(k_pile_sample_close, dim3(1), dim3(1), 0, s, pile_cnt);
}

void launch_pile_build(const NodesDev &nd, const PrefSufCfg &cfg, const ClusterCfg &cc, int uniform_len, const uint32_t *skeys, const uint32_t *sids, const void *dir, void *rec, void *rec2,
                       void *tab, uint32_t epoch, void *side, const void *runs, int nwin, const unsigned long long *pile_cnt, uint32_t *own_mask, void *plist, hipStream_t s) {
    const uint64_t n_entries = nd.n > 0 ? (uint64_t) nd.n : 0;
    if (n_entries == 0) return;
    const uint64_t tiles = (n_entries + PB_TILE - 1) / PB_TILE;
    if (!own_mask) plist = nullptr;
    uint32_t *pl = (uint32_t *) plist, *pc = pl ? pl + tiles * PB_THREADS : nullptr;
    if (own_mask) (void) hipMemsetAsync(own_mask, 0, pile_own_mask_bytes(n_entries), s);
    hipLaunchKernelGGL((k_pile_build<false>), dim3((unsigned) tiles), dim3(PB_THREADS), 0, s, nd, skeys, sids, n_entries, (const uint4 *) dir, cc, uniform_len, (uint4 *) rec, (uint4 *) tab, epoch,
                       (uint4 *) side, const_cast<unsigned long long *>(pile_cnt), own_mask, pl, pc);
    if (pl)
        hipLaunchKernelGGL(k_pile_runs_consensus_list, dim3((unsigned) ((tiles + PR_SEGS - 1) / PR_SEGS)), dim3(TK_ROWS), 0, s, (const uint32_t *) pl, (const uint32_t *) pc, (uint32_t) tiles,
                           (const uint4 *) side, n_entries, (uint4 *) tab, (const uint4 *) rec, (uint4 *) rec2, cc, uniform_len, cfg.Lmin, pile_cnt, own_mask);
    else if (own_mask)
        hipLaunchKernelGGL(k_pile_runs_consensus, dim3((unsigned) ((n_entries + PR_TILE - 1) / PR_TILE)), dim3(TK_ROWS), 0, s, (const uint4 *) side, n_entries, cc.n_buckets, (uint4 *) tab,
                           (const uint4 *) rec, (uint4 *) rec2, cc, uniform_len, cfg.Lmin, pile_cnt, own_mask);
    else
        hipLaunchKernelGGL(k_pile_runs, dim3((unsigned) ((n_entries + 255) / 256)), dim3(256), 0, s, (const uint4 *) side, n_entries, cc.n_buckets, (uint4 *) tab, (const uint2 *) runs, nd.n, nwin, pile_cnt);
}

size_t pile_own_mask_bytes(uint64_t n) { return (size_t) ((n + 31) / 32 + 1024) * 4; }

size_t pile_list_bytes(uint64_t n) { const uint64_t tiles = (n + PB_TILE - 1) / PB_TILE; return (size_t) (tiles * (PB_THREADS + 1) + 64) * 4; }

void launch_pile_own_ids(const uint32_t *own_mask, const uint32_t *sids, uint64_t n_entries, int32_t *list, uint32_t cap, unsigned long long *pile_cnt, hipStream_t s) {
    if (n_entries == 0) return;
    const uint64_t words = (n_entries + 31) / 32;
    hipLaunchKernelGGL(k_pile_own_ids, dim3((unsigned) ((words + 1023) / 1024)), dim3(256), 0, s, own_mask, sids, n_entries, list, cap, pile_cnt + 3, (const unsigned long long *) pile_cnt);
}

void launch_pile_check(const void *side, uint64_t n_entries, uint32_t n_buckets, const void *tab, const void *rec2, uint32_t epoch, const void *runs, int n_nodes, int nwin,
                       unsigned long long *pile_cnt, hipStream_t s) {
    if (n_entries == 0) return;
    hipLaunchKernelGGL(k_pile_list_check, dim3((unsigned) ((n_entries + 255) / 256)), dim3(256), 0, s, (const uint4 *) side, n_entries, n_buckets, (const uint4 *) tab, (const uint4 *) rec2, epoch,
                       (const uint2 *) runs,
                       n_nodes, nwin, pile_cnt + 4, (const unsigned long long *) pile_cnt);
}

constexpr int PSR_IPT = 4;
__global__ void __launch_bounds__(256) k_pile_side_range(const uint4 *__restrict__ side, uint64_t n_entries, uint32_t src_begin, uint32_t src_end, uint4 *__restrict__ out,
                                                         uint64_t out_cap, unsigned long long *__restrict__ cursor, const unsigned long long *__restrict__ pile_cnt) {
    if (pile_declines(pile_cnt)) return;
    __shared__ uint32_t cnt[PSR_IPT * 4];
    __shared__ unsigned long long base;
    const int wave = (int) (threadIdx.x >> 6);
    const uint64_t b0 = (uint64_t) blockIdx.x * (256 * PSR_IPT);
    uint4 v[PSR_IPT];
    uint32_t before[PSR_IPT];
    bool in[PSR_IPT];
#pragma unroll
    for (int k = 0; k < PSR_IPT; k++) {
        const uint64_t j = b0 + (uint64_t) k * 256 + threadIdx.x;
        v[k] = j < n_entries ? side[j] : make_uint4(0xFFFFFFFFu, 0u, 0u, 0u);
        in[k] = j < n_entries && v[k].x >= src_begin && v[k].x < src_end;
        const uint64_t m = __ballot(in[k]);
        before[k] = (uint32_t) __builtin_amdgcn_mbcnt_hi((uint32_t) (m >> 32), __builtin_amdgcn_mbcnt_lo((uint32_t) m, 0u));
        if ((threadIdx.x & 63u) == 0u) cnt[k * 4 + wave] = (uint32_t) __popcll(m);
    }
    __syncthreads();
    if (threadIdx.x == 0) {
        uint32_t tot = 0;
        for (int i = 0; i < PSR_IPT * 4; i++) tot += cnt[i];
        base = tot ? atomicAdd(cursor, (unsigned long long) tot) : 0ull;
    }
    __syncthreads();
    uint32_t run = 0;
#pragma unroll
    for (int k = 0; k < PSR_IPT; k++) {
        uint32_t mine = run;
        for (int w = 0; w < 4; w++) { if (w < wave) mine += cnt[k * 4 + w]; run += cnt[k * 4 + w]; }
        const unsigned long long at = base + mine + before[k];
        if (in[k] && at < out_cap) out[at] = v[k];
    }
}

void launch_pile_probe(const NodesDev &nd, const PrefSufCfg &cfg, const ClusterCfg &cc, int uniform_len, const void *tab, uint32_t epoch, const void *rec, const void *rec2,
                       const void *side, const void *runs, unsigned long long *counters, uint32_t *deg, unsigned long long *first, unsigned long long *second,
                       int32_t *defer_list, uint32_t defer_cap, const unsigned long long *pile_cnt, int n_cu, hipStream_t s, int32_t src_begin, int32_t src_end,
                       void *side_range, unsigned long long *cursor, bool lean) {
    const uint64_t n_entries = nd.n > 0 ? (uint64_t) nd.n : 0;
    if (n_entries == 0 || src_end <= src_begin) return;
    ProbeOut o{};
    o.counters = counters; o.deg = deg; o.first = first; o.second = second; o.src_base = src_begin;
    uint64_t n_mine = n_entries;
    const void *side_src = side;
    if (src_begin != 0 || src_end != nd.n) {
        n_mine = (uint64_t) (src_end - src_begin);
        (void) hipMemsetAsync(cursor, 0, sizeof(unsigned long long), s);
        hipLaunchKernelGGL(k_pile_side_range, dim3((unsigned) ((n_entries + 256 * PSR_IPT - 1) / (256 * PSR_IPT))), dim3(256), 0, s, (const uint4 *) side, n_entries,
                           (uint32_t) src_begin, (uint32_t) src_end, (uint4 *) side_range, n_mine, cursor, pile_cnt);
        side_src = side_range;
    }
    const uint64_t tiles = (n_mine + PP_WAVES * 64 - 1) / (PP_WAVES * 64);
    const dim3 grid((unsigned) std::max<uint64_t>(1, std::min<uint64_t>(tiles, (uint64_t) std::max(1, n_cu) * (PP_OCC * 4 / PP_WAVES)))), block(PP_WAVES * 64);
    hipLaunchKernelGGL(lean ? k_pile_probe<true> : k_pile_probe<false>, grid, block, 0, s, cfg, cc, uniform_len, nd, n_entries, n_mine, nd.n, (const uint4 *) tab, epoch, (const uint4 *) rec, (const uint4 *) rec2,
                       (const uint4 *) side, (const uint4 *) side_src, (const uint2 *) runs, o, defer_list, defer_cap, pile_cnt);
}

void launch_pile_deg(int32_t n, unsigned long long *first, uint32_t *deg, const unsigned long long *pile_cnt, hipStream_t s) {
    if (n <= 0) return;
    hipLaunchKernelGGL(k_pile_deg, dim3((unsigned) (((int64_t) n + 255) / 256)), dim3(256), 0, s, n, first, deg, pile_cnt);
}

}
```

Baseline: 5.128 billion edges/s.

## Make pile build persistent with software-pipelined prefetch of next tiles

Adds a persistent-grid variant of the pile build kernel, enabled by default with grid = CUs × occupancy. Each workgroup loops over tiles and issues the key, directory and row loads for the next one to three tiles while it processes the current tile. The goal is to hide the chain of dependent global loads (key, then dir, then row) and cut per-tile block launch overhead. In exchange it holds more registers live for the prefetched data, which may lower occupancy, and adds an extra barrier per tile.

```diff
diff --git a/alga_amd/csrc/engine.hip b/alga_amd/csrc/engine.hip
--- a/alga_amd/csrc/engine.hip
+++ b/alga_amd/csrc/engine.hip
@@ -212,7 +212,7 @@
             }
             if (pile) {
                 launch_pile_sample(nd, cc, pp.uniform_len, (const uint32_t *) e->cl_keys[1].p, (const uint32_t *) e->cl_vals[1].p, e->cl_dir.p,
-                                   (unsigned long long *) e->cl_pile_cnt.p, e->opt_pile >= 2 ? e->opt_pile - 1 : 0, s);
+                                   (unsigned long long *) e->cl_pile_cnt.p, e->opt_pile >= 2 ? e->opt_pile - 1 : 0, s, e->opt_pile_build_ahead, e->n_cu);
                 if ((rc = alga_check_launch(e, "k_pile_build<sample>"))) return rc;
             }
             HIP_TRY(e, launch_cluster_gather(nd, cc, pp.cluster_eq, (const uint32_t *) e->cl_keys[1].p, (const uint32_t *) e->cl_vals[1].p, (const uint32_t *) e->cl_meta.p,
@@ -227,7 +227,7 @@
                 const bool from_consensus = e->opt_pile_runs != 0;
                 launch_pile_build(nd, cfg, cc, pp.uniform_len, (const uint32_t *) e->cl_keys[1].p, (const uint32_t *) e->cl_vals[1].p, e->cl_dir.p, e->cl_pile_rec.p, e->cl_pile_rec2.p, e->cl_pile_tab.p,
                                   e->pile_epoch, e->cl_pile_succ.p, e->cl_runs.p, pp.uniform_len - cfg.Lmin + 1, (const unsigned long long *) e->cl_pile_cnt.p,
-                                  from_consensus ? (uint32_t *) e->cl_pile_own.p : nullptr, (from_consensus && e->opt_pile_runs_list) ? e->cl_pile_list.p : nullptr, s);
+                                  from_consensus ? (uint32_t *) e->cl_pile_own.p : nullptr, (from_consensus && e->opt_pile_runs_list) ? e->cl_pile_list.p : nullptr, s, e->opt_pile_build_ahead, e->n_cu);
                 if ((rc = alga_check_launch(e, "k_pile_build"))) return rc;
                 if (keys_only) {
                     launch_pile_own_ids((const uint32_t *) e->cl_pile_own.p, (const uint32_t *) e->cl_vals[1].p, (uint64_t) nd.n, (int32_t *) e->cl_defer.p, (uint32_t) nd.n,
@@ -632,6 +632,9 @@
         e->opt_pile_runs_list = value != 0;
     } else if (!strcmp(name, "pile_deg_fold")) {
         e->opt_pile_deg_fold = value != 0;
+    } else if (!strcmp(name, "pile_build_ahead")) {
+        if (value < 0 || value > (1 << 20)) return alga_fail(e, ALGA_ERR_INVALID_ARGUMENT, "option pile_build_ahead: 0 one tile per workgroup, 1 persistent, 2 .. 2^20 (tests) that many workgroups");
+        e->opt_pile_build_ahead = (int) value;
     } else if (!strcmp(name, "pile_probe_lean")) {
         e->opt_pile_probe_lean = value != 0;
     } else if (!strcmp(name, "pile_check")) {
diff --git a/alga_amd/csrc/engine_internal.h b/alga_amd/csrc/engine_internal.h
--- a/alga_amd/csrc/engine_internal.h
+++ b/alga_amd/csrc/engine_internal.h
@@ -58,6 +58,7 @@
     int    opt_pile_runs_list = 1;
     DevBuf cl_pile_list;
     int    opt_pile_deg_fold = 1;
+    int    opt_pile_build_ahead = 1;
     int    opt_pile_probe_lean = 1;
     bool   pile_deg_pending = false;
     int    opt_pile_check = 0;
diff --git a/alga_amd/csrc/prefsuf_kernels.h b/alga_amd/csrc/prefsuf_kernels.h
--- a/alga_amd/csrc/prefsuf_kernels.h
+++ b/alga_amd/csrc/prefsuf_kernels.h
@@ -65,14 +65,16 @@
 size_t     pile_record_bytes(uint64_t n);
 size_t     pile_table_bytes(uint32_t n_buckets);
 void       launch_pile_sample(const NodesDev &nd, const ClusterCfg &cc, int uniform_len, const uint32_t *skeys , const uint32_t *sids , const void *dir,
-                              unsigned long long *pile_cnt , int no_sample, hipStream_t s);
+                              unsigned long long *pile_cnt , int no_sample, hipStream_t s,
+                              int ahead , int n_cu);
 constexpr int PILE_CNT_WORDS = 6;
 size_t     pile_own_mask_bytes(uint64_t n);
 size_t     pile_list_bytes(uint64_t n);
 void       launch_pile_build(const NodesDev &nd, const PrefSufCfg &cfg, const ClusterCfg &cc, int uniform_len, const uint32_t *skeys, const uint32_t *sids, const void *dir, void *rec,
                              void *rec2 , void *tab, uint32_t epoch, void *side, const void *runs, int nwin, const unsigned long long *pile_cnt,
                              uint32_t *own_mask ,
-                             void *plist , hipStream_t s);
+                             void *plist , hipStream_t s,
+                             int ahead , int n_cu);
 void       launch_pile_own_ids(const uint32_t *own_mask, const uint32_t *sids, uint64_t n_entries, int32_t *list, uint32_t cap, unsigned long long *pile_cnt, hipStream_t s);
 void       launch_pile_check(const void *side, uint64_t n_entries, uint32_t n_buckets, const void *tab, const void *rec2, uint32_t epoch, const void *runs, int n_nodes, int nwin,
                              unsigned long long *pile_cnt, hipStream_t s);
diff --git a/alga_amd/csrc/prefsuf_pile.hip b/alga_amd/csrc/prefsuf_pile.hip
--- a/alga_amd/csrc/prefsuf_pile.hip
+++ b/alga_amd/csrc/prefsuf_pile.hip
@@ -30,179 +30,261 @@
     }
 }
 
+struct PileBuildLds {
+    uint32_t sRow[PB_THREADS][PILE_SW];
+    unsigned long long sKm[PB_THREADS];
+    unsigned long long sLead[PB_THREADS];
+    unsigned long long sRm[PB_THREADS];
+    uint32_t sMin[PB_THREADS], sMax[PB_THREADS];
+    uint32_t sBad[PB_THREADS];
+    uint8_t sTag[PB_THREADS];
+    uint2 sZw[PB_THREADS];
+    uint32_t sCount[3];
+    uint32_t sPiles;
+};
+
+__device__ __forceinline__ uint64_t pb_entry(uint64_t tile, int t, uint64_t n_entries) {
+    const uint64_t j = tile * PB_TILE + (uint64_t) t;
+    return j < n_entries ? j : (n_entries ? n_entries - 1 : 0);
+}
+__device__ __forceinline__ uint32_t pb_load_key(const uint32_t *__restrict__ skeys, uint64_t tile, int t, uint64_t n_entries, bool live) {
+    return live ? skeys[pb_entry(tile, t, n_entries)] : 0xFFFFFFFFu;
+}
+struct PbDir { uint4 rec; uint32_t id; };
+__device__ __forceinline__ PbDir pb_load_dir(const uint4 *__restrict__ dir, const uint32_t *__restrict__ sids, uint64_t tile, int t, uint64_t n_entries, uint32_t key, int idx_shift, bool live) {
+    const bool tgt = tile * PB_TILE + (uint64_t) t < n_entries && key != 0xFFFFFFFFu;
+    PbDir d{make_uint4(0u, 0u, 0u, 0u), 0u};
+    if (live) d.id = sids[pb_entry(tile, t, n_entries)];
+    if (tgt) d.rec = dir[key >> idx_shift];
+    return d;
+}
+struct PbOwn { bool have, tgt, owned, part; };
+__device__ __forceinline__ PbOwn pb_own(uint64_t tile, int t, uint64_t n_entries, uint32_t key, const uint4 &drec) {
+    const uint64_t base = tile * PB_TILE, j = base + (uint64_t) t, e0 = drec.x;
+    PbOwn o;
+    o.have = j < n_entries;
+    o.tgt = o.have && key != 0xFFFFFFFFu;
+    o.owned = o.tgt && e0 >= base && e0 < base + PB_TILE && e0 <= j && j - e0 < (uint64_t) drec.y;
+    o.part = o.owned && drec.y <= 64u;
+    return o;
+}
+__device__ __forceinline__ void pb_load_row(const NodesDev &nd, uint64_t tile, int t, uint64_t n_entries, uint32_t key, const PbDir &d, uint32_t (&row)[9]) {
+#pragma unroll
+    for (int q = 0; q < 9; q++) row[q] = 0u;
+    if (pb_own(tile, t, n_entries, key, d.rec).part) load_row9(nd, min(d.id, (uint32_t) nd.n - 1u), row);
+}
+
+__device__ __forceinline__ void pile_build_rows(PileBuildLds &lds, const uint32_t key, const uint32_t (&row)[9], const ClusterCfg &cc, const int U) {
+    const int t = (int) threadIdx.x, kk = cc.kk;
+    const uint32_t meta = key >> (cc.idx_shift - CL_MBITS);
+    lds.sLead[t] = 0ull; lds.sRm[t] = 0ull; lds.sMin[t] = 0xFFFFFFFFu; lds.sMax[t] = 0u; lds.sBad[t] = 0u;
+    if (t < 3) lds.sCount[t] = 0u;
+    if (t == 0) lds.sPiles = 0u;
+    const int m = (int) (meta & 63u);
+    uint32_t A[PILE_SW];
+    {
+        const int w0 = (2 * m) >> 5, sh = (2 * m) & 31;
+        const int lo = 2 * (64 - m), hi = lo + 2 * U;
+        uint32_t Rp[18];
+#pragma unroll
+        for (int k = 0; k < 18; k++) Rp[k] = 0u;
+#pragma unroll
+        for (int k = 0; k < 9; k++) Rp[4 + k] = row[k];
+        uint32_t m1 = 0u - (uint32_t) (w0 & 1), m2 = 0u - (uint32_t) ((w0 >> 1) & 1);
+        asm volatile("" : "+v"(m1), "+v"(m2));
+        uint32_t y1[PILE_SW + 3], y[PILE_SW + 1];
+#pragma unroll
+        for (int k = 0; k < PILE_SW + 3; k++) y1[k] = (Rp[k + 1] & m1) | (Rp[k] & ~m1);
+#pragma unroll
+        for (int k = 0; k <= PILE_SW; k++) y[k] = (y1[k + 2] & m2) | (y1[k] & ~m2);
+#pragma unroll
+        for (int k = 0; k < PILE_SW; k++) A[k] = funnel(y[k], y[k + 1], sh) & low_bits32(hi - 32 * k) & ~low_bits32(lo - 32 * k);
+    }
+    const unsigned long long kmask = kk >= 32 ? ~0ull : ((1ull << (2 * kk)) - 1ull);
+    const unsigned long long kmer = (((unsigned long long) A[5] << 32) | A[4]) & kmask;
+    lds.sKm[t] = kmer;
+#pragma unroll
+    for (int k = 0; k < PILE_SW; k++) lds.sRow[t][k] = A[k];
+}
+
+template <bool SAMPLE>
+__device__ __forceinline__ void pile_build_tile(PileBuildLds &lds, const uint64_t tile, const uint64_t n_entries, const NodesDev &nd, const uint32_t key, const PbDir &pd,
+                                                const ClusterCfg &cc, const int U, uint4 *__restrict__ rec, uint4 *__restrict__ tab, const uint32_t epoch, uint4 *__restrict__ side,
+                                                uint32_t *__restrict__ own_mask, uint32_t *__restrict__ plist, uint32_t *__restrict__ pcount, uint32_t &sampled) {
+    const int idx_shift = cc.idx_shift;
+    const int t = (int) threadIdx.x;
+    const uint64_t base = tile * PB_TILE, j = base + (uint64_t) t;
+    const uint32_t node_id = min(pd.id, (uint32_t) nd.n - 1u);
+    const uint4 drec = pd.rec;
+    const int m = (int) ((key >> (cc.idx_shift - CL_MBITS)) & 63u);
+    const PbOwn own = pb_own(tile, t, n_entries, key, drec);
+    const bool have = own.have, tgt = own.tgt, owned = own.owned, part = own.part;
+    const uint64_t e0 = drec.x;
+    const uint32_t cnt = drec.y;
+    const int s = owned ? (int) (e0 - base) : 0;
+    const int i = owned ? (int) (j - e0) : 0;
+    if (owned && i == 0) lds.sZw[t] = make_uint2(drec.z, drec.w);
+    __syncthreads();
+    const unsigned long long kmer = lds.sKm[t];
+    int L = t;
+    if (part) {
+        for (int u = 0; u < i; u++) if (lds.sKm[s + u] == kmer) { L = s + u; break; }
+        if (L == t) {
+            atomicOr(&lds.sLead[s], 1ull << i);
+            lds.sTag[t] = (uint8_t) (cluster_key(kmer_hash((uint32_t) kmer & cc.lo_mask, (uint32_t) (kmer >> 32) & cc.hi_mask), idx_shift - CL_MBITS) & 31u);
+        }
+        atomicMin(&lds.sMin[L], ((uint32_t) m << 16) | (uint32_t) t);
+        atomicMax(&lds.sMax[L], ((uint32_t) m << 16) | (uint32_t) t);
+        const unsigned long long bit = 1ull << (63 - m);
+        if (atomicOr(&lds.sRm[L], bit) & bit) atomicOr(&lds.sBad[s], 1u);
+    }
+    __syncthreads();
+    uint32_t *sSlot = reinterpret_cast<uint32_t *>(lds.sKm);
+    int my_slot = -1, my_rank = 0;
+    if (part) {
+        const unsigned long long lm = lds.sLead[s];
+        const int kgrp = __popcll(lm & ((1ull << (L - s)) - 1ull));
+        if (kgrp < PILE_MAXSUB) {
+            int before = 0;
+            unsigned long long rest = lm;
+#pragma unroll
+            for (int g = 0; g < PILE_MAXSUB - 1; g++) {
+                if (g < kgrp) { before += __popcll(lds.sRm[s + __builtin_ctzll(rest)]); rest &= rest - 1ull; }
+            }
+            my_rank = m == 0 ? 0 : __popcll(lds.sRm[L] >> (64 - m));
+            my_slot = s + before + my_rank;
+            if (my_slot < s + (int) cnt) sSlot[my_slot] = node_id; else my_slot = -1;
+        }
+    }
+    auto consensus = [&](int k) { return lds.sRow[lds.sMax[L] & 0xFFFFu][k] | lds.sRow[lds.sMin[L] & 0xFFFFu][k]; };
+    auto consensus4 = [&](int k) { return make_uint4(consensus(k), consensus(k + 1), consensus(k + 2), consensus(k + 3)); };
+    if (part) {
+        const int lo = 2 * (64 - m), hi = lo + 2 * U;
+        uint32_t diff = 0u;
+#pragma unroll
+        for (int k = 0; k < PILE_SW; k++) {
+            diff |= (lds.sRow[t][k] ^ consensus(k)) & low_bits32(hi - 32 * k) & ~low_bits32(lo - 32 * k);
+            if ((k & 3) == 3) __builtin_amdgcn_sched_barrier(0);
+        }
+        if (diff != 0u) atomicOr(&lds.sBad[s], 1u);
+    }
+    __syncthreads();
+    if (owned) {
+        uint4 *line = tab + (size_t) (key >> idx_shift) * 8;
+        if (!part) {
+            if (i == 0) {
+                if (!SAMPLE) { line[3] = make_uint4(0u, 0u, 0u, (1u << 22) | (epoch << 23)); line[4] = make_uint4(127u, drec.x, lds.sZw[t].x, lds.sZw[t].y); }
+                atomicAdd(&lds.sCount[0], 1u); atomicAdd(&lds.sCount[1], 1u);
+            }
+        } else {
+            const unsigned long long lm = lds.sLead[s];
+            const int nsub = __popcll(lm);
+            const int iL = L - s;
+            const int k = __popcll(lm & ((1ull << iL) - 1ull));
+            if (!SAMPLE) {
+                const unsigned long long right = m == 0 ? 0ull : (lds.sRm[L] >> (64 - m));
+                uint32_t succ_id = 0xFFFFFFFFu, delta = 0u;
+                if (right != 0ull && my_slot > s && my_rank >= 1) { succ_id = sSlot[my_slot - 1]; delta = 1u + (uint32_t) __builtin_ctzll(right); }
+                const bool first_group = (k == 0 || own_mask != nullptr) && k < PILE_MAXSUB && lds.sBad[s] == 0u && nsub <= PILE_MAXSUB;
+                const bool leftmost = first_group && t == (int) (lds.sMax[L] & 0xFFFFu);
+                side[j] = make_uint4(node_id, succ_id, delta | ((uint32_t) m << 8) | ((uint32_t) k << 16) | (leftmost ? 0x40000000u : 0u) | (first_group ? 0x80000000u : 0u),
+                                     k == 0 ? key >> idx_shift : (uint32_t) (e0 + (uint64_t) k));
+                if (leftmost && plist) plist[(size_t) tile * PB_THREADS + atomicAdd(&lds.sPiles, 1u)] = pile_who((uint32_t) k, k == 0 ? key >> idx_shift : (uint32_t) (e0 + (uint64_t) k), cc.n_buckets, n_entries);
+                if (!first_group && own_mask) atomicOr(&own_mask[j >> 5], 1u << (j & 31u));
+            }
+            if (!SAMPLE && L == t && k >= 1 && k < PILE_MAXSUB) {
+                const unsigned long long rm = lds.sRm[t];
+                const uint64_t slot = e0 + (uint64_t) k;
+                rec[slot * 4 + 0] = consensus4(0); __builtin_amdgcn_sched_barrier(0);
+                rec[slot * 4 + 1] = consensus4(4); __builtin_amdgcn_sched_barrier(0);
+                rec[slot * 4 + 2] = consensus4(8); __builtin_amdgcn_sched_barrier(0);
+                rec[slot * 4 + 3] = make_uint4(consensus(12), 0u, (uint32_t) rm, (uint32_t) (rm >> 32));
+            }
+            if (i == 0) {
+                uint32_t tg[PILE_MAXSUB] = {0u, 0u, 0u, 0u};
+                unsigned long long rest = lm;
+#pragma unroll
+                for (int g = 0; g < PILE_MAXSUB; g++) {
+                    if (rest) { tg[g] = lds.sTag[s + __builtin_ctzll(rest)]; rest &= rest - 1ull; }
+                }
+                const bool irregular = lds.sBad[s] != 0u || nsub > PILE_MAXSUB;
+                const uint32_t ns1 = (uint32_t) (nsub < PILE_MAXSUB ? nsub : PILE_MAXSUB) - 1u;
+                if (!SAMPLE) {
+                    const unsigned long long rm = lds.sRm[t];
+                    line[0] = consensus4(0); __builtin_amdgcn_sched_barrier(0);
+                    line[1] = consensus4(4); __builtin_amdgcn_sched_barrier(0);
+                    line[2] = consensus4(8); __builtin_amdgcn_sched_barrier(0);
+                    line[3] = make_uint4(consensus(12), (uint32_t) rm, (uint32_t) (rm >> 32), tg[0] | (tg[1] << 5) | (tg[2] << 10) | (tg[3] << 15) | (ns1 << 20) | (irregular ? 1u << 22 : 0u) | (epoch << 23));
+                }
+                atomicAdd(&lds.sCount[0], 1u);
+                if (irregular) atomicAdd(&lds.sCount[1], 1u);
+            }
+            if (!SAMPLE && L == s && t == (int) (lds.sMax[s] & 0xFFFFu)) {
+                line[4] = make_uint4(cnt, drec.x, lds.sZw[s].x, lds.sZw[s].y);
+                line[5] = make_uint4(sSlot[s], lds.sMin[s] >> 16, 0u, 0u);
+            }
+        }
+    }
+    if (!SAMPLE && have && t < PB_TILE && !(tgt && cnt <= 64u)) {
+        side[j] = make_uint4(node_id, 0xFFFFFFFFu, 0u, 0u);
+        if (own_mask) atomicOr(&own_mask[j >> 5], 1u << (j & 31u));
+    }
+    if (SAMPLE && owned) atomicAdd(&lds.sCount[2], 1u);
+    __syncthreads();
+    if (!SAMPLE && plist && t == 0) pcount[tile] = lds.sPiles;
+    if (SAMPLE && t < 3) sampled += lds.sCount[t];
+}
+
 template <bool SAMPLE>
 __global__ void __launch_bounds__(PB_THREADS, 6) k_pile_build(NodesDev nd, const uint32_t *__restrict__ skeys, const uint32_t *__restrict__ sids, uint64_t n_entries, const uint4 *__restrict__ dir, ClusterCfg cc, int U,
                                                            uint4 *__restrict__ rec, uint4 *__restrict__ tab, uint32_t epoch,
                                                            uint4 *__restrict__ side, unsigned long long *__restrict__ pile_cnt, uint32_t *__restrict__ own_mask,
                                                            uint32_t *__restrict__ plist, uint32_t *__restrict__ pcount) {
     if (!SAMPLE && pile_declines(pile_cnt)) return;
-    const int idx_shift = cc.idx_shift, kk = cc.kk;
-    __shared__ uint32_t sRow[PB_THREADS][PILE_SW];
-    __shared__ unsigned long long sKm[PB_THREADS];
-    __shared__ unsigned long long sLead[PB_THREADS];
-    __shared__ unsigned long long sRm[PB_THREADS];
-    __shared__ uint32_t sMin[PB_THREADS], sMax[PB_THREADS];
-    __shared__ uint32_t sBad[PB_THREADS];
-    __shared__ uint8_t sTag[PB_THREADS];
-    __shared__ uint32_t sCount[3];
-    __shared__ uint32_t sPiles;
+    __shared__ PileBuildLds lds;
     const int t = (int) threadIdx.x;
-    const uint64_t base = (uint64_t) blockIdx.x * PB_TILE;
-    const uint64_t j = base + (uint64_t) t;
-    const bool have = j < n_entries;
-    const uint64_t jc = have ? j : (n_entries ? n_entries - 1 : 0);
-    const uint32_t key = skeys[jc], node_id = min(sids[jc], (uint32_t) nd.n - 1u);
-    const uint32_t meta = key >> (cc.idx_shift - CL_MBITS);
-    const bool tgt = have && key != 0xFFFFFFFFu;
-    uint4 drec = make_uint4(0u, 0u, 0u, 0u);
-    if (tgt) drec = dir[key >> idx_shift];
-    const uint64_t e0 = drec.x;
-    const uint32_t cnt = drec.y;
-    const bool owned = tgt && e0 >= base && e0 < base + PB_TILE && e0 <= j && j - e0 < (uint64_t) cnt;
-    const int s = owned ? (int) (e0 - base) : 0;
-    const int i = owned ? (int) (j - e0) : 0;
-    const bool part = owned && cnt <= 64u;
-    uint32_t row[9] = {0u, 0u, 0u, 0u, 0u, 0u, 0u, 0u, 0u};
-    if (part) load_row9(nd, node_id, row);
-    sLead[t] = 0ull; sRm[t] = 0ull; sMin[t] = 0xFFFFFFFFu; sMax[t] = 0u; sBad[t] = 0u;
-    if (t < 3) sCount[t] = 0u;
-    if (t == 0) sPiles = 0u;
-    __syncthreads();
-    const int m = (int) (meta & 63u);
-    uint32_t A[PILE_SW];
-    {
-        const int w0 = (2 * m) >> 5, sh = (2 * m) & 31;
-        const int lo = 2 * (64 - m), hi = lo + 2 * U;
-        uint32_t Rp[18];
-#pragma unroll
-        for (int k = 0; k < 18; k++) Rp[k] = 0u;
-#pragma unroll
-        for (int k = 0; k < 9; k++) Rp[4 + k] = row[k];
-        uint32_t m1 = 0u - (uint32_t) (w0 & 1), m2 = 0u - (uint32_t) ((w0 >> 1) & 1);
-        asm volatile("" : "+v"(m1), "+v"(m2));
-        uint32_t y1[PILE_SW + 3], y[PILE_SW + 1];
-#pragma unroll
-        for (int k = 0; k < PILE_SW + 3; k++) y1[k] = (Rp[k + 1] & m1) | (Rp[k] & ~m1);
-#pragma unroll
-        for (int k = 0; k <= PILE_SW; k++) y[k] = (y1[k + 2] & m2) | (y1[k] & ~m2);
-#pragma unroll
-        for (int k = 0; k < PILE_SW; k++) A[k] = funnel(y[k], y[k + 1], sh) & low_bits32(hi - 32 * k) & ~low_bits32(lo - 32 * k);
-    }
-    const unsigned long long kmask = kk >= 32 ? ~0ull : ((1ull << (2 * kk)) - 1ull);
-    const unsigned long long kmer = (((unsigned long long) A[5] << 32) | A[4]) & kmask;
-    sKm[t] = kmer;
-#pragma unroll
-    for (int k = 0; k < PILE_SW; k++) sRow[t][k] = A[k];
-    __syncthreads();
-    int L = t;
-    if (part) {
-        for (int u = 0; u < i; u++) if (sKm[s + u] == kmer) { L = s + u; break; }
-        if (L == t) {
-            atomicOr(&sLead[s], 1ull << i);
-            sTag[t] = (uint8_t) (cluster_key(kmer_hash((uint32_t) kmer & cc.lo_mask, (uint32_t) (kmer >> 32) & cc.hi_mask), idx_shift - CL_MBITS) & 31u);
-        }
-        atomicMin(&sMin[L], ((uint32_t) m << 16) | (uint32_t) t);
-        atomicMax(&sMax[L], ((uint32_t) m << 16) | (uint32_t) t);
-        const unsigned long long bit = 1ull << (63 - m);
-        if (atomicOr(&sRm[L], bit) & bit) atomicOr(&sBad[s], 1u);
-    }
-    __syncthreads();
-    uint32_t *sSlot = reinterpret_cast<uint32_t *>(sKm);
-    int my_slot = -1, my_rank = 0;
-    if (part) {
-        const unsigned long long lm = sLead[s];
-        const int kgrp = __popcll(lm & ((1ull << (L - s)) - 1ull));
-        if (kgrp < PILE_MAXSUB) {
-            int before = 0;
-            unsigned long long rest = lm;
-#pragma unroll
-            for (int g = 0; g < PILE_MAXSUB - 1; g++) {
-                if (g < kgrp) { before += __popcll(sRm[s + __builtin_ctzll(rest)]); rest &= rest - 1ull; }
-            }
-            my_rank = m == 0 ? 0 : __popcll(sRm[L] >> (64 - m));
-            my_slot = s + before + my_rank;
-            if (my_slot < s + (int) cnt) sSlot[my_slot] = node_id; else my_slot = -1;
-        }
-    }
-    uint32_t S[PILE_SW];
-#pragma unroll
-    for (int k = 0; k < PILE_SW; k++) S[k] = 0u;
-    if (part) {
-        const int t0 = (int) (sMax[L] & 0xFFFFu), t1 = (int) (sMin[L] & 0xFFFFu);
-        const int lo = 2 * (64 - m), hi = lo + 2 * U;
-        uint32_t diff = 0u;
-#pragma unroll
-        for (int k = 0; k < PILE_SW; k++) {
-            S[k] = sRow[t0][k] | sRow[t1][k];
-            diff |= (A[k] ^ S[k]) & low_bits32(hi - 32 * k) & ~low_bits32(lo - 32 * k);
-        }
-        if (diff != 0u) atomicOr(&sBad[s], 1u);
-    }
-    __syncthreads();
-    if (owned) {
-        uint4 *line = tab + (size_t) (key >> idx_shift) * 8;
-        if (!part) {
-            if (i == 0) {
-                if (!SAMPLE) { line[3] = make_uint4(0u, 0u, 0u, (1u << 22) | (epoch << 23)); line[4] = make_uint4(127u, drec.x, drec.z, drec.w); }
-                atomicAdd(&sCount[0], 1u); atomicAdd(&sCount[1], 1u);
-            }
-        } else {
-            const unsigned long long lm = sLead[s];
-            const int nsub = __popcll(lm);
-            const int iL = L - s;
-            const int k = __popcll(lm & ((1ull << iL) - 1ull));
-            if (!SAMPLE) {
-                const unsigned long long right = m == 0 ? 0ull : (sRm[L] >> (64 - m));
-                uint32_t succ_id = 0xFFFFFFFFu, delta = 0u;
-                if (right != 0ull && my_slot > s && my_rank >= 1) { succ_id = sSlot[my_slot - 1]; delta = 1u + (uint32_t) __builtin_ctzll(right); }
-                const bool first_group = (k == 0 || own_mask != nullptr) && k < PILE_MAXSUB && sBad[s] == 0u && nsub <= PILE_MAXSUB;
-                const bool leftmost = first_group && t == (int) (sMax[L] & 0xFFFFu);
-                side[j] = make_uint4(node_id, succ_id, delta | ((uint32_t) m << 8) | ((uint32_t) k << 16) | (leftmost ? 0x40000000u : 0u) | (first_group ? 0x80000000u : 0u),
-                                     k == 0 ? key >> idx_shift : (uint32_t) (e0 + (uint64_t) k));
-                if (leftmost && plist) plist[(size_t) blockIdx.x * PB_THREADS + atomicAdd(&sPiles, 1u)] = pile_who((uint32_t) k, k == 0 ? key >> idx_shift : (uint32_t) (e0 + (uint64_t) k), cc.n_buckets, n_entries);
-                if (!first_group && own_mask) atomicOr(&own_mask[j >> 5], 1u << (j & 31u));
-            }
-            if (!SAMPLE && L == t && k >= 1 && k < PILE_MAXSUB) {
-                const unsigned long long rm = sRm[t];
-                const uint64_t slot = e0 + (uint64_t) k;
-                rec[slot * 4 + 0] = make_uint4(S[0], S[1], S[2], S[3]);
-                rec[slot * 4 + 1] = make_uint4(S[4], S[5], S[6], S[7]);
-                rec[slot * 4 + 2] = make_uint4(S[8], S[9], S[10], S[11]);
-                rec[slot * 4 + 3] = make_uint4(S[12], 0u, (uint32_t) rm, (uint32_t) (rm >> 32));
-            }
-            if (i == 0) {
-                uint32_t tg[PILE_MAXSUB] = {0u, 0u, 0u, 0u};
-                unsigned long long rest = lm;
-#pragma unroll
-                for (int g = 0; g < PILE_MAXSUB; g++) {
-                    if (rest) { tg[g] = sTag[s + __builtin_ctzll(rest)]; rest &= rest - 1ull; }
-                }
-                const bool irregular = sBad[s] != 0u || nsub > PILE_MAXSUB;
-                const uint32_t ns1 = (uint32_t) (nsub < PILE_MAXSUB ? nsub : PILE_MAXSUB) - 1u;
-                if (!SAMPLE) {
-                    const unsigned long long rm = sRm[t];
-                    line[0] = make_uint4(S[0], S[1], S[2], S[3]);
-                    line[1] = make_uint4(S[4], S[5], S[6], S[7]);
-                    line[2] = make_uint4(S[8], S[9], S[10], S[11]);
-                    line[3] = make_uint4(S[12], (uint32_t) rm, (uint32_t) (rm >> 32), tg[0] | (tg[1] << 5) | (tg[2] << 10) | (tg[3] << 15) | (ns1 << 20) | (irregular ? 1u << 22 : 0u) | (epoch << 23));
-                }
-                atomicAdd(&sCount[0], 1u);
-                if (irregular) atomicAdd(&sCount[1], 1u);
-            }
-            if (!SAMPLE && L == s && t == (int) (sMax[s] & 0xFFFFu)) {
-                line[4] = make_uint4(cnt, drec.x, drec.z, drec.w);
-                line[5] = make_uint4(sSlot[s], sMin[s] >> 16, 0u, 0u);
-            }
-        }
-    }
-    if (!SAMPLE && have && t < PB_TILE && !(tgt && cnt <= 64u)) {
-        side[j] = make_uint4(node_id, 0xFFFFFFFFu, 0u, 0u);
-        if (own_mask) atomicOr(&own_mask[j >> 5], 1u << (j & 31u));
-    }
-    if (SAMPLE && owned) atomicAdd(&sCount[2], 1u);
-    __syncthreads();
-    if (!SAMPLE && plist && t == 0) pcount[blockIdx.x] = sPiles;
-    if (SAMPLE && t < 3 && sCount[t]) atomicAdd(&pile_cnt[t], (unsigned long long) sCount[t]);
+    const uint64_t tile = blockIdx.x;
+    const uint32_t key = pb_load_key(skeys, tile, t, n_entries, true);
+    const PbDir pd = pb_load_dir(dir, sids, tile, t, n_entries, key, cc.idx_shift, true);
+    uint32_t row[9];
+    pb_load_row(nd, tile, t, n_entries, key, pd, row);
+    uint32_t sampled = 0u;
+    pile_build_rows(lds, key, row, cc, U);
+    pile_build_tile<SAMPLE>(lds, tile, n_entries, nd, key, pd, cc, U, rec, tab, epoch, side, own_mask, plist, pcount, sampled);
+    if (SAMPLE && t < 3 && sampled) atomicAdd(&pile_cnt[t], (unsigned long long) sampled);
+}
+
+template <bool SAMPLE>
+__global__ void __launch_bounds__(PB_THREADS, 6) k_pile_build_ahead(NodesDev nd, const uint32_t *__restrict__ skeys, const uint32_t *__restrict__ sids, uint64_t n_entries, const uint4 *__restrict__ dir, ClusterCfg cc, int U,
+                                                                 uint4 *__restrict__ rec, uint4 *__restrict__ tab, uint32_t epoch,
+                                                                 uint4 *__restrict__ side, unsigned long long *__restrict__ pile_cnt, uint32_t *__restrict__ own_mask,
+                                                                 uint32_t *__restrict__ plist, uint32_t *__restrict__ pcount, uint64_t n_tiles) {
+    if (!SAMPLE && pile_declines(pile_cnt)) return;
+    __shared__ PileBuildLds lds;
+    const int t = (int) threadIdx.x;
+    const uint64_t G = gridDim.x;
+    uint64_t tile = blockIdx.x;
+    if (tile >= n_tiles) return;
+    uint32_t k1 = pb_load_key(skeys, tile, t, n_entries, true);
+    uint32_t k2 = pb_load_key(skeys, tile + G, t, n_entries, tile + G < n_tiles);
+    uint32_t k3 = pb_load_key(skeys, tile + 2 * G, t, n_entries, tile + 2 * G < n_tiles);
+    PbDir d1 = pb_load_dir(dir, sids, tile, t, n_entries, k1, cc.idx_shift, true);
+    PbDir d2 = pb_load_dir(dir, sids, tile + G, t, n_entries, k2, cc.idx_shift, tile + G < n_tiles);
+    uint32_t r1[9];
+    pb_load_row(nd, tile, t, n_entries, k1, d1, r1);
+    uint32_t sampled = 0u;
+    for (; tile < n_tiles; tile += G) {
+        const uint32_t kc = k1;
+        const PbDir dc = d1;
+        pile_build_rows(lds, kc, r1, cc, U);
+        k1 = k2; d1 = d2; k2 = k3;
+        pb_load_row(nd, tile + G, t, n_entries, k1, d1, r1);
+        d2 = pb_load_dir(dir, sids, tile + 2 * G, t, n_entries, k2, cc.idx_shift, tile + 2 * G < n_tiles);
+        k3 = pb_load_key(skeys, tile + 3 * G, t, n_entries, tile + 3 * G < n_tiles);
+        pile_build_tile<SAMPLE>(lds, tile, n_entries, nd, kc, dc, cc, U, rec, tab, epoch, side, own_mask, plist, pcount, sampled);
+        __syncthreads();
+    }
+    if (SAMPLE && t < 3 && sampled) atomicAdd(&pile_cnt[t], (unsigned long long) sampled);
 }
 
 constexpr int PILE_RUNS = 8;
@@ -904,29 +986,44 @@
 
 __global__ void k_pile_sample_force(unsigned long long *__restrict__ pile_cnt, unsigned long long buckets, unsigned long long irregular) { pile_cnt[0] = buckets; pile_cnt[1] = irregular; }
 
+constexpr int PB_OCC = 6;
+static unsigned pile_build_grid(int ahead, int n_cu, uint64_t tiles) {
+    if (ahead <= 0) return 0u;
+    if (ahead >= 2) return (unsigned) std::min(ahead, 1 << 20);
+    return (unsigned) std::max<uint64_t>(1, std::min<uint64_t>(tiles, (uint64_t) std::max(1, n_cu) * PB_OCC));
+}
+
 void launch_pile_sample(const NodesDev &nd, const ClusterCfg &cc, int uniform_len, const uint32_t *skeys, const uint32_t *sids, const void *dir, unsigned long long *pile_cnt,
-                        int no_sample, hipStream_t s) {
+                        int no_sample, hipStream_t s, int ahead, int n_cu) {
     (void) hipMemsetAsync(pile_cnt, 0, PILE_CNT_WORDS * sizeof(unsigned long long), s);
     const uint64_t n_entries = nd.n > 0 ? (uint64_t) nd.n : 0;
     if (no_sample == 2) hipLaunchKernelGGL(k_pile_sample_force, dim3(1), dim3(1), 0, s, pile_cnt, 100ull, 1ull);
     if (n_entries == 0 || no_sample) return;
     const uint64_t tiles = (n_entries + PB_TILE - 1) / PB_TILE;
     const dim3 sample((unsigned) std::max<uint64_t>(1, std::min<uint64_t>(tiles, std::max<uint64_t>(64, tiles / 32)))), block(PB_THREADS);
-    hipLaunchKernelGGL((k_pile_build<true>), sample, block, 0, s, nd, skeys, sids, n_entries, (const uint4 *) dir, cc, uniform_len, (uint4 *) nullptr, (uint4 *) nullptr, 0u, (uint4 *) nullptr, pile_cnt,
-                       (uint32_t *) nullptr, (uint32_t *) nullptr, (uint32_t *) nullptr);
+    if (const unsigned grid = pile_build_grid(ahead, n_cu, sample.x))
+        hipLaunchKernelGGL((k_pile_build_ahead<true>), dim3(grid), block, 0, s, nd, skeys, sids, n_entries, (const uint4 *) dir, cc, uniform_len, (uint4 *) nullptr, (uint4 *) nullptr, 0u, (uint4 *) nullptr,
+                           pile_cnt, (uint32_t *) nullptr, (uint32_t *) nullptr, (uint32_t *) nullptr, (uint64_t) sample.x);
+    else
+        hipLaunchKernelGGL((k_pile_build<true>), sample, block, 0, s, nd, skeys, sids, n_entries, (const uint4 *) dir, cc, uniform_len, (uint4 *) nullptr, (uint4 *) nullptr, 0u, (uint4 *) nullptr, pile_cnt,
+                           (uint32_t *) nullptr, (uint32_t *) nullptr, (uint32_t *) nullptr);
     hipLaunchKernelGGL(k_pile_sample_close, dim3(1), dim3(1), 0, s, pile_cnt);
 }
 
 void launch_pile_build(const NodesDev &nd, const PrefSufCfg &cfg, const ClusterCfg &cc, int uniform_len, const uint32_t *skeys, const uint32_t *sids, const void *dir, void *rec, void *rec2,
-                       void *tab, uint32_t epoch, void *side, const void *runs, int nwin, const unsigned long long *pile_cnt, uint32_t *own_mask, void *plist, hipStream_t s) {
+                       void *tab, uint32_t epoch, void *side, const void *runs, int nwin, const unsigned long long *pile_cnt, uint32_t *own_mask, void *plist, hipStream_t s, int ahead, int n_cu) {
     const uint64_t n_entries = nd.n > 0 ? (uint64_t) nd.n : 0;
     if (n_entries == 0) return;
     const uint64_t tiles = (n_entries + PB_TILE - 1) / PB_TILE;
     if (!own_mask) plist = nullptr;
     uint32_t *pl = (uint32_t *) plist, *pc = pl ? pl + tiles * PB_THREADS : nullptr;
     if (own_mask) (void) hipMemsetAsync(own_mask, 0, pile_own_mask_bytes(n_entries), s);
-    hipLaunchKernelGGL((k_pile_build<false>), dim3((unsigned) tiles), dim3(PB_THREADS), 0, s, nd, skeys, sids, n_entries, (const uint4 *) dir, cc, uniform_len, (uint4 *) rec, (uint4 *) tab, epoch,
-                       (uint4 *) side, const_cast<unsigned long long *>(pile_cnt), own_mask, pl, pc);
+    if (const unsigned grid = pile_build_grid(ahead, n_cu, tiles))
+        hipLaunchKernelGGL((k_pile_build_ahead<false>), dim3(grid), dim3(PB_THREADS), 0, s, nd, skeys, sids, n_entries, (const uint4 *) dir, cc, uniform_len, (uint4 *) rec, (uint4 *) tab, epoch,
+                           (uint4 *) side, const_cast<unsigned long long *>(pile_cnt), own_mask, pl, pc, tiles);
+    else
+        hipLaunchKernelGGL((k_pile_build<false>), dim3((unsigned) tiles), dim3(PB_THREADS), 0, s, nd, skeys, sids, n_entries, (const uint4 *) dir, cc, uniform_len, (uint4 *) rec, (uint4 *) tab, epoch,
+                           (uint4 *) side, const_cast<unsigned long long *>(pile_cnt), own_mask, pl, pc);
     if (pl)
         hipLaunchKernelGGL(k_pile_runs_consensus_list, dim3((unsigned) ((tiles + PR_SEGS - 1) / PR_SEGS)), dim3(TK_ROWS), 0, s, (const uint32_t *) pl, (const uint32_t *) pc, (uint32_t) tiles,
                            (const uint4 *) side, n_entries, (uint4 *) tab, (const uint4 *) rec, (uint4 *) rec2, cc, uniform_len, cfg.Lmin, pile_cnt, own_mask);
```

Result: slower. 4.866 billion edges/s (-5.1%).
